# AtharvRN/dflash

Hardware: AMD Instinct MI355X
Metric: accepted_tokens_per_sec (higher is better)
Workload: dtype bf16

## Files before the change

### dflash_amd/_lib.py

```python
from __future__ import annotations

import ctypes as C
import os

import torch

HERE = os.path.dirname(os.path.abspath(__file__))
LIB_PATH = os.environ.get("DFL_LIB_PATH") or os.path.join(HERE, "lib", "libdflash_hip.so")

_p, _i, _i64, _f, _u64 = C.c_void_p, C.c_int, C.c_int64, C.c_float, C.c_uint64


class Rows(C.Structure):
    _fields_ = [("frag", C.c_void_p), ("rows", C.c_void_p), ("ld", C.c_int64), ("ss", C.c_void_p),
                ("nss", C.c_int32), ("norm_w", C.c_void_p), ("eps", C.c_float), ("valid_word", C.c_int32),
                ("mode", C.c_int32)]


_r = C.POINTER(Rows)


class RowsBatch(C.Structure):
    _fields_ = [("r0", Rows), ("frag_stride", C.c_int64), ("rows_stride", C.c_int64), ("ss_stride", C.c_int64)]


_rb = C.POINTER(RowsBatch)

W_BF16, W_E4M3 = 0, 1


class Weight(C.Structure):
    _fields_ = [("wp", C.c_void_p), ("scale", C.c_void_p), ("format", C.c_int32)]


_w = C.POINTER(Weight)

SIGNATURES = {
    "dfl_version": (_i, []),
    "dfl_last_error": (C.c_char_p, []),
    "dfl_pack_weight": (_i, [_p, _p, _i, _i, _p]),
    "dfl_pack_weight_gateup": (_i, [_p, _p, _p, _i, _i, _p]),
    "dfl_set_dyn": (_i, [_p, _i, _i, _i, _i, _p]),
    "dfl_set_dyn2": (_i, [_p, _i, _i, _i, _i, _p]),
    "dfl_pack_rows": (_i, [_p, _i64, _i, _i, _p, _p, _i, _p]),
    "dfl_gemm_f32": (_i, [_p, _r, _r, _i, _i, _i, _i, _p, _p, _p]),
    "dfl_gemm_silu_mul": (_i, [_w, _r, _i, _i, _p, _p, _p]),
    "dfl_gemm_resid": (_i, [_w, _r, _i, _i, _p, _i64, _i, _p, _i64, _p, _p, _p]),
    "dfl_embed_rows": (_i, [_p, _p, _p, _i, _p, _p, _i, _p]),
    "dfl_pack_weight_fp8": (_i, [_p, _p, _i, _i, _p]),
    "dfl_pack_weight_gateup_fp8": (_i, [_p, _p, _p, _i, _i, _p]),
    "dfl_argmax_ws_bytes": (_i64, []),
    "dfl_gemm_argmax": (_i, [_w, _r, _i, _i, _i, _i, _p, _i, _p, _p, _i, _p, _p, _p, _p, _p]),
    "dfl_gemm_sample": (_i, [_w, _r, _i, _i, _i, _i, _p, _i, _p, _p, _i, _p, _p, _u64, _f, _i, _p, _i, _i, _i, _p]),
    "dfl_sample_rows": (_i, [_p, _i64, _i, _i, _u64, _f, _i, _i, _p, _i, _p, _p, _p]),
    "dfl_sample_rows_nucleus": (_i, [_p, _i64, _i64, _i, _i, _i, _i, _p, _i, _i, _i, _p, _i, _i, _p, _u64, _p, _i, _p, _f,
                                     _p, _f, _i, _i, _p, _i64, _i, _p, _p, _p]),
    "dfl_norm_pack": (_i, [_p, _i, _i64, _i, _i, _p, _p, _p, _p, _p, _i64, _p, _f, _p, _i, _p, _i, _p]),
    "dfl_qknorm_rope_append": (_i, [_p, _i, _i64, _i, _i, _i, _i, _i, _i, _i, _i, _p, _p, _f, _p, _p, _i, _p, _p, _p, _i, _p,
                                    _i, _i, _p]),
    "dfl_attn_ws_bytes": (_i64, [_i, _i]),
    "dfl_block_attn": (_i, [_p, _p, _p, _i, _i, _i, _f, _i, _p, _i, _p, _i, _p, _p]),
    "dfl_attn_fused_ws_bytes": (_i64, [_i, _i, _i]),
    "dfl_attn_fused": (_i, [_p, _i, _i64, _i, _i, _i, _i, _i, _i, _i, _i, _p, _p, _f, _p, _p, _i, _p, _p, _i, _f, _i, _p,
                            _i, _p, _i, _p, _p]),
    "dfl_attn_head_ws_bytes": (_i64, [_i, _i, _i]),
    "dfl_attn_head": (_i, [_p, _i64, _i, _i, _i, _p, _i64, _i, _i, _i, _i, _p, _p, _f, _p, _p, _i, _p, _p, _i, _f, _i,
                           _p, _i, _i, _i, _i, _i, _p, _i, _p, _i64, _p]),
    "dfl_attn_head_oproj": (_i, [_p, _i64, _i, _i, _i, _p, _i64, _i, _i, _i, _i, _p, _p, _f, _p, _p, _i, _p, _p, _i, _f, _i,
                                 _p, _i, _i, _i, _i, _p, _i, _p, _p, _i, _p, _i64, _p, _p, _p]),
    "dfl_attn_head_cand": (_i, [_p, _i64, _i, _i, _i, _i, _i64, _i, _i, _p, _p, _f, _p, _p, _i, _p, _p, _i, _f, _i, _i,
                                _p, _i, _p, _i64, _i64, _i, _p, _p, _i64, _i, _p]),
    "dfl_attn_head_batch_f32": (_i, [_p, _i, _i64, _i64, _i, _i, _i, _i, _i64, _i, _i, _p, _p, _f, _p, _p, _i, _p, _p, _i, _i64, _f,
                                     _i, _p, _i, _p, _i, _p, _i64, _p]),
    "dfl_attn_head_batch": (_i, [_p, _i64, _i, _i, _i, _i, _i64, _i, _i, _p, _p, _f, _p, _p, _i, _p, _p, _i, _i64, _f, _i,
                                 _p, _i, _p, _i, _p, _i64, _i64, _i, _p]),
    "dfl_topk_rows": (_i, [_p, _i64, _i, _i, _i, _p, _p, _p, _p]),
    "dfl_candidate_select": (_i, [_p, _i64, _p, _i64, _p, _i, _i, _p, _i64, _p, _p, _i, _p, _p]),
    "dfl_moe_route": (_i, [_p, _i, _i, _i, _i, _p, _p, _p, _p, _p, _i, _p]),
    "dfl_moe_router": (_i, [_p, _i64, _p, _f, _p, _p, _i, _i, _i, _i, _p, _i, _p, _p, _p, _p, _p, _i, _p, _p]),
    "dfl_gemm_silu_mul_experts": (_i, [_p, _i64, _r, _i, _i, _i, _p, _i64, _p, _p, _p, _p]),
    "dfl_moe_gate_up": (_i, [_w, _p, _i, _i, _i, _p, _p, _p, _p, _i, _p]),
    "dfl_moe_down": (_i, [_w, _i64, _p, _i64, _p, _p, _p, _i, _i, _i, _i, _p, _p]),
    "dfl_argmax": (_i, [_p, _i, _i, _i64, _p, _p]),
    "dfl_accept_commit": (_i, [_p, _p, _i, _p, _i64, _p, _p, _i, _p, _p, _i, _i64, _p, _p]),
    "dfl_prefill_rows_padded": (_i64, [_i]),
    "dfl_prefill_gemm_rows": (_i, [_p, _p, _i, _i, _i, _p, _i64, _p]),
    "dfl_prefill_gemm_resid": (_i, [_p, _p, _i, _i, _i, _p, _i64, _p, _i64, _p]),
    "dfl_prefill_gemm_silu": (_i, [_p, _p, _i, _i, _i, _p, _p]),
    "dfl_prefill_norm_pack": (_i, [_p, _i64, _i, _i, _p, _f, _p, _p]),
    "dfl_prefill_pack_rows": (_i, [_p, _i64, _i, _i, _p, _p]),
    "dfl_prefill_qk_rope": (_i, [_p, _i64, _i, _i, _i, _i, _i, _i, _p, _p, _f, _p, _p, _i, _i, _p, _p, _i, _i, _p]),
    "dfl_prefill_attn": (_i, [_p, _i64, _i, _p, _p, _i, _i, _i, _i, _f, _p, _p]),
    "dfl_prefill_moe_max_tiles": (_i64, [_i, _i, _i]),
    "dfl_prefill_moe_max_items": (_i64, [_i, _i, _i]),
    "dfl_prefill_moe_route": (_i, [_p, _i64, _i, _i, _i, _i, _p, _p, _p, _p, _p, _p, _p, _p, _p, _i, _p]),
    "dfl_prefill_moe_gather": (_i, [_p, _i, _i, _i, _i, _p, _p, _p, _p]),
    "dfl_prefill_moe_gemm_silu": (_i, [_p, _i64, _p, _p, _p, _i, _i, _i, _p, _i, _p, _p, _p]),
    "dfl_prefill_moe_gemm_down": (_i, [_p, _i64, _p, _p, _p, _i, _i, _i, _p, _p, _i, _p]),
    "dfl_prefill_moe_combine": (_i, [_p, _p, _i, _i, _i, _p, _i64, _p, _i64, _p, _p]),
    "dfl_moe_grouped_gate_up": (_i, [_w, _i64, _p, _p, _p, _i, _i, _i, _p, _i, _p, _p, _p]),
    "dfl_moe_grouped_down": (_i, [_w, _i64, _p, _p, _p, _i, _i, _i, _p, _p, _i, _p]),
    "dfl_batch_tiles": (_i, [_i]),
    "dfl_batch_ksplit": (_i, [_i]),
    "dfl_gemm_batch_ws_bytes": (_i64, [_i, _i]),
    "dfl_gemm_f32_batch": (_i, [_w, _rb, _i, _i, _i, _p, _p, _p]),
    "dfl_gemm_silu_mul_batch": (_i, [_w, _rb, _i, _i, _i, _p, _i64, _p, _p, _p]),
    "dfl_gemm_resid_batch": (_i, [_p, _rb, _i, _i, _i, _p, _i64, _i64, _i, _p, _i64, _i64, _p, _i64, _p, _p, _p]),
    "dfl_gemm_argmax_batch": (_i, [_w, _rb, _i, _i, _i, _i, _i, _p, _i, _p, _p, _i64, _i, _p, _i64, _p]),
    "dfl_gemm_sample_batch": (_i, [_w, _rb, _i, _i, _i, _i, _i, _p, _i, _p, _p, _i64, _i, _p, _i64, _p, _p, _f, _i, _i, _i, _i,
                                   _p]),
    "dfl_embed_rows_batch": (_i, [_p, _p, _i64, _i, _p, _i64, _i, _p, _i64, _p, _i, _p]),
    "dfl_norm_frag_batch": (_i, [_p, _i64, _i64, _i, _p, _i, _i64, _i, _p, _i64, _i64, _p, _f, _p, _i64, _i, _p, _i, _p]),
    "dfl_kv_append_batch": (_i, [_p, _i, _i64, _i, _i, _i, _i, _i, _i, _i, _i, _p, _i64, _f, _p, _p, _i, _p, _p, _i,
                                 _i64, _i64, _p, _i, _p]),
    "dfl_attn_fused_batch_ws_bytes": (_i64, [_i, _i, _i, _i]),
    "dfl_attn_fused_batch": (_i, [_p, _i, _i64, _i, _i, _i, _i, _i, _i, _i, _i, _i, _p, _p, _f, _p, _p, _i, _p, _p, _i,
                                  _i64, _f, _i, _p, _i, _p, _i, _p, _i64, _p]),
    "dfl_accept_commit_batch": (_i, [_p, _i64, _p, _i64, _i, _p, _i64, _i64, _p, _p, _p, _i, _p, _p, _i64, _i, _p, _p, _p]),
    "dfl_admit_slot": (_i, [_i, _i, _p, _i, _p, _p, _i64, _i64, _p, _p, _i, _p, _p, _i64, _i, _p, _i, _p, _p, _i, _p, _i64,
                            _i64, _p]),
}

_lib = None


class DFlashHipError(RuntimeError):
    pass


def lib():
    global _lib
    if _lib is None:
        if not os.path.exists(LIB_PATH):
            raise DFlashHipError(
                f"{LIB_PATH} not found: build it with `python -m dflash_amd.build` (hipcc, gfx950). "
                "dflash_amd has no CPU or PyTorch fallback for its kernels.")
        handle = C.CDLL(LIB_PATH)
        for name, (res, args) in SIGNATURES.items():
            fn = getattr(handle, name)
            fn.restype, fn.argtypes = res, args
        if handle.dfl_version() != 1:
            raise DFlashHipError(f"ABI version mismatch: library {handle.dfl_version()} != binding 1")
        _lib = handle
    return _lib


def check(rc: int, what: str) -> None:
    if rc != 0:
        raise DFlashHipError(f"{what} failed (rc={rc}): {lib().dfl_last_error().decode()}")
```

### dflash_amd/csrc/gemm_rows.h

```cpp
#pragma once
#include "dfl_common.h"

namespace {

enum { EPI_F32 = 0, EPI_SILU = 1, EPI_ARGMAX = 2, EPI_RESID = 3, EPI_SILU_E = 4 ,
       EPI_SAMPLE = 5 ,
       EPI_SAMPLE_T = 6  };

struct RowSrc {
  const bf16x8 *frag;
  const bf16_t *rows;
  int64_t ld;
  const float *ss;
  int nss;
  const bf16_t *nw;
  float eps;
  int valid_word;
  int mode;
};

__device__ __forceinline__ bf16x8 ld_stream(const bf16x8 *p) { return __builtin_nontemporal_load(p); }

template <int NF, int AUX = 2 >
__device__ __forceinline__ void load_ksteps(bf16x8 (&wr)[NF], const bf16x8 *first, int nf, int l, int half = -1) {
  const __amdgpu_buffer_rsrc_t r =
      __builtin_amdgcn_make_buffer_rsrc(const_cast<bf16x8 *>(first), 0, (nf < 0 ? 0 : nf) * 1024, 0x00020000);
  const int voff = (half < 0 || ((l >> 3) & 1) == half) ? l * 16 : 0x40000000;
#pragma unroll
  for (int f = 0; f < NF; ++f)
    wr[f] = __builtin_bit_cast(bf16x8, __builtin_amdgcn_raw_buffer_load_b128(r, voff + (f & 3) * 1024, (f >> 2) * 4096, AUX));
}

template <int NF, int AUX = 2>
__device__ __forceinline__ void load_ksteps_w8(bf16x8 (&wr)[NF / 2], const bf16x8 *first, int nf, int l, int half = -1) {
  static_assert(NF % 2 == 0, "W8: a wave's share is a whole number of k-step pairs");
  load_ksteps<NF / 2, AUX>(wr, first, nf >> 1, l, half);
}

__device__ __forceinline__ bf16x8 w8_frag(bf16x8 raw, int hi) {
  const u32x4 q = __builtin_bit_cast(u32x4, raw);
  const uint32_t d0 = hi ? q[2] : q[0], d1 = hi ? q[3] : q[1];
  const bf16x2 a = __builtin_amdgcn_cvt_scalef32_pk_bf16_fp8(d0, 1.0f, false);
  const bf16x2 b = __builtin_amdgcn_cvt_scalef32_pk_bf16_fp8(d0, 1.0f, true);
  const bf16x2 c = __builtin_amdgcn_cvt_scalef32_pk_bf16_fp8(d1, 1.0f, false);
  const bf16x2 d = __builtin_amdgcn_cvt_scalef32_pk_bf16_fp8(d1, 1.0f, true);
  return (bf16x8){a[0], a[1], b[0], b[1], c[0], c[1], d[0], d[1]};
}

template <bool W8, int NW>
__device__ __forceinline__ bf16x8 weight_frag(const bf16x8 (&wr)[NW], int f) {
  if constexpr (W8)
    return w8_frag(wr[f >> 1], f & 1);
  else
    return wr[f];
}

typedef float f32x16 __attribute__((ext_vector_type(16)));
__device__ __forceinline__ f32x16 tile_scales(const float *wscale, int t) {
  typedef const __attribute__((address_space(4))) f32x16 *cptr;
  return *(cptr)(uintptr_t)(wscale + (size_t)__builtin_amdgcn_readfirstlane(t) * 16);
}
__device__ __forceinline__ f32x4 lane_scales(const f32x16 &s, int fg) {
  f32x4 o;
#pragma unroll
  for (int r = 0; r < 4; ++r) o[r] = fg == 0 ? s[r] : fg == 1 ? s[4 + r] : fg == 2 ? s[8 + r] : s[12 + r];
  return o;
}

__device__ __forceinline__ float row_sum16(float v) {
  v += __builtin_bit_cast(float, __builtin_amdgcn_mov_dpp(__builtin_bit_cast(int, v), 0xB1, 0xF, 0xF, true));
  v += __builtin_bit_cast(float, __builtin_amdgcn_mov_dpp(__builtin_bit_cast(int, v), 0x4E, 0xF, 0xF, true));
  v += __builtin_bit_cast(float, __builtin_amdgcn_mov_dpp(__builtin_bit_cast(int, v), 0x141, 0xF, 0xF, true));
  v += __builtin_bit_cast(float, __builtin_amdgcn_mov_dpp(__builtin_bit_cast(int, v), 0x140, 0xF, 0xF, true));
  return v;
}

template <int NF, bool NORM = true>
__device__ __forceinline__ void issue_x(const RowSrc &s, const int (&ks)[NF], int l, int nv, bf16x8 (&raw)[NF],
                                        bf16x8 (&wv)[NF]) {
  (void)nv;
  const int m = l & 15, kq = l >> 4;
  const bool fr = s.mode == 0;
  const char *base = fr ? reinterpret_cast<const char *>(s.frag) + l * 16
                        : reinterpret_cast<const char *>(s.rows) + ((int64_t)m * s.ld + kq * 8) * 2;
  const int kstep = fr ? 1024 : 64;
  const char *nwb = s.mode == 2 ? reinterpret_cast<const char *>(s.nw) + kq * 16 : base;
  const int nstep = s.mode == 2 ? 64 : kstep;
#pragma unroll
  for (int f = 0; f < NF; ++f) raw[f] = *reinterpret_cast<const bf16x8 *>(base + (int64_t)ks[f] * kstep);
  if (NORM) {
#pragma unroll
    for (int f = 0; f < NF; ++f) wv[f] = *reinterpret_cast<const bf16x8 *>(nwb + (int64_t)ks[f] * nstep);
  }
}

template <int NF, bool NORM = true>
__device__ __forceinline__ void finish_x(const RowSrc &s, const bool (&take)[NF], int l, int nv, float rstd,
                                         const bf16x8 (&raw)[NF], const bf16x8 (&wv)[NF], bf16x8 (&x)[NF]) {
  const bf16x8 z = {0, 0, 0, 0, 0, 0, 0, 0};
  if (s.mode == 0) {
#pragma unroll
    for (int f = 0; f < NF; ++f) x[f] = take[f] ? raw[f] : z;
    return;
  }
  const int m = l & 15;
  const bool norm = NORM && s.mode == 2;
#pragma unroll
  for (int f = 0; f < NF; ++f) {
    const bf16x8 r = raw[f];
    bf16x8 o = r;
    if (norm) {
      const bf16x8 wq = wv[f];
#pragma unroll
      for (int j = 0; j < 8; ++j) o[j] = f2bf(bf2f(wq[j]) * rbf(bf2f(r[j]) * rstd));
    }
    x[f] = (take[f] && m < nv) ? o : z;
  }
}

template <int NF>
__device__ __forceinline__ void finish_xl(const RowSrc &s, const int (&ks)[NF], const bool (&take)[NF], int l, int nv,
                                          float rstd, const bf16x8 (&raw)[NF], const bf16x8 *nwl, bf16x8 (&x)[NF]) {
  const bf16x8 z = {0, 0, 0, 0, 0, 0, 0, 0};
  if (s.mode == 0) {
#pragma unroll
    for (int f = 0; f < NF; ++f) x[f] = take[f] ? raw[f] : z;
    return;
  }
  const int m = l & 15, kq = l >> 4;
  const bool norm = s.mode == 2;
#pragma unroll
  for (int f = 0; f < NF; ++f) {
    const bf16x8 r = raw[f];
    bf16x8 o = r;
    if (norm) {
      const bf16x8 wq = nwl[(ks[f] * 4 + kq) & 511];
#pragma unroll
      for (int j = 0; j < 8; ++j) o[j] = f2bf(bf2f(wq[j]) * rbf(bf2f(r[j]) * rstd));
    }
    x[f] = (take[f] && m < nv) ? o : z;
  }
}

template <int NF, bool NORM = true>
__device__ __forceinline__ void build_x(const RowSrc &s, const int (&ks)[NF], const bool (&take)[NF], int l, int nv,
                                        float rstd, bf16x8 (&x)[NF]) {
  bf16x8 raw[NF], wv[NF];
#pragma unroll
  for (int f = 0; f < NF; ++f) wv[f] = raw[f] = (bf16x8){0, 0, 0, 0, 0, 0, 0, 0};
  issue_x<NF, NORM>(s, ks, l, nv, raw, wv);
  finish_x<NF, NORM>(s, take, l, nv, rstd, raw, wv, x);
}

inline int pick_ksplit_min(int KS, int fr_max) { return (KS + 16 * fr_max - 1) / (16 * fr_max); }

inline int grid_x_for(int ngroups, int ksplit = 1) {
  int gx_max = 256 / ksplit;
  if (gx_max < 1) gx_max = 1;
  const int per_wg = (ngroups + gx_max - 1) / gx_max;
  return (ngroups + per_wg - 1) / per_wg;
}

inline bool fill_src(RowSrc &d, const dfl_rows *s, int K, const char *who) {
  if (!s) {
    dfl_set_error("%s: null row source", who);
    return false;
  }
  d.frag = (const bf16x8 *)s->frag;
  d.rows = (const bf16_t *)s->rows;
  d.ld = s->ld;
  d.ss = s->ss;
  d.nss = s->nss;
  d.nw = (const bf16_t *)s->norm_w;
  d.eps = s->eps;
  d.valid_word = s->valid_word;
  d.mode = s->mode;

  const bool ok = (s->mode == 0 && s->frag) || (s->mode == 1 && s->rows && s->ld >= K && s->ld % 8 == 0) ||
                  (s->mode == 2 && s->rows && s->ss && s->nss >= 1 && s->norm_w && s->ld >= K && s->ld % 8 == 0);
  if (!ok) dfl_set_error("%s: bad row source (mode %d)", who, s->mode);
  if (ok && s->mode == 2 && K > 4096) {
    dfl_set_error("%s: a normalised row source needs K <= 4096 (K=%d)", who, K);
    return false;
  }
  if (ok && s->mode == 2 && s->nss > 256) {
    dfl_set_error("%s: a normalised row source takes at most 256 partial sums of squares (nss=%d)", who, s->nss);
    return false;
  }
  return ok;
}


}
```

### dflash_amd/csrc/gemm_skinny.hip

```cpp
#include "gemm_rows.h"
#include "dfl_rng.h"

namespace {

struct GemmArgs {
  const bf16x8 *wp;
  int KS;
  int ntiles;
  int nfr;
  int nch;
  int nhalf;
  int gx;
  const int32_t *dyn;
  RowSrc src[2];
  float *out;
  int ldo;
  bf16_t *act;
  const int32_t *elist, *n_active;
  int npp;
  int row0, nrows;
  int nrows_word;
  float *best_val;
  int *best_idx;
  float *best2_val;
  bf16_t *logits;
  int N;
  bf16_t *h_io;
  int64_t ldh;
  int add_resid;
  bf16_t *tap;
  int64_t ldtap;
  float *ss_out;
  const float *wscale;
};

struct SampleArgs {
  uint64_t seed;
  float inv_t;
  int rng_stream;
  const int32_t *pos_dyn;
  int pos_word, pos_base, pos_add;
};

struct HeadBits {
  uint64_t KS : 17, nfr : 4, mode : 2, valid_word1 : 6 , nrows_word1 : 6 , gx : 9,
      nhalf : 9, nch_nss : 11 ;
};
static_assert(sizeof(HeadBits) == 8, "HeadBits is one 64-bit kernel argument");
struct GemmHead {
  const bf16x8 *wp;
  const void *x;
  const float *ss;
  const bf16_t *nw;
  const int32_t *dyn;
  uint64_t bits;
  int ld, ntiles;
};
#define GEMM_HEAD_DWORDS 14
static_assert(sizeof(GemmHead) == 4 * GEMM_HEAD_DWORDS, "the head is what the hardware preloads: at most 14 dwords, no padding");
#define GEMM_HEAD_PARAMS \
  const bf16x8 *wp, const void *x, const float *ss, const bf16_t *nw, const int32_t *dyn, uint64_t bits, int ld, int ntiles
#define GEMM_HEAD_NAMES wp, x, ss, nw, dyn, bits, ld, ntiles
#define GEMM_HEAD_OF(h) (h).wp, (h).x, (h).ss, (h).nw, (h).dyn, (h).bits, (h).ld, (h).ntiles

template <bool CHUNKED, bool NORM>
__device__ __forceinline__ GemmArgs with_head(GemmArgs a, GEMM_HEAD_PARAMS) {
  const HeadBits b = __builtin_bit_cast(HeadBits, bits);
  a.wp = wp;
  a.dyn = dyn;
  a.ntiles = ntiles;
  a.KS = (int)b.KS;
  a.nfr = (int)b.nfr;
  a.nhalf = (int)b.nhalf;
  a.gx = (int)b.gx;
  a.nch = CHUNKED ? (int)b.nch_nss : 1;
  a.nrows_word = (int)b.nrows_word1 - 1;
  RowSrc &s = a.src[0];
  s.frag = reinterpret_cast<const bf16x8 *>(x);
  s.rows = reinterpret_cast<const bf16_t *>(x);
  s.ld = ld;
  s.ss = ss;
  s.nw = nw;
  s.mode = (int)b.mode;
  s.valid_word = (int)b.valid_word1 - 1;
  if (NORM) s.nss = (int)b.nch_nss;
  return a;
}

template <bool CHUNKED>
bool gemm_head(GemmHead &h, const GemmArgs &a) {
  const RowSrc &s = a.src[0];
  HeadBits b{};
  b.KS = a.KS;
  b.nfr = a.nfr;
  b.mode = s.mode;
  b.valid_word1 = s.valid_word < 0 ? 0 : s.valid_word + 1;
  b.nrows_word1 = a.nrows_word < 0 ? 0 : a.nrows_word + 1;
  b.gx = a.gx;
  b.nhalf = a.nhalf;
  const int nch_nss = CHUNKED ? a.nch : (s.mode == 2 ? s.nss : 0);
  b.nch_nss = nch_nss;
  const int64_t ld = s.mode == 0 ? 0 : s.ld;
  const bool fits = (int)b.KS == a.KS && (int)b.nfr == a.nfr && (int)b.mode == s.mode && (int)b.gx == a.gx &&
                    (int)b.nhalf == a.nhalf && (int)b.nch_nss == nch_nss && (CHUNKED || a.nch == 1) && ld == (int)ld &&
                    (int)b.valid_word1 == (s.valid_word < 0 ? 0 : s.valid_word + 1) &&
                    (int)b.nrows_word1 == (a.nrows_word < 0 ? 0 : a.nrows_word + 1);
  if (!fits) {
    dfl_set_error("skinny GEMM: launch arguments outside the preloaded head's fields (K=%d, grid %d, ld=%lld)", a.KS * 32, a.gx,
                  (long long)s.ld);
    return false;
  }
  h.wp = a.wp;
  h.x = s.mode == 0 ? (const void *)s.frag : (const void *)s.rows;
  h.ss = s.ss;
  h.nw = s.nw;
  h.dyn = a.dyn;
  h.bits = __builtin_bit_cast(uint64_t, b);
  h.ld = (int)ld;
  h.ntiles = a.ntiles;
  return true;
}

#ifdef DFL_GEMM_STAMPS
__device__ unsigned long long g_gstamps[8];
__device__ unsigned long long g_wgstamps[256][4];
#define GSTAMP(i)                                                                         \
  do {                                                                                    \
    if (threadIdx.x == 0 && blockIdx.x == 0 && blockIdx.y == 0) g_gstamps[i] = __builtin_amdgcn_s_memrealtime(); \
    if (threadIdx.x == 0 && blockIdx.y == 0 && blockIdx.x < 256 && ((i) == 0 || (i) == 4 || (i) == 5))            \
      g_wgstamps[blockIdx.x][(i) == 0 ? 0 : (i) - 3] = __builtin_amdgcn_s_memrealtime();                           \
  } while (0)
#else
#define GSTAMP(i)
#endif

constexpr int gemm_fr(int MT, bool CHUNKED) { return CHUNKED ? 4 : (MT == 1 ? 8 : 4); }

template <int MT, bool CHUNKED, int EPI, bool NORM, bool W8 = false>
__device__ __forceinline__ void gemm_body(const GemmArgs &a, const SampleArgs &sa) {
  GSTAMP(0);
  constexpr int FR = gemm_fr(MT, CHUNKED);
  constexpr int NW = W8 ? FR / 2 : FR;
  __shared__ float red[2][16][MT][256];
  __shared__ float ssred[NORM ? MT : 1][16][16];
  __shared__ bf16x8 nwl[NORM ? MT : 1][NORM ? 512 : 1];

  const int tid = threadIdx.x;
  const int w = __builtin_amdgcn_readfirstlane(tid >> 6);
  const int l = tid & 63;

  auto ks0_of = [&](int c) { return ((blockIdx.y * a.nch + c) * 16 + w) * a.nfr; };
  auto nf_of = [&](int c) {
    int nf = a.KS - ks0_of(c);
    return nf < 0 ? 0 : (nf > a.nfr ? a.nfr : nf);
  };

  const int stride = a.gx;
  constexpr bool SILU = EPI == EPI_SILU || EPI == EPI_SILU_E;
  constexpr bool moe = EPI == EPI_SILU_E;
  const int nwhole = (!SILU && (int)blockIdx.x < a.ntiles) ? (a.ntiles - 1 - (int)blockIdx.x) / stride + 1 : 0;
  const bool has_half = !SILU && (int)blockIdx.x < a.nhalf;
  const int myhalf = (int)blockIdx.x & 1;
  auto half_of = [&](int j) -> int { return (!SILU && j >= nwhole) ? myhalf : -1; };
  auto tile_of = [&](int j) -> int {
    if (!SILU) return j < nwhole ? (int)blockIdx.x + j * stride : a.ntiles + ((int)blockIdx.x >> 1);
    int p = (int)blockIdx.x + (j >> 1) * stride;
    if (moe) p = a.elist[p / a.npp] * a.npp + p % a.npp;
    return 2 * p + (j & 1);
  };

  bf16x8 wA[NW], wB[NW];
  float scA = 1.f, scB = 1.f;
  bf16x8 xA[MT][FR], xB[MT][FR];
  bf16x8 xr[MT][FR];

  const int nf0 = nf_of(0);
  const int ngroups = SILU ? a.ntiles >> 1 : a.ntiles;
  int nseq;
  if (SILU) {
    const int npairs = moe ? a.n_active[0] * a.npp : a.ntiles >> 1;
    nseq = (int)blockIdx.x < npairs ? 2 * ((npairs - 1 - (int)blockIdx.x) / stride + 1) : 0;
  } else {
    nseq = nwhole + (has_half ? 1 : 0);
  }
  const int nitems = nseq * a.nch;

  int nv[MT];
  auto read_nv = [&]() {
#pragma unroll
    for (int mt = 0; mt < MT; ++mt) {
      const RowSrc &s0 = a.src[mt];
      nv[mt] = (s0.valid_word >= 0 && a.dyn) ? a.dyn[s0.valid_word] : 16;
    }
  };

  float best = -INFINITY;
  int bestn = 0x7fffffff;
  float second = -INFINITY;
  float gate_sum = 0.f;
  int arg_rows = 0;
  int pos_row0 = 0, rng_extra = 0;

  auto load_item_x = [&](bf16x8(&xb)[MT][FR], int c) {
    const int ks0 = ks0_of(c);
    int ks[FR];
#pragma unroll
    for (int f = 0; f < FR; ++f) ks[f] = ks0 + f < a.KS ? ks0 + f : a.KS - 1;
    bf16x8 wv[MT][FR];
#pragma unroll
    for (int mt = 0; mt < MT; ++mt)
#pragma unroll
      for (int f = 0; f < FR; ++f) wv[mt][f] = xb[mt][f] = (bf16x8){0, 0, 0, 0, 0, 0, 0, 0};
#pragma unroll
    for (int mt = 0; mt < MT; ++mt) issue_x<FR, false>(a.src[mt], ks, l, nv[mt], xb[mt], wv[mt]);
  };
  auto load_w8 = [&](bf16x8(&wr)[NW], float &sc, int t, int ks0, int nf, int half) {
    if constexpr (W8) {
      load_ksteps_w8<FR>(wr, a.wp + ((size_t)t * (a.KS >> 1) + (ks0 >> 1)) * 64, nf, l, half);
      sc = a.wscale[(size_t)t * 16 + (tid & 15)];
    }
  };
  auto load_item = [&](bf16x8(&wr)[NW], float &sc, bf16x8(&xb)[MT][FR], int t, int c, int half) {
    if constexpr (W8)
      load_w8(wr, sc, t, ks0_of(c), nf_of(c), half);
    else
      load_ksteps<FR>(wr, a.wp + ((size_t)t * a.KS + ks0_of(c)) * 64, nf_of(c), l, half);
    if (CHUNKED) load_item_x(xb, c);
  };

  f32x4 acc[MT];
  constexpr bool PREF = EPI == EPI_RESID && !NORM;
  bf16_t resid0 = (bf16_t)0.f;

  auto finish = [&](int t, int pos, float wsc) {
    const int buf = pos & 1;
    const int hf = half_of(pos);
#pragma unroll
    for (int mt = 0; mt < MT; ++mt) *reinterpret_cast<f32x4 *>(&red[buf][w][mt][l * 4]) = acc[mt];
    __syncthreads();
    if (tid < MT * 256) {
      const int mt = tid >> 8, ff = tid & 255;
      const int m = ff >> 4, nl = ff & 15;
      const int idx = 4 * (m + 16 * (nl >> 2)) + (nl & 3);
      float s = 0.f;
#pragma unroll
      for (int ww = 0; ww < 16; ++ww) s += red[buf][ww][mt][idx];
      if (W8) s *= wsc;
      const bool colok = hf < 0 || (nl >> 3) == hf;
      if (EPI == EPI_F32) {
        if (colok) a.out[((size_t)(blockIdx.y * MT + mt) * 16 + m) * a.ldo + t * 16 + nl] = s;
      } else if (SILU) {
        if (buf == 0) {
          gate_sum = s;
        } else {
          const float gb = rbf(gate_sum), ub = rbf(s);
          const float act = rbf(gb / (1.f + __expf(-gb)));
          const int n = (t >> 1) * 16 + nl;
          a.act[((size_t)(n >> 3) * 16 + m) * 8 + (n & 7)] = f2bf(act * ub);
        }
      } else if (EPI == EPI_ARGMAX || EPI == EPI_SAMPLE) {
        const int n = t * 16 + nl;
        float vb = rbf(s);
        const bool live = (m >= a.row0) && (m < a.row0 + arg_rows) && colok;
        if (a.logits && live) a.logits[(size_t)m * a.N + n] = f2bf(s);
        if (EPI == EPI_SAMPLE) {
          uint32_t wd[4];
          dfl_rng_words(sa.seed, (uint32_t)sa.rng_stream, (uint32_t)(pos_row0 + m), (uint32_t)n, (uint32_t)rng_extra, wd);
          const int k = nl & 3;
          vb = dfl_perturb_w(vb, sa.inv_t, k == 0 ? wd[0] : (k == 1 ? wd[1] : (k == 2 ? wd[2] : wd[3])));
        }
        if (live && (vb > best || bestn == 0x7fffffff)) {
          second = best;
          best = vb;
          bestn = n;
        } else if (live) {
          second = fmaxf(second, vb);
        }
      } else {
        const int n = t * 16 + nl;
        const float v = rbf(s);
        bf16_t *hp = a.h_io + (int64_t)m * a.ldh + n;
        float hn = v;
        if (a.add_resid) hn = rbf(bf2f((PREF && pos == 0) ? resid0 : *hp) + v);
        if (colok) {
          *hp = f2bf(hn);
          if (a.tap) a.tap[(int64_t)m * a.ldtap + n] = f2bf(hn);
        }
        const float q = row_sum16(hn * hn);
        if (nl == 0 && a.ss_out) a.ss_out[t * 16 + m] = q;
      }
    }
  };

  auto process = [&](bf16x8(&wr)[NW], float wsc, bf16x8(&xb)[MT][FR], int t, int c, int pos) {
    if (!CHUNKED || c == 0) {
#pragma unroll
      for (int mt = 0; mt < MT; ++mt) acc[mt] = (f32x4){0.f, 0.f, 0.f, 0.f};
    }
    const int ks0c = ks0_of(c);
#pragma unroll
    for (int f = 0; f < FR; ++f)
#pragma unroll
      for (int mt = 0; mt < MT; ++mt) {
        bf16x8 xv = xr[mt][f];
        if (CHUNKED) {
          const bool keep = ks0c + f < a.KS && (a.src[mt].mode == 0 || (l & 15) < nv[mt]);
          xv = keep ? xb[mt][f] : (bf16x8){0, 0, 0, 0, 0, 0, 0, 0};
        }
        acc[mt] = __builtin_amdgcn_mfma_f32_16x16x32_bf16(weight_frag<W8>(wr, f), xv, acc[mt], 0, 0, 0);
      }
    if (!CHUNKED || c == a.nch - 1) finish(t, pos, wsc);
  };

  const int first_tile = (SILU || nwhole > 0) ? (int)blockIdx.x : a.ntiles + ((int)blockIdx.x >> 1);
  const int first_half = (SILU || nwhole > 0) ? -1 : myhalf;
  const bool first_live = SILU ? (int)blockIdx.x < ngroups : (nwhole > 0 || has_half);
  auto ask_resid0 = [&]() {
    if (PREF) {
      const int ff = tid & 255;
      resid0 = a.h_io[(int64_t)(ff >> 4) * a.ldh + first_tile * 16 + (ff & 15)];
    }
  };

  read_nv();
  int arg_word = 0;
  const bool arg_dyn = (EPI == EPI_ARGMAX || EPI == EPI_SAMPLE) && a.dyn && a.nrows_word >= 0;
  if (arg_dyn) arg_word = a.dyn[a.nrows_word];
  if (EPI == EPI_SAMPLE) {
    const int base = sa.pos_dyn ? sa.pos_dyn[sa.pos_word] : sa.pos_base;
    pos_row0 = base + sa.pos_add;
    rng_extra = sa.rng_stream == (int)DFL_RNG_DRAFT ? base : 0;
  }
  __builtin_amdgcn_sched_barrier(0);
  float rstd[MT];
#pragma unroll
  for (int mt = 0; mt < MT; ++mt) rstd[mt] = 1.f;
  if (!CHUNKED) {
    bf16x8 nwv[MT];
    float ssv[MT][4];
    bool any_norm = false;
#pragma unroll
    for (int mt = 0; mt < MT; ++mt) {
      const RowSrc &s = a.src[mt];
#pragma unroll
      for (int u = 0; u < 4; ++u) ssv[mt][u] = 0.f;
      nwv[mt] = (bf16x8){0, 0, 0, 0, 0, 0, 0, 0};
      if (NORM) {
        const int c = min(tid & 511, a.KS * 4 - 1);
        const char *nb = s.mode == 2 ? reinterpret_cast<const char *>(s.nw)
                                     : (s.mode == 0 ? reinterpret_cast<const char *>(s.frag) : reinterpret_cast<const char *>(s.rows));
        nwv[mt] = *reinterpret_cast<const bf16x8 *>(nb + c * 16);
      }
      if (NORM && s.mode == 2) {
        const int m = l & 15, part = l >> 4;
#pragma unroll
        for (int u = 0; u < 4; ++u) {
          const int i = w + 16 * (part + 4 * u);
          ssv[mt][u] = s.ss[(i < s.nss ? i : s.nss - 1) * 16 + m];
        }
        any_norm = true;
      }
    }
    int ks[FR];
    bool take[FR];
#pragma unroll
    for (int f = 0; f < FR; ++f) {
      take[f] = f < nf0;
      ks[f] = take[f] ? ks0_of(0) + f : 0;
    }
    bf16x8 raw[MT][FR], wv0[MT][FR];
#pragma unroll
    for (int mt = 0; mt < MT; ++mt)
#pragma unroll
      for (int f = 0; f < FR; ++f) wv0[mt][f] = raw[mt][f] = (bf16x8){0, 0, 0, 0, 0, 0, 0, 0};
#pragma unroll
    for (int mt = 0; mt < MT; ++mt) issue_x<FR, false>(a.src[mt], ks, l, 16, raw[mt], wv0[mt]);
    __builtin_amdgcn_sched_barrier(0);
    if (!NORM) {
      __builtin_amdgcn_s_barrier();
      __builtin_amdgcn_sched_barrier(0);
    }
    if constexpr (W8)
      load_w8(wA, scA, SILU ? 2 * (int)blockIdx.x : first_tile, ks0_of(0), first_live ? nf0 : 0, first_half);
    else if (!moe)
      load_ksteps<FR>(wA, a.wp + ((size_t)(SILU ? 2 * blockIdx.x : first_tile) * a.KS + ks0_of(0)) * 64,
                      first_live ? nf0 : 0, l, first_half);
    else if (nitems > 0)
      load_ksteps<FR>(wA, a.wp + ((size_t)tile_of(0) * a.KS + ks0_of(0)) * 64, nf0, l);
    GSTAMP(6);
    __builtin_amdgcn_sched_barrier(0);
    ask_resid0();
    GSTAMP(1);
    if (NORM && any_norm) {
#pragma unroll
      for (int mt = 0; mt < MT; ++mt) {
        const RowSrc &s = a.src[mt];
        if (NORM) nwl[mt][tid & 511] = nwv[mt];
        if (NORM && s.mode == 2) {
          const int m = l & 15, part = l >> 4;
          float v[4];
#pragma unroll
          for (int u = 0; u < 4; ++u) v[u] = (w + 16 * (part + 4 * u)) < s.nss ? ssv[mt][u] : 0.f;
          float t = (v[0] + v[1]) + (v[2] + v[3]);
          t += __shfl_xor(t, 16, 64);
          t += __shfl_xor(t, 32, 64);
          if (part == 0) ssred[mt][w][m] = t;
        }
      }
      __syncthreads();
#pragma unroll
      for (int mt = 0; mt < MT; ++mt)
        if (a.src[mt].mode == 2) {
          float t = 0.f;
#pragma unroll
          for (int ww = 0; ww < 16; ++ww) t += ssred[mt][ww][l & 15];
          rstd[mt] = rsqrtf(t / (float)(a.KS * 32) + a.src[mt].eps);
        }
    }
    GSTAMP(2);
#pragma unroll
    for (int mt = 0; mt < MT; ++mt) {
      if (NORM)
        finish_xl<FR>(a.src[mt], ks, take, l, nv[mt], rstd[mt], raw[mt], nwl[mt], xr[mt]);
      else
        finish_x<FR, false>(a.src[mt], take, l, nv[mt], 1.f, raw[mt], wv0[mt], xr[mt]);
    }
  } else {
    if constexpr (W8)
      load_w8(wA, scA, first_tile, ks0_of(0), first_live ? nf0 : 0, first_half);
    else if (nitems > 0 || !moe)
      load_ksteps<FR>(wA, a.wp + ((size_t)first_tile * a.KS + ks0_of(0)) * 64, first_live ? nf0 : 0, l, first_half);
    GSTAMP(6);
    load_item_x(xA, 0);
    ask_resid0();
    GSTAMP(1);
    GSTAMP(2);
  }

  if (EPI == EPI_ARGMAX || EPI == EPI_SAMPLE) arg_rows = arg_dyn ? arg_word - a.row0 : a.nrows;
  GSTAMP(3);
  if (nitems > 0) {
    int j = 0, c = 0;
    for (int i = 0;; i += 2) {
      int jn = j, cn = c + 1;
      if (cn == a.nch) {
        cn = 0;
        ++jn;
      }
      if (i + 1 < nitems) load_item(wB, scB, xB, tile_of(jn), cn, half_of(jn));
      process(wA, scA, xA, tile_of(j), c, j);
      if (i == 0) GSTAMP(4);
      if (i + 1 >= nitems) break;
      int j2 = jn, c2 = cn + 1;
      if (c2 == a.nch) {
        c2 = 0;
        ++j2;
      }
      if (i + 2 < nitems) load_item(wA, scA, xA, tile_of(j2), c2, half_of(j2));
      process(wB, scB, xB, tile_of(jn), cn, jn);
      if (i + 2 >= nitems) break;
      j = j2;
      c = c2;
    }
  }

  GSTAMP(5);
  if (EPI == EPI_ARGMAX || EPI == EPI_SAMPLE) {
    if (tid < 256) {
#pragma unroll
      for (int o = 1; o <= 8; o <<= 1) {
        const float ov = __shfl_xor(best, o, 64);
        const int oi = __shfl_xor(bestn, o, 64);
        const float os = __shfl_xor(second, o, 64);
        second = fmaxf(fmaxf(second, os), fminf(best, ov));
        if (ov > best || (ov == best && oi < bestn)) {
          best = ov;
          bestn = oi;
        }
      }
      if ((tid & 15) == 0) {
        a.best_val[blockIdx.x * 16 + (tid >> 4)] = best;
        a.best_idx[blockIdx.x * 16 + (tid >> 4)] = bestn;
        if (a.best2_val) a.best2_val[blockIdx.x * 16 + (tid >> 4)] = second;
      }
    }
  }
}

template <int MT, bool CHUNKED, int EPI, bool NORM>
__global__ __launch_bounds__(1024) void k_gemm(GEMM_HEAD_PARAMS, GemmArgs rest) {
  gemm_body<MT, CHUNKED, EPI, NORM>(with_head<CHUNKED, NORM>(rest, GEMM_HEAD_NAMES), SampleArgs{});
}

template <bool CHUNKED, int EPI, bool NORM>
__global__ __launch_bounds__(1024) void k_gemm_w8(GEMM_HEAD_PARAMS, GemmArgs rest) {
  gemm_body<1, CHUNKED, EPI, NORM, true>(with_head<CHUNKED, NORM>(rest, GEMM_HEAD_NAMES), SampleArgs{});
}

template <bool NORM>
__global__ __launch_bounds__(1024) void k_gemm_s(GEMM_HEAD_PARAMS, GemmArgs rest, SampleArgs sa) {
  gemm_body<1, false, EPI_SAMPLE, NORM>(with_head<false, NORM>(rest, GEMM_HEAD_NAMES), sa);
}

template <bool NORM>
__global__ __launch_bounds__(1024) void k_gemm_s_w8(GEMM_HEAD_PARAMS, GemmArgs rest, SampleArgs sa) {
  gemm_body<1, false, EPI_SAMPLE, NORM, true>(with_head<false, NORM>(rest, GEMM_HEAD_NAMES), sa);
}

template <int MT, bool CHUNKED, int EPI, bool W8 = false>
bool launch_gemm(GemmArgs &a, dim3 grid, hipStream_t stream) {
  bool norm = false;
  for (int mt = 0; mt < MT; ++mt) norm |= a.src[mt].mode == 2;
  a.gx = (int)grid.x;
  GemmHead h;
  if (!gemm_head<CHUNKED>(h, a)) return false;
  if constexpr (W8) {
    static_assert(MT == 1, "the W8 kernels take one 16-row tile");
    if (!a.wscale || a.KS % 2 || a.nfr % 2) {
      dfl_set_error("skinny GEMM (fp8): needs a scale vector, K %% 64 == 0 and an even share per wave (K=%d, nfr=%d)",
                    a.KS * 32, a.nfr);
      return false;
    }
    if constexpr (!CHUNKED) {
      if (norm) {
        hipLaunchKernelGGL((k_gemm_w8<false, EPI, true>), grid, dim3(1024), 0, stream, GEMM_HEAD_OF(h), a);
        return true;
      }
    }
    hipLaunchKernelGGL((k_gemm_w8<CHUNKED, EPI, false>), grid, dim3(1024), 0, stream, GEMM_HEAD_OF(h), a);
    return true;
  }
  if constexpr (!CHUNKED) {
    if (norm) {
      hipLaunchKernelGGL((k_gemm<MT, false, EPI, true>), grid, dim3(1024), 0, stream, GEMM_HEAD_OF(h), a);
      return true;
    }
  }
  hipLaunchKernelGGL((k_gemm<MT, CHUNKED, EPI, false>), grid, dim3(1024), 0, stream, GEMM_HEAD_OF(h), a);
  return true;
}

__global__ __launch_bounds__(64) void k_argmax_finish(const float *best_val, const int *best_idx, const float *best2_val,
                                                      int nblk, int row0, int nrows, const int32_t *dyn, int nrows_word,
                                                      int64_t *out_ids, int out_off, float *margin_out) {
  int rows = nrows;
  if (dyn && nrows_word >= 0) rows = dyn[nrows_word] - row0;
  const int m = row0 + blockIdx.x;
  if ((int)blockIdx.x >= rows) return;
  float bv = -INFINITY, sv = -INFINITY;
  int bi = 0x7fffffff;
  for (int b = threadIdx.x; b < nblk; b += 64) {
    const float ov = best_val[b * 16 + m];
    const int oi = best_idx[b * 16 + m];
    const float os = best2_val ? best2_val[b * 16 + m] : -INFINITY;
    if (oi != 0x7fffffff) sv = fmaxf(fmaxf(sv, os), bi == 0x7fffffff ? -INFINITY : fminf(bv, ov));
    if (ov > bv || (ov == bv && oi < bi) || bi == 0x7fffffff) {
      bv = ov;
      bi = oi;
    }
  }
#pragma unroll
  for (int o = 32; o > 0; o >>= 1) {
    const float ov = __shfl_xor(bv, o, 64);
    const int oi = __shfl_xor(bi, o, 64);
    const float os = __shfl_xor(sv, o, 64);
    const bool have = bi != 0x7fffffff, ohave = oi != 0x7fffffff;
    sv = fmaxf(sv, os);
    if (have && ohave) sv = fmaxf(sv, fminf(bv, ov));
    if (ohave && (!have || ov > bv || (ov == bv && oi < bi))) {
      bv = ov;
      bi = oi;
    }
  }
  if (threadIdx.x == 0) {
    out_ids[out_off + blockIdx.x] = (int64_t)bi;
    if (margin_out) margin_out[out_off + blockIdx.x] = bv - sv;
  }
}

__global__ void k_pack_weight(const bf16x8 *__restrict__ w, bf16x8 *__restrict__ wp, int ntiles, int KS,
                              int tile_mul, int tile_add) {
  const size_t total = (size_t)ntiles * KS * 64;
  for (size_t c = blockIdx.x * (size_t)blockDim.x + threadIdx.x; c < total; c += (size_t)gridDim.x * blockDim.x) {
    const int l = c & 63;
    const size_t tk = c >> 6;
    const int ks = tk % KS;
    const size_t t = tk / KS;
    const size_t row = t * 16 + (l & 15);
    const size_t src = row * (size_t)(KS * 4) + (size_t)ks * 4 + (l >> 4);
    const size_t dt = t * tile_mul + tile_add;
    wp[(dt * KS + ks) * 64 + l] = w[src];
  }
}

__global__ void k_pack_weight_fp8(const uint2 *__restrict__ q, uint4 *__restrict__ wp, int ntiles, int KP, int tile_mul,
                                  int tile_add) {
  const size_t total = (size_t)ntiles * KP * 64;
  for (size_t c = blockIdx.x * (size_t)blockDim.x + threadIdx.x; c < total; c += (size_t)gridDim.x * blockDim.x) {
    const int l = c & 63;
    const size_t tj = c >> 6;
    const int j = tj % KP;
    const size_t t = tj / KP;
    const size_t row = t * 16 + (l & 15);
    const size_t src = row * (size_t)(KP * 8) + (size_t)j * 8 + (l >> 4);
    const uint2 lo = q[src], hi = q[src + 4];
    const size_t dt = t * tile_mul + tile_add;
    wp[(dt * KP + j) * 64 + l] = make_uint4(lo.x, lo.y, hi.x, hi.y);
  }
}

__global__ __launch_bounds__(256) void k_embed_rows(const bf16_t *embed, const int64_t *ids, bf16_t *h, int H,
                                                    float *ss_out, const int32_t *dyn, int dyn_word) {
  __shared__ float wsum[4];
  const int m = blockIdx.x, tid = threadIdx.x;
  const int nv = dyn ? dyn[dyn_word] : 16;
  float ss = 0.f;
  if (m < nv) {
    const bf16_t *src = embed + ids[m] * (int64_t)H;
    for (int c = tid; c < (H >> 3); c += 256) {
      const bf16x8 v = *reinterpret_cast<const bf16x8 *>(src + c * 8);
      *reinterpret_cast<bf16x8 *>(h + (int64_t)m * H + c * 8) = v;
#pragma unroll
      for (int j = 0; j < 8; ++j) ss += bf2f(v[j]) * bf2f(v[j]);
    }
  }
  ss = wave_sum(ss);
  if ((tid & 63) == 0) wsum[tid >> 6] = ss;
  __syncthreads();
  if (tid == 0) ss_out[m] = wsum[0] + wsum[1] + wsum[2] + wsum[3];
}

}

#ifdef DFL_GEMM_STAMPS
extern "C" int dfl_debug_read_gemm_stamps(unsigned long long *host_out) {
  return (int)hipMemcpyFromSymbol(host_out, HIP_SYMBOL(g_gstamps), sizeof(unsigned long long) * 8);
}
extern "C" int dfl_debug_read_wg_stamps(unsigned long long *host_out) {
  return (int)hipMemcpyFromSymbol(host_out, HIP_SYMBOL(g_wgstamps), sizeof(unsigned long long) * 256 * 4);
}
#endif

static void plan_tiles(GemmArgs &a, int ntiles, bool allow_half, int &gx) {
  gx = grid_x_for(ntiles);
  a.ntiles = ntiles;
  a.nhalf = 0;
  const int r = ntiles % 256;
  if (allow_half && ntiles <= 128) {
    gx = 2 * ntiles;
    a.ntiles = 0;
    a.nhalf = 2 * ntiles;
    return;
  }
  if (!allow_half || ntiles <= 256 || r == 0 || r > 128) return;
  gx = 256;
  a.ntiles = ntiles - r;
  a.nhalf = 2 * r;
}

extern "C" int dfl_pack_weight(const void *w, void *wp, int N, int K, void *stream) {
  DFL_REQUIRE(w && wp, "dfl_pack_weight: null pointer");
  DFL_REQUIRE(N > 0 && K > 0 && N % 16 == 0 && K % 32 == 0, "dfl_pack_weight: need N%%16==0, K%%32==0 (N=%d K=%d)", N, K);
  hipLaunchKernelGGL(k_pack_weight, dim3(2048), dim3(256), 0, (hipStream_t)stream, (const bf16x8 *)w, (bf16x8 *)wp,
                     N / 16, K / 32, 1, 0);
  DFL_CHECK_LAUNCH("dfl_pack_weight");
  return DFL_OK;
}

extern "C" int dfl_pack_weight_gateup(const void *gate, const void *up, void *wp, int I, int K, void *stream) {
  DFL_REQUIRE(gate && up && wp, "dfl_pack_weight_gateup: null pointer");
  DFL_REQUIRE(I > 0 && K > 0 && I % 16 == 0 && K % 32 == 0, "dfl_pack_weight_gateup: need I%%16==0, K%%32==0");
  hipLaunchKernelGGL(k_pack_weight, dim3(2048), dim3(256), 0, (hipStream_t)stream, (const bf16x8 *)gate,
                     (bf16x8 *)wp, I / 16, K / 32, 2, 0);
  hipLaunchKernelGGL(k_pack_weight, dim3(2048), dim3(256), 0, (hipStream_t)stream, (const bf16x8 *)up, (bf16x8 *)wp,
                     I / 16, K / 32, 2, 1);
  DFL_CHECK_LAUNCH("dfl_pack_weight_gateup");
  return DFL_OK;
}

extern "C" int dfl_pack_weight_fp8(const void *q, void *wp8, int N, int K, void *stream) {
  DFL_REQUIRE(q && wp8, "dfl_pack_weight_fp8: null pointer");
  DFL_REQUIRE(N > 0 && K > 0 && N % 16 == 0 && K % 64 == 0, "dfl_pack_weight_fp8: need N%%16==0, K%%64==0 (N=%d K=%d)", N, K);
  hipLaunchKernelGGL(k_pack_weight_fp8, dim3(2048), dim3(256), 0, (hipStream_t)stream, (const uint2 *)q, (uint4 *)wp8,
                     N / 16, K / 64, 1, 0);
  DFL_CHECK_LAUNCH("dfl_pack_weight_fp8");
  return DFL_OK;
}

extern "C" int dfl_pack_weight_gateup_fp8(const void *gate_q, const void *up_q, void *wp8, int I, int K, void *stream) {
  DFL_REQUIRE(gate_q && up_q && wp8, "dfl_pack_weight_gateup_fp8: null pointer");
  DFL_REQUIRE(I > 0 && K > 0 && I % 16 == 0 && K % 64 == 0, "dfl_pack_weight_gateup_fp8: need I%%16==0, K%%64==0 (I=%d K=%d)", I,
              K);
  hipLaunchKernelGGL(k_pack_weight_fp8, dim3(2048), dim3(256), 0, (hipStream_t)stream, (const uint2 *)gate_q, (uint4 *)wp8,
                     I / 16, K / 64, 2, 0);
  hipLaunchKernelGGL(k_pack_weight_fp8, dim3(2048), dim3(256), 0, (hipStream_t)stream, (const uint2 *)up_q, (uint4 *)wp8,
                     I / 16, K / 64, 2, 1);
  DFL_CHECK_LAUNCH("dfl_pack_weight_gateup_fp8");
  return DFL_OK;
}

extern "C" int dfl_embed_rows(const void *embed, const int64_t *ids, void *h_out, int H, float *ss_out,
                              const int32_t *dyn, int dyn_word, void *stream) {
  DFL_REQUIRE(embed && ids && h_out && ss_out, "dfl_embed_rows: null pointer");
  DFL_REQUIRE(H > 0 && H % 8 == 0, "dfl_embed_rows: H%%8 != 0");
  hipLaunchKernelGGL(k_embed_rows, dim3(16), dim3(256), 0, (hipStream_t)stream, (const bf16_t *)embed, ids,
                     (bf16_t *)h_out, H, ss_out, dyn, dyn_word);
  DFL_CHECK_LAUNCH("dfl_embed_rows");
  return DFL_OK;
}

extern "C" int dfl_gemm_f32(const void *wp, const dfl_rows *x0, const dfl_rows *x1, int mt, int N, int K, int ksplit,
                            float *out, const int32_t *dyn, void *stream) {
  DFL_REQUIRE(wp && out, "dfl_gemm_f32: null pointer");
  DFL_REQUIRE(mt == 1 || mt == 2, "dfl_gemm_f32: mt must be 1 or 2");
  DFL_REQUIRE(N > 0 && K > 0 && N % 16 == 0 && K % 32 == 0, "dfl_gemm_f32: need N%%16==0, K%%32==0 (N=%d K=%d)", N, K);
  const int KS = K / 32;
  const int fr_max = mt == 1 ? 8 : 4;
  DFL_REQUIRE(ksplit >= pick_ksplit_min(KS, fr_max) && ksplit <= 64, "dfl_gemm_f32: ksplit=%d too small for K=%d (need >= %d)",
              ksplit, K, pick_ksplit_min(KS, fr_max));
  GemmArgs a{};
  if (!fill_src(a.src[0], x0, K, "dfl_gemm_f32")) return DFL_EINVAL;
  if (mt == 2 && !fill_src(a.src[1], x1, K, "dfl_gemm_f32")) return DFL_EINVAL;
  a.wp = (const bf16x8 *)wp;
  a.dyn = dyn;
  a.KS = KS;
  a.ntiles = N / 16;
  a.nfr = (KS + 16 * ksplit - 1) / (16 * ksplit);
  a.nch = 1;
  a.out = out;
  a.ldo = N;
  int gx1 = 0;
  if (ksplit == 1) plan_tiles(a, N / 16, true, gx1);
  dim3 grid(ksplit == 1 ? gx1 : grid_x_for(a.ntiles, ksplit), ksplit);
  const bool ok = mt == 1 ? launch_gemm<1, false, EPI_F32>(a, grid, (hipStream_t)stream)
                          : launch_gemm<2, false, EPI_F32>(a, grid, (hipStream_t)stream);
  if (!ok) return DFL_EINVAL;
  DFL_CHECK_LAUNCH("dfl_gemm_f32");
  return DFL_OK;
}

namespace {
template <bool W8>
int gemm_silu_mul_impl(const char *who, const dfl_weight *w, const dfl_rows *x, int I, int K, void *act_frag,
                       const int32_t *dyn, void *stream) {
  DFL_REQUIRE(w->wp && act_frag && (!W8 || w->scale), "%s: null pointer", who);
  DFL_REQUIRE(I > 0 && K > 0 && I % 16 == 0 && K % (W8 ? 64 : 32) == 0, "%s: need I%%16==0, K%%%d==0", who, W8 ? 64 : 32);
  const int KS = K / 32;
  DFL_REQUIRE(KS <= 16 * 8, "%s: K=%d needs a K split, which the fused activation cannot take", who, K);
  GemmArgs a{};
  if (!fill_src(a.src[0], x, K, who)) return DFL_EINVAL;
  a.wp = (const bf16x8 *)w->wp;
  a.wscale = w->scale;
  a.dyn = dyn;
  a.KS = KS;
  a.ntiles = 2 * (I / 16);
  a.nfr = (KS + 15) / 16;
  if (W8) a.nfr += a.nfr & 1;
  a.nch = 1;
  a.act = (bf16_t *)act_frag;
  if (!launch_gemm<1, false, EPI_SILU, W8>(a, dim3(grid_x_for(I / 16), 1), (hipStream_t)stream)) return DFL_EINVAL;
  DFL_CHECK_LAUNCH(who);
  return DFL_OK;
}
}

extern "C" int dfl_gemm_silu_mul(const dfl_weight *w_gateup, const dfl_rows *x, int I, int K, void *act_frag,
                                 const int32_t *dyn, void *stream) {
  const char *who = "dfl_gemm_silu_mul";
  if (!weight_ok(who, w_gateup)) return DFL_EINVAL;
  return w_gateup->format == DFL_W_BF16 ? gemm_silu_mul_impl<false>(who, w_gateup, x, I, K, act_frag, dyn, stream)
                                        : gemm_silu_mul_impl<true>(who, w_gateup, x, I, K, act_frag, dyn, stream);
}

extern "C" int dfl_gemm_silu_mul_experts(const void *wp_gateup, int64_t wp_expert_stride, const dfl_rows *x, int E, int I, int K,
                                         void *act_frag, int64_t act_expert_stride, const int32_t *list,
                                         const int32_t *n_active, const int32_t *dyn, void *stream) {
  DFL_REQUIRE(wp_gateup && act_frag && list && n_active, "dfl_gemm_silu_mul_experts: null pointer");
  DFL_REQUIRE(E >= 1 && E <= 1024 && I > 0 && K > 0 && I % 16 == 0 && K % 32 == 0, "dfl_gemm_silu_mul_experts: bad shape");
  DFL_REQUIRE(wp_expert_stride == (int64_t)2 * I * K && act_expert_stride == (int64_t)16 * I,
              "dfl_gemm_silu_mul_experts: the experts' weights and outputs must lie back to back (strides %lld, %lld)",
              (long long)wp_expert_stride, (long long)act_expert_stride);
  const int KS = K / 32;
  DFL_REQUIRE(KS <= 16 * 8, "dfl_gemm_silu_mul_experts: K=%d exceeds 4096", K);
  GemmArgs a{};
  if (!fill_src(a.src[0], x, K, "dfl_gemm_silu_mul_experts")) return DFL_EINVAL;
  a.wp = (const bf16x8 *)wp_gateup;
  a.dyn = dyn;
  a.KS = KS;
  a.ntiles = 2 * (I / 16) * E;
  a.nfr = (KS + 15) / 16;
  a.nch = 1;
  a.act = (bf16_t *)act_frag;
  a.elist = list;
  a.n_active = n_active;
  a.npp = I / 16;
  if (!launch_gemm<1, false, EPI_SILU_E>(a, dim3(256, 1), (hipStream_t)stream)) return DFL_EINVAL;
  DFL_CHECK_LAUNCH("dfl_gemm_silu_mul_experts");
  return DFL_OK;
}

extern "C" int64_t dfl_argmax_ws_bytes(void) { return 256 * 16 * (int64_t)(2 * sizeof(float) + sizeof(int)); }

namespace {
int gemm_argmax_impl(const char *who, const dfl_weight *w, const dfl_rows *x, int V, int K, int row0, int nrows,
                     const int32_t *dyn, int nrows_dyn_word, void *ws, int64_t *out_ids, int out_off, void *logits,
                     float *margin_out, hipEvent_t ev0, hipEvent_t ev1, void *stream, const SampleArgs *smp = nullptr) {
  const bool w8 = w->format == DFL_W_E4M3;
  DFL_REQUIRE(w->wp && ws && out_ids && (!w8 || w->scale), "%s: null pointer", who);
  DFL_REQUIRE(V > 0 && K > 0 && V % 16 == 0 && K % (w8 ? 64 : 32) == 0, "%s: need V%%16==0, K%%%d==0 (V=%d K=%d)", who,
              w8 ? 64 : 32, V, K);
  DFL_REQUIRE(row0 >= 0 && nrows >= 0 && row0 + nrows <= 16, "%s: rows [%d,%d) outside the 16-row tile", who, row0,
              row0 + nrows);
  const int KS = K / 32;
  DFL_REQUIRE(KS <= 16 * 8, "%s: K=%d exceeds 4096 (argmax needs finished sums)", who, K);
  GemmArgs a{};
  if (!fill_src(a.src[0], x, K, who)) return DFL_EINVAL;
  a.wp = (const bf16x8 *)w->wp;
  a.dyn = dyn;
  a.KS = KS;
  a.ntiles = V / 16;
  a.nfr = (KS + 15) / 16;
  if (w8) a.nfr += a.nfr & 1;
  a.wscale = w->scale;
  a.nch = 1;
  a.row0 = row0;
  a.nrows = nrows;
  a.nrows_word = nrows_dyn_word;
  a.best_val = (float *)ws;
  a.best_idx = (int *)((char *)ws + 256 * 16 * sizeof(float));
  a.best2_val = margin_out ? (float *)((char *)ws + 256 * 16 * (sizeof(float) + sizeof(int))) : nullptr;
  a.logits = (bf16_t *)logits;
  a.N = V;
  int gx = 0;
  plan_tiles(a, V / 16, true, gx);
  if (ev0) (void)hipEventRecord(ev0, (hipStream_t)stream);
  if (smp) {
    a.gx = gx;
    GemmHead h;
    if (!gemm_head<false>(h, a)) return DFL_EINVAL;
    if (w8) {
      if (a.src[0].mode == 2)
        hipLaunchKernelGGL(k_gemm_s_w8<true>, dim3(gx, 1), dim3(1024), 0, (hipStream_t)stream, GEMM_HEAD_OF(h), a, *smp);
      else
        hipLaunchKernelGGL(k_gemm_s_w8<false>, dim3(gx, 1), dim3(1024), 0, (hipStream_t)stream, GEMM_HEAD_OF(h), a, *smp);
    } else if (a.src[0].mode == 2)
      hipLaunchKernelGGL(k_gemm_s<true>, dim3(gx, 1), dim3(1024), 0, (hipStream_t)stream, GEMM_HEAD_OF(h), a, *smp);
    else
      hipLaunchKernelGGL(k_gemm_s<false>, dim3(gx, 1), dim3(1024), 0, (hipStream_t)stream, GEMM_HEAD_OF(h), a, *smp);
  } else if (w8) {
    if (!launch_gemm<1, false, EPI_ARGMAX, true>(a, dim3(gx, 1), (hipStream_t)stream)) return DFL_EINVAL;
  } else {
    if (!launch_gemm<1, false, EPI_ARGMAX>(a, dim3(gx, 1), (hipStream_t)stream)) return DFL_EINVAL;
  }
  if (ev1) (void)hipEventRecord(ev1, (hipStream_t)stream);
  hipLaunchKernelGGL(k_argmax_finish, dim3(16), dim3(64), 0, (hipStream_t)stream, a.best_val, a.best_idx, a.best2_val, gx,
                     row0, nrows, dyn, nrows_dyn_word, out_ids, out_off, margin_out);
  DFL_CHECK_LAUNCH(who);
  return DFL_OK;
}
}

extern "C" int dfl_gemm_argmax(const dfl_weight *w, const dfl_rows *x, int V, int K, int row0, int nrows,
                               const int32_t *dyn, int nrows_dyn_word, void *ws, int64_t *out_ids, int out_off,
                               void *logits, float *margin_out, void *ev_start, void *ev_end, void *stream) {
  const char *who = "dfl_gemm_argmax";
  if (!weight_ok(who, w)) return DFL_EINVAL;
  return gemm_argmax_impl(who, w, x, V, K, row0, nrows, dyn, nrows_dyn_word, ws, out_ids, out_off, logits, margin_out,
                          (hipEvent_t)ev_start, (hipEvent_t)ev_end, stream);
}

extern "C" int dfl_gemm_sample(const dfl_weight *w, const dfl_rows *x, int V, int K, int row0, int nrows,
                               const int32_t *dyn, int nrows_dyn_word, void *ws, int64_t *out_ids, int out_off,
                               void *logits, float *margin_out, uint64_t seed, float inv_t, int rng_stream,
                               const int32_t *pos_dyn, int pos_word, int pos_base, int pos_add, void *stream) {
  const char *who = "dfl_gemm_sample";
  if (!weight_ok(who, w)) return DFL_EINVAL;
  DFL_REQUIRE(w->wp && (w->format == DFL_W_BF16 || w->scale) && ws && out_ids, "%s: null pointer", who);
  DFL_REQUIRE(inv_t > 0.f && inv_t <= 1e5f, "%s: inv_t=%g outside (0, 1e5]", who, (double)inv_t);
  DFL_REQUIRE(rng_stream == (int)DFL_RNG_TARGET || rng_stream == (int)DFL_RNG_DRAFT, "%s: unknown stream %d", who,
              rng_stream);
  DFL_REQUIRE(!pos_dyn || (pos_word >= 0 && pos_word < DFL_DYN_WORDS), "%s: pos_word=%d outside the record", who, pos_word);
  const SampleArgs smp{seed, inv_t, rng_stream, pos_dyn, pos_word, pos_base, pos_add};
  return gemm_argmax_impl(who, w, x, V, K, row0, nrows, dyn, nrows_dyn_word, ws, out_ids, out_off, logits, margin_out,
                          nullptr, nullptr, stream, &smp);
}


namespace {
template <bool W8>
int gemm_resid_impl(const char *who, const dfl_weight *w, const dfl_rows *x, int N, int K, void *h_io, int64_t ldh,
                    int add_residual, void *tap, int64_t ldtap, float *ss_out, const int32_t *dyn, void *stream) {
  DFL_REQUIRE(w->wp && h_io && (!W8 || w->scale), "%s: null pointer", who);
  DFL_REQUIRE(N > 0 && K > 0 && N % 16 == 0 && K % (W8 ? 64 : 32) == 0, "%s: need N%%16==0, K%%%d==0 (N=%d K=%d)", who,
              W8 ? 64 : 32, N, K);
  DFL_REQUIRE(ldh >= N && (!tap || ldtap >= N), "%s: row strides shorter than N", who);
  const int KS = K / 32;
  GemmArgs a{};
  if (!fill_src(a.src[0], x, K, who)) return DFL_EINVAL;
  a.wp = (const bf16x8 *)w->wp;
  a.wscale = w->scale;
  a.dyn = dyn;
  a.KS = KS;
  a.ntiles = N / 16;
  a.h_io = (bf16_t *)h_io;
  a.ldh = ldh;
  a.add_resid = add_residual ? 1 : 0;
  a.tap = (bf16_t *)tap;
  a.ldtap = ldtap;
  a.ss_out = ss_out;
  int gx = 0;
  plan_tiles(a, N / 16, KS <= 16 * 8 && !ss_out, gx);
  const dim3 grid(gx, 1);
  if (KS <= 16 * 8) {
    a.nfr = (KS + 15) / 16;
    if (W8) a.nfr += a.nfr & 1;
    a.nch = 1;
    if (!launch_gemm<1, false, EPI_RESID, W8>(a, grid, (hipStream_t)stream)) return DFL_EINVAL;
  } else {
    DFL_REQUIRE(a.src[0].mode != 2, "%s: a normalised source needs K <= 4096", who);
    a.nfr = 4;
    a.nch = (KS + 63) / 64;
    if (!launch_gemm<1, true, EPI_RESID, W8>(a, grid, (hipStream_t)stream)) return DFL_EINVAL;
  }
  DFL_CHECK_LAUNCH(who);
  return DFL_OK;
}
}

extern "C" int dfl_gemm_resid(const dfl_weight *w, const dfl_rows *x, int N, int K, void *h_io, int64_t ldh,
                              int add_residual, void *tap, int64_t ldtap, float *ss_out, const int32_t *dyn,
                              void *stream) {
  const char *who = "dfl_gemm_resid";
  if (!weight_ok(who, w)) return DFL_EINVAL;
  return w->format == DFL_W_BF16
             ? gemm_resid_impl<false>(who, w, x, N, K, h_io, ldh, add_residual, tap, ldtap, ss_out, dyn, stream)
             : gemm_resid_impl<true>(who, w, x, N, K, h_io, ldh, add_residual, tap, ldtap, ss_out, dyn, stream);
}
```

### dflash_amd/model.py

```python
from __future__ import annotations

import json
import os
from typing import Optional

import torch

from . import ops
from .config import DFlashConfig
from .tile_stack import TileStack, gemm_ws

BF16 = torch.bfloat16


def _rope_tables(head_dim: int, theta: float, max_pos: int, device):
    inv = 1.0 / (theta ** (torch.arange(0, head_dim, 2, dtype=torch.float) / head_dim))
    pos = torch.arange(max_pos, dtype=torch.float)
    freqs = (inv[None, :, None] @ pos[None, None, :]).transpose(1, 2)[0]
    return freqs.cos().to(BF16).to(device).contiguous(), freqs.sin().to(BF16).to(device).contiguous()


class DFlashKVCache:

    def __init__(self, cfg: DFlashConfig, max_rows: int, device):
        self.cfg = cfg
        self.max_rows = int(max_rows)
        L, kv = cfg.num_hidden_layers, cfg.num_key_value_heads
        self.k = torch.zeros(L, kv, self.max_rows, cfg.head_dim, dtype=BF16, device=device)
        self.v = torch.zeros_like(self.k)
        self.dyn = torch.zeros(16, dtype=torch.int32, device=device)
        self.length = 0

    def get_seq_length(self, layer_idx: int = 0) -> int:
        return self.length

    def crop(self, max_length: int) -> None:
        if 0 < max_length < self.length:
            self.length = int(max_length)
        elif max_length < 0:
            self.length = max(0, self.length + int(max_length))



class WideRows:

    def __init__(self, src, dyn, tiles: int = 2):
        self.src, self.dyn, self.tiles = src, dyn, tiles

    def __len__(self):
        return self.tiles


WEIGHT_FORMATS = ("bf16", "fp8_e4m3")


class DFlashDraftModel:
    def __init__(self, config, device=None, weight_format: str = "bf16"):
        if weight_format not in WEIGHT_FORMATS:
            raise ValueError(f"weight_format must be one of {WEIGHT_FORMATS}, got {weight_format!r}")
        self.weight_format = weight_format
        self.config = DFlashConfig.from_any(config)
        c = self.config
        if c.head_dim != 128:
            raise NotImplementedError("the gfx950 kernels are built for head_dim == 128")
        if c.hidden_size % 32 or c.intermediate_size % 32 or c.vocab_size % 16:
            raise NotImplementedError("need hidden/intermediate % 32 == 0 and vocab % 16 == 0")
        self.wide_hidden = c.hidden_size // 32 > 128
        self.block_size = c.block_size
        self.mask_token_id = c.mask_token_id
        self.target_layer_ids = list(c.target_layer_ids)
        self.device = torch.device(device) if device is not None else torch.device("cuda", torch.cuda.current_device())
        self.dtype = BF16
        if weight_format == "fp8_e4m3" and any(k % 64 for k in (c.hidden_size, c.intermediate_size, c.fc_in, c.q_dim)):
            raise NotImplementedError("fp8_e4m3 weights need hidden, intermediate, fc input and q widths % 64 == 0")
        self.w: Optional[dict] = None
        self.w8: Optional[dict] = None
        self.fp8_stream = True
        self._ws = None
        self._lm_head_cache = {}
        self._lm_head_cache8 = {}
        self._tile_layers = {}
        self._rope = None
        self.attn_impl = "head"
        self.fuse_oproj = False
        self.wide_one_pass = True
        self._wide = None
        self.lm_head_events = None
        self.lm_head_events_log = None
        self.wide_prefill = True
        self.rows_prefill = True

    def eval(self):
        return self

    def load_state_dict(self, sd: dict, strict: bool = True):
        c = self.config
        want = c.state_dict_shapes()
        missing = [k for k in want if k not in sd]
        unexpected = [k for k in sd if k not in want and "rotary_emb" not in k]
        if strict and (missing or unexpected):
            raise KeyError(f"load_state_dict: missing={missing[:4]}... unexpected={unexpected[:4]}...")
        for k, shape in want.items():
            if k in sd and tuple(sd[k].shape) != tuple(shape):
                raise ValueError(f"{k}: shape {tuple(sd[k].shape)} != {tuple(shape)}")

        def dev(name):
            return sd[name].to(device=self.device, dtype=BF16).contiguous()

        fp8 = self.weight_format == "fp8_e4m3"
        w8 = {"layers": []} if fp8 else None

        def mat(name, store, key):
            m = dev(name)
            if fp8:
                m, store[key] = ops.quantize_keep_fp8(m)
            return m

        top8 = {}
        w = {"fc": ops.pack_weight(mat("fc.weight", top8, "fc")), "hidden_norm": dev("hidden_norm.weight"),
             "norm": dev("norm.weight"), "layers": []}
        if fp8:
            w8["fc"] = ops.pack_weight_fp8(*top8.pop("fc"))
        for i in range(c.num_hidden_layers):
            p = f"layers.{i}."
            l8 = {}
            qkv = torch.cat([mat(p + "self_attn.q_proj.weight", l8, "q"), mat(p + "self_attn.k_proj.weight", l8, "k"),
                             mat(p + "self_attn.v_proj.weight", l8, "v")], dim=0)
            gate, up = mat(p + "mlp.gate_proj.weight", l8, "gate"), mat(p + "mlp.up_proj.weight", l8, "up")
            o, down = mat(p + "self_attn.o_proj.weight", l8, "o"), mat(p + "mlp.down_proj.weight", l8, "down")
            if fp8:
                w8["layers"].append(ops.pack_layer_fp8(l8))
            del l8
            w["layers"].append({
                "qkv": ops.pack_weight(qkv),
                "o": ops.pack_weight(o),
                "gu": ops.pack_weight_gateup(gate, up),
                "down": ops.pack_weight(down),
                "q_norm": dev(p + "self_attn.q_norm.weight"), "k_norm": dev(p + "self_attn.k_norm.weight"),
                "ln1": dev(p + "input_layernorm.weight"), "ln2": dev(p + "post_attention_layernorm.weight"),
            })
            del qkv, gate, up, o, down
        w["kv_all"] = torch.cat([lw["qkv"][c.q_dim * c.hidden_size:] for lw in w["layers"]]).contiguous()
        w["k_norm_all"] = torch.stack([lw["k_norm"] for lw in w["layers"]]).contiguous()
        if fp8:
            nkv2 = 2 * c.kv_dim
            w8["kv_all"] = ops.Fp8Weight(
                torch.cat([l8["qkv"].wp[c.q_dim * c.hidden_size:] for l8 in w8["layers"]]).contiguous(),
                torch.cat([l8["qkv"].scale[c.q_dim:] for l8 in w8["layers"]]).contiguous(),
                c.num_hidden_layers * nkv2, c.hidden_size)
        torch.cuda.synchronize(self.device)
        self.w = w
        self.w8 = w8
        self._tile_layers = {}
        self._ws = None
        return self

    @classmethod
    def from_pretrained(cls, path: str, device=None, weight_format: str = "bf16", **_):
        from safetensors.torch import load_file
        with open(os.path.join(path, "config.json")) as f:
            cfg = json.load(f)
        model = cls(cfg, device=device, weight_format=weight_format)
        sd = {}
        for fn in sorted(os.listdir(path)):
            if fn.endswith(".safetensors"):
                sd.update(load_file(os.path.join(path, fn)))
        sd = {k[len("model."):] if k.startswith("model.") and k[6:] in model.config.state_dict_shapes() else k: v
              for k, v in sd.items()}
        return model.load_state_dict(sd)

    def _workspace(self):
        if self._ws is None:
            c, d = self.config, self.device
            H, I = c.hidden_size, c.intermediate_size
            nqkv = c.q_dim + 2 * c.kv_dim
            self.ks_fc = ops.pick_ksplit(H, c.fc_in, 1)
            self.ks_qkv = ops.pick_ksplit(nqkv, H, 2)
            self.ks_o = ops.pick_ksplit(H, c.q_dim, 1)
            self.ks_down = ops.pick_ksplit(H, I, 1)
            self.ks_kv = ops.pick_ksplit(2 * c.kv_dim, H, 1)
            npart = max(self.ks_fc * 16 * H, self.ks_qkv * 32 * nqkv, self.ks_o * 16 * H, self.ks_down * 16 * H,
                        self.ks_kv * 16 * 2 * c.kv_dim)
            self.max_splits = 32
            NT = 2
            self._ws = dict(
                th_frag=torch.zeros(16 * c.fc_in, dtype=BF16, device=d),
                ctx_frag=torch.zeros(16 * H, dtype=BF16, device=d),
                xn_frag=torch.zeros(NT, 16 * H, dtype=BF16, device=d),
                attn_frag=torch.zeros(NT, 16 * c.q_dim, dtype=BF16, device=d),
                act_frag=torch.zeros(NT, 16 * I, dtype=BF16, device=d),
                h=torch.zeros(16 * NT, H, dtype=BF16, device=d),
                ctxh=torch.zeros(16, H, dtype=BF16, device=d),
                ss_emb=torch.zeros(16 * NT, dtype=torch.float32, device=d),
                ss_h=torch.zeros(NT, H, dtype=torch.float32, device=d),
                ss_ctx=torch.zeros(H, dtype=torch.float32, device=d),
                q_rot=torch.zeros(c.num_attention_heads, 16, 128, dtype=BF16, device=d),
                part=torch.zeros(npart, dtype=torch.float32, device=d),
                attn_ws=ops.attn_fused_ws(c.num_attention_heads, c.num_key_value_heads, self.max_splits, d),
                argmax_ws=ops.argmax_ws(d),
                ids16=torch.zeros(16, dtype=torch.int64, device=d),
                xq=torch.zeros(16 * NT, nqkv, dtype=BF16, device=d),
                xc=torch.zeros(16, c.num_hidden_layers * 2 * c.kv_dim, dtype=BF16, device=d),
                head_ws=ops.attn_head_ws(c.num_attention_heads, self.max_splits, NT, d),
                sync=torch.zeros(ops.ATTN_OPROJ_SYNC_WORDS, dtype=torch.int32, device=d),
            )
            ws, eps, nt = self._ws, c.rms_norm_eps, H // 16
            L = self.w["layers"]
            hs = [ws["h"][16 * t:16 * t + 16] for t in range(NT)]
            self._src = dict(
                ctx=ops.rows_normed(ws["ctxh"], ws["ss_ctx"], nt, self.w["hidden_norm"], eps, ops.DYN_TAU),
                ln1_first=[ops.rows_normed(hs[t], ws["ss_emb"][16 * t:], 1, L[0]["ln1"], eps, ops.DYN_BS) for t in range(NT)],
                ln1=[[ops.rows_normed(hs[t], ws["ss_h"][t], nt, lw["ln1"], eps, ops.DYN_BS) for t in range(NT)] for lw in L],
                ln2=[[ops.rows_normed(hs[t], ws["ss_h"][t], nt, lw["ln2"], eps, ops.DYN_BS) for t in range(NT)] for lw in L],
                final=[ops.rows_normed(hs[t], ws["ss_h"][t], nt, self.w["norm"], eps, ops.DYN_BS) for t in range(NT)],
                attn=[ops.rows_frag(ws["attn_frag"][t]) for t in range(NT)],
                act=[ops.rows_frag(ws["act_frag"][t]) for t in range(NT)],
            )
        return self._ws

    def _rope_tab(self, need: int):
        if self._rope is None or self._rope[0].shape[0] < need:
            n = max(need, 4096)
            n = 1 << (n - 1).bit_length()
            self._rope = _rope_tables(self.config.head_dim, self.config.rope_theta, n, self.device)
        return self._rope

    def new_cache(self, max_rows: int) -> DFlashKVCache:
        return DFlashKVCache(self.config, max_rows, self.device)

    def packed_lm_head(self, lm_head) -> torch.Tensor:
        wt = lm_head.weight if hasattr(lm_head, "weight") else lm_head
        key = (wt.data_ptr(), tuple(wt.shape), wt._version)
        if key not in self._lm_head_cache:
            self._lm_head_cache.clear()
            self._lm_head_cache[key] = ops.pack_weight(wt.detach().to(device=self.device, dtype=BF16).contiguous())
        return self._lm_head_cache[key]

    def packed_lm_head_fp8(self, lm_head) -> ops.Fp8Weight:
        wt = lm_head.weight if hasattr(lm_head, "weight") else lm_head
        key = (wt.data_ptr(), tuple(wt.shape), wt._version)
        if key not in self._lm_head_cache8:
            self._lm_head_cache8.clear()
            q, sc = ops.quantize_fp8_rows(wt.detach().to(device=self.device, dtype=BF16).contiguous())
            self._lm_head_cache8[key] = ops.pack_weight_fp8(q, sc)
        return self._lm_head_cache8[key]

    def streams_fp8(self, bs: int) -> bool:
        return (self.w8 is not None and self.fp8_stream and bs <= 16 and self.attn_impl == "head" and not self.fuse_oproj
                and not self.wide_hidden)

    def streams_fp8_tiles(self) -> bool:
        return self.w8 is not None and self.fp8_stream and self.attn_impl == "head"

    def tile_layers(self, qkv_parts: bool) -> list:
        if not self.streams_fp8_tiles():
            return self.w["layers"]
        return ops.tile_layers(self.w["layers"], self.w8["layers"], qkv_parts, self._tile_layers)

    def _ctx_rows(self, th_rows: torch.Tensor, n: int, dyn, dyn_word: Optional[int]):
        c, ws, w = self.config, self._workspace(), self.w
        ops.pack_rows(th_rows, n, ws["th_frag"], dyn if dyn_word is not None else None, dyn_word or 0)
        ops.gemm_f32(w["fc"], ws["th_frag"], None, 1, c.hidden_size, c.fc_in, self.ks_fc, ws["part"])
        ops.norm_pack(norm_w=w["hidden_norm"], frag=ws["ctx_frag"], H=c.hidden_size, eps=c.rms_norm_eps,
                      part=ws["part"], nsplit=self.ks_fc, part_split=16 * c.hidden_size, ldp=c.hidden_size,
                      dyn=dyn if dyn_word is not None else None, dyn_word=dyn_word or 0)

    def _prefill_ws(self):
        if getattr(self, "_pws", None) is None:
            c, d, MT = self.config, self.device, 4
            H, nkv = c.hidden_size, c.num_hidden_layers * 2 * c.kv_dim
            z = lambda *s_, dt=BF16: torch.zeros(*s_, dtype=dt, device=d)
            self._pws = dict(taps=z(MT, 16, c.fc_in), ctxh=z(MT, 16, H), xn=z(MT, 16 * H),
                             part=z(ops.batch_ksplit(H) * MT * 16 * nkv, dt=torch.float32),
                             dyn=z(MT, 8, dt=torch.int32),
                             gws=torch.zeros(ops.lib().dfl_gemm_batch_ws_bytes(H, c.fc_in), dtype=torch.uint8, device=d))
            p = self._pws
            p["src_taps"], p["src_xn"] = ops.brows_plain(p["taps"], ops.DYN_TAU), ops.brows_frag(p["xn"])
        return self._pws

    def _prefill_context_wide(self, cache: DFlashKVCache, th: torch.Tensor, pos0: int) -> None:
        c, w, p = self.config, self.w, self._prefill_ws()
        MT, H, L = 4, c.hidden_size, c.num_hidden_layers
        nkv = L * 2 * c.kv_dim
        n, S = th.shape[0], cache.length
        cos, sin = self._rope_tab(pos0 + n + 64)
        nsp = ops.batch_ksplit(H)
        for g0 in range(0, n, 64):
            rows = min(64, n - g0)
            R = (rows + 15) // 16
            rec = [[S + g0 + 16 * r, max(0, min(16, rows - 16 * r)), 0, pos0 + g0 + 16 * r, 0, 0, 0, 0] for r in range(MT)]
            p["dyn"].copy_(torch.tensor(rec, dtype=torch.int32))
            p["taps"].view(MT * 16, c.fc_in)[:rows].copy_(th[g0:g0 + rows])
            ops.gemm_resid_batch(w["fc"], p["src_taps"], R, H, c.fc_in, p["ctxh"], add_residual=False, ws=p["gws"],
                                 dyn=p["dyn"])
            ops.norm_frag_batch(p["ctxh"], R, w["hidden_norm"], c.rms_norm_eps, p["xn"], p["dyn"], ops.DYN_TAU)
            ops.gemm_f32_batch(w["kv_all"], p["src_xn"], R, nkv, H, p["part"], p["dyn"])
            ops.kv_append_batch(kv=p["part"], nsplit=nsp, split_stride=ops.batch_tiles(R) * 16 * nkv, ld=nkv, k_col=0,
                                v_col=c.kv_dim, col_layer_stride=2 * c.kv_dim, n_layers=L, R=R,
                                n_kv=c.num_key_value_heads, k_norm_w=w["k_norm_all"], eps=c.rms_norm_eps, cos_tab=cos,
                                sin_tab=sin, kcache=cache.k, vcache=cache.v, dyn=p["dyn"])
        cache.length = S + n

    def _prefill_context_rows(self, cache: DFlashKVCache, th: torch.Tensor, pos0: int) -> None:
        c, w = self.config, self.w
        H, L, n, S = c.hidden_size, c.num_hidden_layers, th.shape[0], cache.length
        nkv = L * 2 * c.kv_dim
        Pp = ops.prefill_rows_padded(n)
        r = getattr(self, "_rws", None)
        if r is None or r["h"].shape[0] < Pp:
            z = lambda *s_: torch.zeros(*s_, dtype=BF16, device=self.device)
            r = self._rws = dict(xf=z(Pp * c.fc_in), h=z(Pp, H), xn=z(Pp * H), kv=z(Pp, nkv))
        cos, sin = self._rope_tab(pos0 + n + 64)
        ops.prefill_pack_rows(th, n, c.fc_in, r["xf"])
        ops.prefill_gemm_rows(w["fc"], r["xf"], n, H, c.fc_in, r["h"])
        ops.prefill_norm_pack(r["h"], n, H, w["hidden_norm"], c.rms_norm_eps, r["xn"])
        ops.prefill_gemm_rows(w["kv_all"], r["xn"], n, nkv, H, r["kv"])
        for i, lw in enumerate(w["layers"]):
            ops.prefill_qk_rope(r["kv"], n, 0, i * 2 * c.kv_dim, i * 2 * c.kv_dim + c.kv_dim, 0, c.num_key_value_heads, None,
                                lw["k_norm"], c.rms_norm_eps, cos, sin, pos0, cache.k[i], cache.v[i], S)
        cache.length = S + n

    def prefill_context(self, cache: DFlashKVCache, target_hidden: torch.Tensor, pos0: int) -> None:
        c, ws, w = self.config, self._workspace(), self.w
        th = target_hidden.reshape(-1, c.fc_in)
        if th.dtype != BF16:
            raise TypeError("target_hidden must be bf16")
        n = th.shape[0]
        S = cache.length
        if S + n > cache.max_rows:
            raise ValueError("draft KV cache too small")
        if (n >= 128 and self.rows_prefill and c.hidden_size % 128 == 0 and c.fc_in % 64 == 0
                and (c.num_hidden_layers * 2 * c.kv_dim) % 128 == 0 and "kv_all" in self.w):
            return self._prefill_context_rows(cache, th.contiguous(), pos0)
        if (n > 16 and self.wide_prefill) or self.wide_hidden:
            return self._prefill_context_wide(cache, th, pos0)
        cos, sin = self._rope_tab(pos0 + n + 64)
        ops.set_dyn(cache.dyn, S, 0, 0, pos0)
        nkv2 = 2 * c.kv_dim
        for g0 in range(0, n, 16):
            rows = min(16, n - g0)
            self._ctx_rows(th[g0:g0 + rows], rows, None, None)
            for i, lw in enumerate(w["layers"]):
                kv_wp = lw["qkv"][c.q_dim * c.hidden_size:]
                ops.gemm_f32(kv_wp, ws["ctx_frag"], None, 1, nkv2, c.hidden_size, self.ks_kv, ws["part"])
                ops.qknorm_rope_append(qkv=ws["part"], nsplit=self.ks_kv, split_stride=16 * nkv2, ld=nkv2, q_col=-1,
                                       k_col=0, v_col=c.kv_dim, ctx_row0=0, blk_row0=-1,
                                       n_q=c.num_attention_heads, n_kv=c.num_key_value_heads, q_norm_w=lw["q_norm"],
                                       k_norm_w=lw["k_norm"], eps=c.rms_norm_eps, cos_tab=cos, sin_tab=sin,
                                       q_out=None, kcache=cache.k[i], vcache=cache.v[i], dyn=cache.dyn,
                                       ctx_rows_override=rows, row_base=g0)
        cache.length = S + n


    def raise_if_failed(self) -> None:
        if self.fuse_oproj and self._ws is not None and int(self._ws["sync"][ops.ATTN_OPROJ_FAIL_WORD]) != 0:
            self._ws["sync"].zero_()
            raise RuntimeError("dfl_attn_head_oproj: an o_proj workgroup gave up waiting for the attention stage")

    def draft_block(self, cache: DFlashKVCache, *, th_rows: Optional[torch.Tensor], tau: int, bs: int, pos0: int,
                    block_ids: Optional[torch.Tensor] = None, embed: Optional[torch.Tensor] = None,
                    noise: Optional[torch.Tensor] = None, append: bool = True, dyn_ready: bool = False,
                    s_bound: Optional[int] = None) -> list:
        c, ws, w = self.config, self._workspace(), self.w
        ww = self.w8 if self.streams_fp8(bs) else w
        if bs < 1 or bs > 32 or tau < 0 or tau > 16:
            raise ValueError(f"bs={bs} / tau={tau}: the kernels take 1..32 block rows and 0..16 context rows")
        head = self.attn_impl == "head"
        if bs > 16 and not head:
            raise ValueError("blocks of more than 16 rows need attn_impl='head'")
        ahead = s_bound is not None
        if ahead and not (dyn_ready and bs <= 16 and head and tau > 0 and noise is None):
            raise ValueError("s_bound needs dyn_ready, a block of <= 16 rows, context rows and the 'head' attention stage")
        S = int(s_bound) if ahead else cache.length
        if S + tau + bs > cache.max_rows:
            raise ValueError("draft KV cache too small")
        H, I = c.hidden_size, c.intermediate_size
        nqkv = c.q_dim + 2 * c.kv_dim
        cos, sin = self._rope_tab(pos0 + tau + bs + 64)
        src = self._src
        if not (dyn_ready and bs <= 16):
            ops.set_dyn2(cache.dyn, S, tau, bs, pos0)
        dyn = cache.dyn[:8]
        tiles = [(t, cache.dyn[8 * t:8 * t + 8]) for t in range((bs + 15) // 16)]
        if tau > 0:
            ops.gemm_resid(ww["fc"], ops.rows_plain(th_rows, ops.DYN_TAU), H, c.fc_in, ws["ctxh"], add_residual=False,
                           ss_out=ws["ss_ctx"], dyn=dyn)
        if head and tau > 0:
            ops.gemm_resid(ww["kv_all"], src["ctx"], c.num_hidden_layers * 2 * c.kv_dim, H, ws["xc"], add_residual=False,
                           dyn=dyn)
        L = w["layers"]
        if len(tiles) == 2 and self.wide_one_pass and head:
            return self._draft_block_wide(cache, ws, S, tau, bs, pos0, block_ids, embed, noise, append, cos, sin)
        if noise is not None:
            ws["h"][:bs].copy_(noise[:bs])
            ws["ss_emb"][:bs].copy_(noise[:bs].float().pow(2).sum(-1))
        else:
            for t, dt in tiles:
                ops.embed_rows(embed, block_ids[16 * t:], ws["h"][16 * t:], H, ws["ss_emb"][16 * t:], dt, ops.DYN_BS)
        hrow = [ws["h"][16 * t:16 * t + 16] for t in range(2)]
        fuse_o = self.fuse_oproj and head and len(tiles) == 1 and c.q_dim <= 4096
        for i, lw in enumerate(L):
            lm = ww["layers"][i]
            x1 = src["ln1_first"] if i == 0 else src["ln1"][i]
            if head:
                for t, dt in tiles:
                    ops.gemm_resid(lm["qkv"], x1[t], nqkv, H, ws["xq"][16 * t:], add_residual=False, dyn=dt)
                kw = dict(xq=ws["xq"], q_col=0, k_col=c.q_dim, v_col=c.q_dim + c.kv_dim,
                          xc=ws["xc"] if tau > 0 else None, ck_col=i * 2 * c.kv_dim,
                          cv_col=i * 2 * c.kv_dim + c.kv_dim, n_q=c.num_attention_heads,
                          n_kv=c.num_key_value_heads, q_norm_w=lw["q_norm"], k_norm_w=lw["k_norm"],
                          eps=c.rms_norm_eps, cos_tab=cos, sin_tab=sin, kcache=cache.k[i], vcache=cache.v[i],
                          scale=c.head_dim ** -0.5, causal=False, S=S, tau=tau, bs=bs, pos0=pos0,
                          ws=ws["head_ws"], max_splits=self.max_splits, dyn=dyn if ahead else None)
                if fuse_o:
                    ops.attn_head_oproj(**kw, attn_frag=ws["attn_frag"][0], wo=lw["o"], H=H, h_io=hrow[0],
                                        ss_out=ws["ss_h"][0], sync=ws["sync"])
                else:
                    ops.attn_head(**kw, out_frag=ws["attn_frag"], q_tiles=len(tiles),
                                  out_tile_stride=ws["attn_frag"].stride(0))
            else:
                ops.gemm_f32(lw["qkv"], src["ctx"], x1[0], 2, nqkv, H, self.ks_qkv, ws["part"], dyn)
                ops.attn_fused(qkv=ws["part"], nsplit=self.ks_qkv, split_stride=32 * nqkv, ld=nqkv, q_col=0,
                               k_col=c.q_dim, v_col=c.q_dim + c.kv_dim, ctx_row0=0, blk_row0=16,
                               n_q=c.num_attention_heads, n_kv=c.num_key_value_heads, q_norm_w=lw["q_norm"],
                               k_norm_w=lw["k_norm"], eps=c.rms_norm_eps, cos_tab=cos, sin_tab=sin, kcache=cache.k[i],
                               vcache=cache.v[i], dyn=dyn, scale=c.head_dim ** -0.5, kv_len_max=S + tau + bs,
                               ws=ws["attn_ws"], max_splits=self.max_splits, out_frag=ws["attn_frag"][0])
            for t, dt in tiles:
                if not fuse_o:
                    ops.gemm_resid(lm["o"], src["attn"][t], H, c.q_dim, hrow[t], add_residual=True, ss_out=ws["ss_h"][t],
                                   dyn=dt)
            for t, dt in tiles:
                ops.gemm_silu_mul(lm["gu"], src["ln2"][i][t], I, H, ws["act_frag"][t], dt)
            for t, dt in tiles:
                ops.gemm_resid(lm["down"], src["act"][t], H, I, hrow[t], add_residual=True, ss_out=ws["ss_h"][t],
                               dyn=dt)
        if append and not ahead:
            cache.length = S + tau
        return src["final"][:len(tiles)]

    def _draft_block_wide(self, cache, ws, S, tau, bs, pos0, block_ids, embed, noise, append, cos, sin) -> WideRows:
        c, w, R = self.config, self.w, 2
        H, I = c.hidden_size, c.intermediate_size
        nqkv = c.q_dim + 2 * c.kv_dim
        if self._wide is None:
            self._wide = TileStack(H=H, q_dim=c.q_dim, I=I, nqkv=nqkv, eps=c.rms_norm_eps, MT=2,
                                   gws=gemm_ws(H, (c.vocab_size, 2 * I, nqkv), (H, I, c.q_dim), self.device),
                                   h=ws["h"].view(2, 16, H), attn=ws["attn_frag"], act=ws["act_frag"],
                                   xq=ws["xq"].view(2, 16, nqkv))
            self._wide_ids = torch.zeros(2, 16, dtype=torch.int64, device=self.device)
        st = self._wide
        dyn2 = cache.dyn[:16].view(2, 8)
        if noise is not None:
            ws["h"][:bs].copy_(noise[:bs])
        else:
            self._wide_ids.view(-1)[:bs].copy_(block_ids[:bs])
            ops.embed_rows_batch(embed, self._wide_ids, R, st.h, H, ws["ss_emb"].view(2, 16), dyn2, ops.DYN_BS)

        def attend(i, lw):
            ops.attn_head(xq=ws["xq"], q_col=0, k_col=c.q_dim, v_col=c.q_dim + c.kv_dim,
                          xc=ws["xc"] if tau > 0 else None, ck_col=i * 2 * c.kv_dim, cv_col=i * 2 * c.kv_dim + c.kv_dim,
                          n_q=c.num_attention_heads, n_kv=c.num_key_value_heads, q_norm_w=lw["q_norm"],
                          k_norm_w=lw["k_norm"], eps=c.rms_norm_eps, cos_tab=cos, sin_tab=sin, kcache=cache.k[i],
                          vcache=cache.v[i], scale=c.head_dim ** -0.5, causal=False, S=S, tau=tau, bs=bs, pos0=pos0,
                          ws=ws["head_ws"], max_splits=self.max_splits, out_frag=ws["attn_frag"], q_tiles=2,
                          out_tile_stride=ws["attn_frag"].stride(0))

        st.run(self.tile_layers(qkv_parts=False), R, dyn2, attend, qkv="rows")
        st.finish(w["norm"])
        if append:
            cache.length = S + tau
        return WideRows(st.src["xn"], dyn2)

    def draft_tokens(self, hid_frag, lm_head_wp: torch.Tensor, bs: int, block_ids: torch.Tensor,
                     logits: Optional[torch.Tensor] = None, margins: Optional[torch.Tensor] = None,
                     sample: Optional[dict] = None) -> None:
        c, ws = self.config, self._workspace()
        if isinstance(hid_frag, WideRows):
            if margins is not None:
                raise NotImplementedError("top-2 margins are computed for blocks of <= 16 rows")
            gws, ids = self._wide.gws, self._wide_ids
            if sample is not None and isinstance(lm_head_wp, ops.Fp8Weight):
                raise ValueError("a sampled draft takes the bf16 lm_head")
            if sample is not None and logits is None:
                logits = torch.empty(32, c.vocab_size, dtype=BF16, device=self.device)
            ops.gemm_argmax_batch(lm_head_wp, hid_frag.src, 2, c.vocab_size, c.hidden_size, 0, 16, gws, ids, 0,
                                  hid_frag.dyn, nrows_dyn_word=ops.DYN_BS,
                                  logits=None if logits is None else logits.view(2, 16, c.vocab_size))
            if sample is not None:
                if sample.get("start") is None:
                    raise ValueError("a sampled draft of more than 16 rows needs the block start on the host")
                st = int(sample["start"])
                ops.sample_rows(logits.view(-1, c.vocab_size)[:bs], seed=sample["seed"], temperature=sample["temperature"],
                                pos0=st, stream=ops.RNG_DRAFT, extra=st, out=ids.view(-1)[:bs])
            block_ids[1:bs].copy_(ids.view(-1)[1:bs])
            return
        srcs = hid_frag if isinstance(hid_frag, (list, tuple)) else [hid_frag]
        for t, x in enumerate(srcs):
            row0 = 1 if t == 0 else 0
            nrows = min(bs - 16 * t, 16) - row0
            if nrows <= 0:
                continue
            if sample is not None:
                dyn = sample.get("dyn")
                if dyn is None and sample.get("start") is None:
                    raise ValueError("a sampled draft needs the block start: a length record or the host value")
                ops.gemm_sample(lm_head_wp, x, c.vocab_size, c.hidden_size, row0, nrows, ws["argmax_ws"], block_ids,
                                16 * t + row0, seed=sample["seed"], temperature=sample["temperature"], stream=ops.RNG_DRAFT,
                                pos_dyn=dyn, pos_word=ops.DYN_START, pos_base=int(sample.get("start") or 0),
                                pos_add=16 * t, logits=None if logits is None else logits[16 * t:16 * t + 16],
                                margins=margins)
                continue
            ev = self.lm_head_events if t == 0 else None
            if ev is not None and self.lm_head_events_log is not None:
                self.lm_head_events_log.append(ev)
            ops.gemm_argmax(lm_head_wp, x, c.vocab_size, c.hidden_size, row0, nrows, ws["argmax_ws"], block_ids,
                            16 * t + row0, logits=None if logits is None else logits[16 * t:16 * t + 16],
                            margins=margins, events=ev)

    @torch.inference_mode()
    def forward(self, position_ids: torch.LongTensor, attention_mask=None, noise_embedding=None, target_hidden=None,
                past_key_values: Optional[DFlashKVCache] = None, use_cache: bool = False, **kwargs) -> torch.Tensor:
        if self.w is None:
            raise RuntimeError("weights not loaded")
        if attention_mask is not None:
            raise NotImplementedError("the draft attends without a mask (is_causal=False, attention_mask=None)")
        c = self.config
        if noise_embedding.shape[0] != 1:
            raise NotImplementedError("batch = 1 by construction (SURVEY.md §1)")
        q_len, ctx = noise_embedding.shape[1], target_hidden.shape[1]
        pos0 = int(position_ids[0, 0])
        if position_ids.shape[1] != ctx + q_len:
            raise ValueError("position_ids must cover context + block rows")
        cache = past_key_values if past_key_values is not None else self.new_cache(ctx + q_len)
        if past_key_values is None:
            cache.length = 0
        th = target_hidden[0].to(BF16)
        head = max(0, ctx - 16) if ctx > 16 else 0
        if head:
            self.prefill_context(cache, th[:head], pos0)
        tau = ctx - head
        frag = self.draft_block(cache, th_rows=th[head:].contiguous() if tau else None, tau=tau, bs=q_len,
                                pos0=pos0 + head, noise=noise_embedding[0].to(BF16).contiguous())
        cache.length += q_len
        H, ws = c.hidden_size, self._workspace()
        out = []
        for t in range(len(frag)):
            ops.norm_pack(norm_w=self.w["norm"], frag=ws["xn_frag"][t], H=H, eps=c.rms_norm_eps,
                          resid_in=ws["h"][16 * t:16 * t + 16], dyn=cache.dyn[8 * t:8 * t + 8], dyn_word=ops.DYN_BS)
            out.append(ws["xn_frag"][t].view(H // 8, 16, 8).permute(1, 0, 2).reshape(16, H))
        return torch.cat(out)[:q_len].unsqueeze(0).clone()

    __call__ = forward

    @torch.inference_mode()
    def spec_generate(self, target, input_ids: torch.LongTensor, max_new_tokens: int, stop_token_ids,
                      temperature: float, draft_token_hook=None, sampler: str = "torch",
                      seed: Optional[int] = None, top_k: int = 0, top_p: float = 1.0) -> torch.LongTensor:
        from .generate import _generate_wide_hidden, run_decode
        if self.wide_hidden:
            return _generate_wide_hidden(self, target, input_ids, self.mask_token_id, max_new_tokens, self.block_size,
                                         stop_token_ids, temperature, draft_token_hook=draft_token_hook, sampler=sampler,
                                         seed=seed, top_k=top_k, top_p=top_p).output_ids
        r = run_decode(self, target, input_ids, mask_token_id=self.mask_token_id, max_new_tokens=max_new_tokens,
                       block_size=self.block_size, stop_token_ids=stop_token_ids, temperature=temperature,
                       clamp_tail=False, draft_token_hook=draft_token_hook, sampler=sampler, seed=seed, top_k=top_k,
                       top_p=top_p)
        return r.output_ids
```

### dflash_amd/ops.py

```python
from __future__ import annotations

from typing import NamedTuple, Optional

import torch

from ._lib import W_BF16, W_E4M3, Rows, Weight, check, lib

BF16, F32, I32, I64 = torch.bfloat16, torch.float32, torch.int32, torch.int64
DYN_S, DYN_TAU, DYN_BS, DYN_POS0, DYN_START, DYN_STOP, DYN_CYCLE = range(7)


def _stream() -> int:
    return torch.cuda.current_stream().cuda_stream


def _p(t: Optional[torch.Tensor], dtype=None, name="tensor") -> Optional[int]:
    if t is None:
        return None
    if not t.is_cuda:
        raise RuntimeError(f"dflash_amd: {name} must be a GPU tensor (got {t.device}); there is no CPU path")
    if dtype is not None and t.dtype != dtype:
        raise TypeError(f"dflash_amd: {name} must be {dtype}, got {t.dtype}")
    if not t.is_contiguous():
        raise ValueError(f"dflash_amd: {name} must be contiguous")
    return t.data_ptr()


def pack_weight(w: torch.Tensor) -> torch.Tensor:
    n, k = w.shape
    out = torch.empty(n * k, dtype=BF16, device=w.device)
    check(lib().dfl_pack_weight(_p(w, BF16, "w"), _p(out), n, k, _stream()), "dfl_pack_weight")
    return out


def pack_weight_gateup(gate: torch.Tensor, up: torch.Tensor) -> torch.Tensor:
    i, k = gate.shape
    assert up.shape == gate.shape
    out = torch.empty(2 * i * k, dtype=BF16, device=gate.device)
    check(lib().dfl_pack_weight_gateup(_p(gate, BF16, "gate"), _p(up, BF16, "up"), _p(out), i, k, _stream()),
          "dfl_pack_weight_gateup")
    return out


U8 = torch.uint8
FP8_MAX = 448.0


class Fp8Weight(NamedTuple):
    wp: torch.Tensor
    scale: torch.Tensor
    N: int
    K: int


_fp8_cast_on_device = {}


def fp8_cast_on_device(device) -> bool:
    device = torch.device(device)
    if device.type == "cpu":
        return True
    key = str(device)
    if key not in _fp8_cast_on_device:
        codes = torch.arange(256, dtype=U8)
        v = codes.view(torch.float8_e4m3fn).float()
        v = v[torch.isfinite(v)].sort().values
        probe = torch.cat([v, (v[1:] + v[:-1]) / 2])
        try:
            got = probe.to(device).to(torch.float8_e4m3fn).view(U8).cpu()
            ok = bool(torch.equal(got, probe.to(torch.float8_e4m3fn).view(U8)))
        except (RuntimeError, TypeError, NotImplementedError):
            ok = False
        _fp8_cast_on_device[key] = ok
    return _fp8_cast_on_device[key]


def quantize_fp8_rows(w: torch.Tensor):
    assert w.dim() == 2
    dev = w.device
    if not fp8_cast_on_device(dev):
        q, scale = quantize_fp8_rows(w.cpu())
        return q.to(dev), scale.to(dev)
    wf = w.detach().float()
    amax = wf.abs().amax(dim=1)
    m, e = torch.frexp(amax / FP8_MAX)
    e = torch.where(m == 0.5, e - 1, e)
    scale = torch.ldexp(torch.ones_like(amax), e)
    scale = torch.where(amax / scale > FP8_MAX, scale * 2, scale)
    scale = torch.where(amax == 0, torch.ones_like(scale), scale)
    x = (wf / scale[:, None]).clamp_(-FP8_MAX, FP8_MAX)
    q = x.to(torch.float8_e4m3fn).view(U8)
    return q.contiguous(), scale.contiguous()


def dequantize_fp8_rows(q: torch.Tensor, scale: torch.Tensor) -> torch.Tensor:
    return (q.view(torch.float8_e4m3fn).float() * scale[:, None].float()).to(BF16)


def pack_weight_fp8(q: torch.Tensor, scale: torch.Tensor) -> Fp8Weight:
    n, k = q.shape
    assert scale.numel() == n
    out = torch.empty(n * k, dtype=U8, device=q.device)
    check(lib().dfl_pack_weight_fp8(_p(q, U8, "q"), _p(out), n, k, _stream()), "dfl_pack_weight_fp8")
    return Fp8Weight(out, scale.to(device=q.device, dtype=F32).contiguous(), n, k)


def pack_weight_gateup_fp8(gate_q: torch.Tensor, gate_scale: torch.Tensor, up_q: torch.Tensor,
                           up_scale: torch.Tensor) -> Fp8Weight:
    i, k = gate_q.shape
    assert up_q.shape == gate_q.shape and gate_scale.numel() == i and up_scale.numel() == i
    out = torch.empty(2 * i * k, dtype=U8, device=gate_q.device)
    check(lib().dfl_pack_weight_gateup_fp8(_p(gate_q, U8, "gate_q"), _p(up_q, U8, "up_q"), _p(out), i, k, _stream()),
          "dfl_pack_weight_gateup_fp8")
    sc = torch.stack([gate_scale.to(F32).view(i // 16, 16), up_scale.to(F32).view(i // 16, 16)], dim=1)
    return Fp8Weight(out, sc.reshape(-1).to(gate_q.device).contiguous(), 2 * i, k)


class Fp8Experts(NamedTuple):
    wp: torch.Tensor
    scale: torch.Tensor
    E: int
    N: int
    K: int


def pack_experts_fp8(q: torch.Tensor, scale: torch.Tensor, gateup: bool) -> Fp8Experts:
    e, n, k = q.shape
    assert scale.shape == (e, n) and q.dtype == U8
    wp = torch.empty(e, n * k, dtype=U8, device=q.device)
    sc = torch.empty(e, n, dtype=F32, device=q.device)
    for j in range(e):
        if gateup:
            i = n // 2
            w8 = pack_weight_gateup_fp8(q[j, :i].contiguous(), scale[j, :i], q[j, i:].contiguous(), scale[j, i:])
        else:
            w8 = pack_weight_fp8(q[j].contiguous(), scale[j])
        wp[j].copy_(w8.wp)
        sc[j].copy_(w8.scale)
    return Fp8Experts(wp, sc, e, n, k)


def quantize_keep_fp8(m: torch.Tensor):
    q, sc = quantize_fp8_rows(m)
    return dequantize_fp8_rows(q, sc), (q, sc)


def pack_layer_fp8(l8: dict) -> dict:
    return {"qkv": pack_weight_fp8(torch.cat([l8[k][0] for k in "qkv"]), torch.cat([l8[k][1] for k in "qkv"])),
            "o": pack_weight_fp8(*l8["o"]), "gu": pack_weight_gateup_fp8(*l8["gate"], *l8["up"]),
            "down": pack_weight_fp8(*l8["down"])}


def tile_layers(layers: list, layers8: list, qkv_parts: bool, cache: dict) -> list:
    if qkv_parts not in cache:
        keys = ("gu", "o", "down") + (("qkv",) if qkv_parts else ())
        cache[qkv_parts] = [{**lw, **{k: l8[k] for k in keys}} for lw, l8 in zip(layers, layers8)]
    return cache[qkv_parts]


def _w(wp, N: int, K: int, name: str) -> Weight:
    if not isinstance(wp, Fp8Weight):
        return Weight(_p(wp, BF16, name), None, W_BF16)
    if (wp.N, wp.K) != (N, K):
        raise ValueError(f"dflash_amd: {name} is an fp8 weight of {wp.N} x {wp.K}, the launch asks for {N} x {K}")
    return Weight(_p(wp.wp, U8, name), _p(wp.scale, F32, name + ".scale"), W_E4M3)


def _we(wp, E: int, N: int, K: int, name: str):
    if not isinstance(wp, Fp8Experts):
        assert wp.dim() == 2 and wp.is_contiguous()
        return Weight(_p(wp, BF16, name), None, W_BF16), wp
    if (wp.E, wp.N, wp.K) != (E, N, K):
        raise ValueError(f"dflash_amd: {name} holds fp8 experts of {wp.E} x {wp.N} x {wp.K}, the launch asks for "
                         f"{E} x {N} x {K}")
    return Weight(_p(wp.wp, U8, name), _p(wp.scale, F32, name + ".scale"), W_E4M3), wp.wp


def set_dyn(dyn: torch.Tensor, S: int, tau: int, bs: int, pos0: int) -> None:
    check(lib().dfl_set_dyn(_p(dyn, I32, "dyn"), S, tau, bs, pos0, _stream()), "dfl_set_dyn")


def set_dyn2(dyn: torch.Tensor, S: int, tau: int, bs: int, pos0: int) -> None:
    assert dyn.numel() >= 16
    check(lib().dfl_set_dyn2(_p(dyn, I32, "dyn"), S, tau, bs, pos0, _stream()), "dfl_set_dyn2")


def pack_rows(x: torch.Tensor, rows: int, out_frag: torch.Tensor, dyn=None, dyn_word=0) -> None:
    assert x.dim() == 2 and x.stride(1) == 1 and x.dtype == BF16 and x.is_cuda
    k = x.shape[1]
    assert out_frag.numel() >= 16 * k
    check(lib().dfl_pack_rows(x.data_ptr(), x.stride(0), rows, k, _p(out_frag, BF16, "out_frag"),
                              _p(dyn, I32, "dyn"), dyn_word, _stream()), "dfl_pack_rows")


import ctypes as _C


class RowSource:

    def __init__(self, struct: Rows, *keep):
        self.struct, self.keep = struct, keep

    @property
    def ref(self):
        return _C.byref(self.struct)


def rows_frag(frag: torch.Tensor) -> RowSource:
    return RowSource(Rows(_p(frag, BF16, "frag"), None, 0, None, 0, None, 0.0, -1, 0), frag)


def _readable16(rows: torch.Tensor) -> torch.Tensor:
    need = (15 * rows.stride(0) + rows.shape[1]) * rows.element_size()
    have = rows.untyped_storage().nbytes() - rows.storage_offset() * rows.element_size()
    if rows.shape[0] >= 16 or have >= need:
        return rows
    pad = torch.zeros(16, rows.shape[1], dtype=rows.dtype, device=rows.device)
    pad[:rows.shape[0]] = rows
    return pad


def rows_plain(rows: torch.Tensor, valid_word: int = -1) -> RowSource:
    assert rows.is_cuda and rows.dtype == BF16 and rows.dim() == 2 and rows.stride(1) == 1
    rows = _readable16(rows)
    return RowSource(Rows(None, rows.data_ptr(), rows.stride(0), None, 0, None, 0.0, valid_word, 1), rows)


def rows_normed(rows: torch.Tensor, ss: torch.Tensor, nss: int, norm_w: torch.Tensor, eps: float,
                valid_word: int = -1) -> RowSource:
    assert rows.is_cuda and rows.dtype == BF16 and rows.dim() == 2 and rows.stride(1) == 1
    assert ss.numel() >= nss * 16
    rows = _readable16(rows)
    return RowSource(Rows(None, rows.data_ptr(), rows.stride(0), _p(ss, F32, "ss"), nss, _p(norm_w, BF16, "norm_w"),
                          eps, valid_word, 2), rows, ss, norm_w)


def _src(x) -> RowSource:
    return x if isinstance(x, RowSource) else rows_frag(x)


def gemm_f32(wp, x0, x1, mt: int, N: int, K: int, ksplit: int, out: torch.Tensor, dyn=None) -> None:
    assert out.numel() >= ksplit * mt * 16 * N
    s0, s1 = _src(x0), (_src(x1) if x1 is not None else None)
    check(lib().dfl_gemm_f32(_p(wp, BF16, "wp"), s0.ref, s1.ref if s1 is not None else None, mt, N, K, ksplit,
                             _p(out, F32, "out"), _p(dyn, I32, "dyn"), _stream()), "dfl_gemm_f32")


def min_ksplit(K: int, mt: int) -> int:
    per = 16 * (8 if mt == 1 else 4) * 32
    return (K + per - 1) // per


def pick_ksplit(N: int, K: int, mt: int) -> int:
    ntiles, ks_steps = N // 16, K // 32
    best, best_score = None, None
    for ks in range(min_ksplit(K, mt), 17):
        nfr = -(-ks_steps // (16 * ks))
        if nfr < 2 and ks > min_ksplit(K, mt):
            break
        gx_max = max(1, 256 // ks)
        per_wg = -(-ntiles // gx_max)
        fill = (ntiles * ks) / (256.0 * per_wg)
        score = (round(min(fill, 1.0), 3), min(per_wg, 2), -ks)
        if best_score is None or score > best_score:
            best, best_score = ks, score
    return best


def gemm_silu_mul(wp_gu, x, I: int, K: int, act_frag: torch.Tensor, dyn=None) -> None:
    assert act_frag.numel() >= 16 * I
    check(lib().dfl_gemm_silu_mul(_w(wp_gu, 2 * I, K, "wp_gu"), _src(x).ref, I, K, _p(act_frag, BF16, "act"),
                                  _p(dyn, I32, "dyn"), _stream()), "dfl_gemm_silu_mul")


def argmax_ws(device) -> torch.Tensor:
    return torch.empty(lib().dfl_argmax_ws_bytes(), dtype=torch.uint8, device=device)


def gemm_argmax(wp, x, V: int, K: int, row0: int, nrows: int, ws, out_ids: torch.Tensor, out_off: int = 0,
                dyn=None, nrows_dyn_word: int = -1, logits: Optional[torch.Tensor] = None,
                margins: Optional[torch.Tensor] = None, events=None) -> None:
    if logits is not None:
        assert logits.numel() >= 16 * V
    if margins is not None:
        assert margins.numel() >= out_off + nrows
    ev_start, ev_end = (None, None) if events is None else (events[0].cuda_event, events[1].cuda_event)
    check(lib().dfl_gemm_argmax(_w(wp, V, K, "wp"), _src(x).ref, V, K, row0, nrows, _p(dyn, I32, "dyn"), nrows_dyn_word,
                                _p(ws), _p(out_ids, I64, "out_ids"), out_off, _p(logits, BF16, "logits"),
                                _p(margins, F32, "margins"), ev_start, ev_end, _stream()), "dfl_gemm_argmax")


RNG_TARGET, RNG_DRAFT = 0, 1


def _seed64(seed: int) -> int:
    return int(seed) & 0xFFFFFFFFFFFFFFFF


def inv_temperature(temperature: float) -> float:
    import numpy as np
    return float(np.float32(1.0 / float(temperature)))


def gemm_sample(wp, x, V: int, K: int, row0: int, nrows: int, ws, out_ids: torch.Tensor, out_off: int = 0, *,
                seed: int, temperature: float, stream: int = RNG_TARGET, pos_dyn=None, pos_word: int = DYN_POS0,
                pos_base: int = 0, pos_add: int = 0, dyn=None, nrows_dyn_word: int = -1,
                logits: Optional[torch.Tensor] = None, margins: Optional[torch.Tensor] = None) -> None:
    if logits is not None:
        assert logits.numel() >= 16 * V
    if margins is not None:
        assert margins.numel() >= out_off + nrows
    check(lib().dfl_gemm_sample(_w(wp, V, K, "wp"), _src(x).ref, V, K, row0, nrows, _p(dyn, I32, "dyn"), nrows_dyn_word,
                                _p(ws), _p(out_ids, I64, "out_ids"), out_off, _p(logits, BF16, "logits"),
# ... 706 lines not shown
```

### dflash_amd/target.py

```python
from __future__ import annotations

from types import SimpleNamespace
from typing import Optional, Sequence

import torch

from . import ops
from .model import WEIGHT_FORMATS, _rope_tables
from .tile_stack import TileStack, gemm_ws
from .utils import sample

BF16 = torch.bfloat16


class TargetKVCache:

    def __init__(self, n_layers, n_kv, max_rows, device):
        self.max_rows = int(max_rows)
        self.k = torch.zeros(n_layers, n_kv, self.max_rows, 128, dtype=BF16, device=device)
        self.v = torch.zeros_like(self.k)
        self.dyn = torch.zeros(16, dtype=torch.int32, device=device)
        self.length = 0

    def get_seq_length(self, layer_idx: int = 0) -> int:
        return self.length

    def crop(self, max_length: int) -> None:
        if 0 < max_length < self.length:
            self.length = int(max_length)
        elif max_length < 0:
            self.length = max(0, self.length + int(max_length))


class _HiddenStates:

    def __init__(self, kept: dict, n: int):
        self._kept, self._n = kept, n

    def __len__(self):
        return self._n

    def __getitem__(self, i):
        if i < 0:
            i += self._n
        if i not in self._kept:
            raise KeyError(f"hidden state {i} was not kept by this prefill (tap_layers = {sorted(k - 1 for k in self._kept)})")
        return self._kept[i]


class _Weight:

    def __init__(self, w):
        self.weight = w


class NativeTarget:
    def __init__(self, hf_model, max_splits: int = 32, attn_impl: str = "head", keep_hf: bool = True,
                 prefill: str = "native", weight_format: str = "bf16", expert_format: str = "bf16"):
        if attn_impl not in ("head", "fused"):
            raise ValueError("attn_impl must be 'head' or 'fused'")
        if prefill not in ("native", "hf"):
            raise ValueError("prefill must be 'native' or 'hf'")
        self.attn_impl = attn_impl
        self.fuse_oproj = False
        self.wide_one_pass = True
        self._wide = None
        self._wide_seed = None
        self._nuc_logits = None
        self.moe_pair_kernel = True
        self.moe_shared_pass = True
        self.moe_shared_min = 2
        self._moe_sh = None
        cfg = hf_model.config
        self.check_config(cfg, weight_format, expert_format)
        self.weight_format = weight_format
        self.expert_format = expert_format
        fp8 = weight_format == "fp8_e4m3"
        e8 = expert_format == "fp8_e4m3"
        self.expert_stream = True
        self.experts8 = [] if e8 else None
        self.fp8_stream = True
        self.layers8 = [] if fp8 else None
        self.lm_wp8 = None
        self._tile_layers = {}
        self.hf = hf_model
        self.model = hf_model.model
        self.lm_head = hf_model.lm_head
        self.config = cfg
        dev = hf_model.lm_head.weight.device
        if dev.type != "cuda":
            raise RuntimeError("NativeTarget: the wrapped model must live on the GPU")
        self._dev = dev
        self.H = cfg.hidden_size
        self.L = cfg.num_hidden_layers
        self.n_q = cfg.num_attention_heads
        self.n_kv = getattr(cfg, "num_key_value_heads", self.n_q)
        self.hd = getattr(cfg, "head_dim", None) or self.H // self.n_q
        self.I = cfg.intermediate_size
        self.V = cfg.vocab_size
        self.eps = float(cfg.rms_norm_eps)
        rope = getattr(cfg, "rope_parameters", None) or {}
        rtype = rope.get("rope_type", "default") if isinstance(rope, dict) else "default"
        theta = (rope.get("rope_theta") if isinstance(rope, dict) else None) or getattr(cfg, "rope_theta", None)
        if self.hd != 128 or self.H % 32 or (self.I % 32 and not getattr(cfg, "num_experts", 0)) or self.V % 16:
            raise NotImplementedError("NativeTarget: needs head_dim 128, hidden %32, vocab %16")
        self.wide_hidden = self.H // 32 > 128
        if rtype not in ("default", "llama3", "linear", "yarn") or (rtype == "default" and theta is None):
            raise NotImplementedError(f"NativeTarget: rope_type {rtype!r} is not supported; keep the HF target")
        self.rope_type = rtype
        self.E = int(getattr(cfg, "num_experts", 0) or 0)
        if getattr(cfg, "num_local_experts", 0) and not self.E:
            raise NotImplementedError("NativeTarget: only the Qwen3-MoE expert layout is supported; keep the HF target")
        if self.E:
            self.top_k = int(cfg.num_experts_per_tok)
            self.Ie = int(cfg.moe_intermediate_size)
            self.norm_topk = bool(getattr(cfg, "norm_topk_prob", False))
            if self.E > 256 or self.top_k > 8 or self.Ie % 32:
                raise NotImplementedError("NativeTarget: MoE needs <= 256 experts, top-k <= 8, moe_intermediate_size % 32 == 0")
        if getattr(cfg, "attention_bias", False) or getattr(cfg, "mlp_bias", False):
            raise NotImplementedError("NativeTarget: biased projections are not supported")
        self.theta = float(theta) if theta is not None else None
        sd = hf_model.state_dict()

        def w(name):
            return sd[name].detach().to(device=dev, dtype=BF16).contiguous()

        def mat(name, store, key):
            m = w(name)
            if fp8:
                m, store[key] = ops.quantize_keep_fp8(m)
                with torch.no_grad():
                    sd[name].copy_(m)
            return m

        if fp8:
            h8 = {}
            mat("lm_head.weight", h8, "lm")
            self.lm_wp8 = ops.pack_weight_fp8(*h8.pop("lm"))
        self.layers = []
        for i in range(self.L):
            p = f"model.layers.{i}."
            l8 = {}
            qkv = torch.cat([mat(p + "self_attn.q_proj.weight", l8, "q"), mat(p + "self_attn.k_proj.weight", l8, "k"),
                             mat(p + "self_attn.v_proj.weight", l8, "v")], dim=0)
            has_qk = (p + "self_attn.q_norm.weight") in sd
            lw = {"qkv": ops.pack_weight(qkv), "o": ops.pack_weight(mat(p + "self_attn.o_proj.weight", l8, "o")),
                  "q_norm": w(p + "self_attn.q_norm.weight") if has_qk else None,
                  "k_norm": w(p + "self_attn.k_norm.weight") if has_qk else None,
                  "ln1": w(p + "input_layernorm.weight"), "ln2": w(p + "post_attention_layernorm.weight")}
            if (p + "mlp.experts.0.gate_proj.weight") in sd:
                raise NotImplementedError("NativeTarget: per-expert ModuleList MoE weights (mlp.experts.{e}.gate_proj) are "
                                          "not supported, only the fused gate_up_proj / down_proj tensors; keep the HF target")
            if (p + "mlp.experts.gate_up_proj") in sd:
                gup, dwn = w(p + "mlp.experts.gate_up_proj"), w(p + "mlp.experts.down_proj")
                Ie = self.Ie
                if gup.shape != (self.E, 2 * Ie, self.H) or dwn.shape != (self.E, self.H, Ie):
                    raise ValueError(f"layer {i}: unexpected expert tensor shapes {tuple(gup.shape)} {tuple(dwn.shape)}")
                if e8:
                    x8 = {}
                    for key, name, t in (("gu_e", "mlp.experts.gate_up_proj", gup), ("down_e", "mlp.experts.down_proj", dwn)):
                        q, sc = ops.quantize_fp8_rows(t.view(-1, t.shape[2]))
                        t.copy_(ops.dequantize_fp8_rows(q, sc).view_as(t))
                        with torch.no_grad():
                            sd[p + name].copy_(t)
                        x8[key] = ops.pack_experts_fp8(q.view(t.shape), sc.view(t.shape[:2]), gateup=key == "gu_e")
                        del q, sc
                    self.experts8.append(x8)
                    lw["gu_e8"], lw["down_e8"] = x8["gu_e"], x8["down_e"]
                lw["gu_e"] = torch.stack([ops.pack_weight_gateup(gup[e, :Ie].contiguous(), gup[e, Ie:].contiguous())
                                          for e in range(self.E)])
                lw["down_e"] = torch.stack([ops.pack_weight(dwn[e].contiguous()) for e in range(self.E)])
                ep = (self.E + 15) // 16 * 16
                rw = torch.zeros(ep, self.H, dtype=BF16, device=dev)
                rw[:self.E] = w(p + "mlp.gate.weight")
                lw["router"] = ops.pack_weight(rw)
                if ep % 128:
                    rp = torch.zeros((self.E + 127) // 128 * 128, self.H, dtype=BF16, device=dev)
                    rp[:self.E] = rw[:self.E]
                    lw["router_p"] = ops.pack_weight(rp)
                    del rp
                else:
                    lw["router_p"] = lw["router"]
                del gup, dwn, rw
            else:
                lw["gu"] = ops.pack_weight_gateup(mat(p + "mlp.gate_proj.weight", l8, "gate"),
                                                  mat(p + "mlp.up_proj.weight", l8, "up"))
                lw["down"] = ops.pack_weight(mat(p + "mlp.down_proj.weight", l8, "down"))
                if e8:
                    self.experts8.append(None)
            if fp8:
                if "gate" not in l8:
                    raise NotImplementedError("NativeTarget: fp8_e4m3 needs dense MLP layers")
                self.layers8.append(ops.pack_layer_fp8(l8))
            self.layers.append(lw)
            del qkv, l8
        self.norm = w("model.norm.weight")
        self.embed = w("model.embed_tokens.weight")
        self.lm_wp = None
        self.max_splits = max_splits
        self.q_dim, self.kv_dim = self.n_q * 128, self.n_kv * 128
        self.nqkv = self.q_dim + 2 * self.kv_dim
        self.ks_qkv = ops.pick_ksplit(self.nqkv, self.H, 1)
        self.ks_o = ops.pick_ksplit(self.H, self.q_dim, 1)
        self.ks_down = ops.pick_ksplit(self.H, self.I, 1)
        npart = max(self.ks_qkv * 16 * self.nqkv, self.ks_o * 16 * self.H, self.ks_down * 16 * self.H)
        z = lambda *s, dt=BF16: torch.zeros(*s, dtype=dt, device=dev)
        NT = 2
        self.ws = dict(attn=z(NT, 16 * self.q_dim), act=z(NT, 16 * self.I), h=z(16 * NT, self.H),
                       ss_emb=z(16 * NT, dt=torch.float32), ss_h=z(NT, self.H, dt=torch.float32),
                       q=z(self.n_q, 16, 128), part=z(npart, dt=torch.float32),
                       attn_ws=ops.attn_fused_ws(self.n_q, self.n_kv, max_splits, dev), argmax_ws=ops.argmax_ws(dev),
                       xq=z(16 * NT, self.nqkv), head_ws=ops.attn_head_ws(self.n_q, max_splits, NT, dev),
                       sync=torch.zeros(ops.ATTN_OPROJ_SYNC_WORDS, dtype=torch.int32, device=dev),
                       post=torch.zeros(16 * NT, dtype=torch.int64, device=dev))
        self.is_moe = any("gu_e" in lw for lw in self.layers)
        if self.is_moe:
            ep = (self.E + 15) // 16 * 16
            self.moe_nsplit = 2 if self.H % 32 else 4
            self.ws.update(xn=z(NT, 16 * self.H), xn1=z(NT, 16 * self.H), rlog=z(NT, 16, ep), wt=z(NT, 16, self.E),
                           act_e=z(self.E, 16 * self.Ie), moe_part=z(self.moe_nsplit, 16, self.H, dt=torch.float32),
                           active=torch.zeros(self.E, dtype=torch.int32, device=dev),
                           elist=torch.zeros(self.E, dtype=torch.int32, device=dev),
                           n_active=torch.zeros(1, dtype=torch.int32, device=dev),
                           rticket=torch.zeros(1, dtype=torch.int32, device=dev))
            self.moe_router_fused = self.H <= 4096 and self.E % 2 == 0
        ws, nt = self.ws, self.H // 16
        hs = [ws["h"][16 * t:16 * t + 16] for t in range(NT)]
        self.src = dict(
            ln1=[[ops.rows_normed(hs[t], ws["ss_emb"][16 * t:] if i == 0 else ws["ss_h"][t], 1 if i == 0 else nt,
                                  lw["ln1"], self.eps, ops.DYN_BS) for t in range(NT)]
                 for i, lw in enumerate(self.layers)],
            ln2=[[ops.rows_normed(hs[t], ws["ss_h"][t], nt, lw["ln2"], self.eps, ops.DYN_BS) for t in range(NT)]
                 for lw in self.layers],
            final=[ops.rows_normed(hs[t], ws["ss_h"][t], nt, self.norm, self.eps, ops.DYN_BS) for t in range(NT)],
            attn=[ops.rows_frag(ws["attn"][t]) for t in range(NT)], act=[ops.rows_frag(ws["act"][t]) for t in range(NT)])
        if self.is_moe:
            self.src["xn"] = [ops.rows_frag(ws["xn"][t]) for t in range(NT)]
            self.src["xn1"] = [ops.rows_frag(ws["xn1"][t]) for t in range(NT)]
        q_dim, kv_dim = self.n_q * 128, self.n_kv * 128
        self._pf = self._pf_moe = None
        dense_ok = all("gu_e" in lw for lw in self.layers) or self.I % 64 == 0
        self.native_prefill = (prefill == "native" and (q_dim + 2 * kv_dim) % 128 == 0 and self.H % 128 == 0 and dense_ok
                               and q_dim % 64 == 0 and (not self.is_moe or self.Ie % 64 == 0))
        self.prefill_attn = "native"
        self._rotary = getattr(hf_model.model, "rotary_emb", None)
        if not keep_hf:
            if not self.native_prefill:
                raise NotImplementedError("NativeTarget(keep_hf=False) needs the native prefill (widths % 128, FFN widths % 64)")
            if self.lm_wp is None:
                self.lm_wp = ops.pack_weight(self.lm_head.weight.detach().to(BF16).contiguous())
            self.hf = None
            self.model = SimpleNamespace(embed_tokens=_Weight(self.embed), rotary_emb=self._rotary)
            self.lm_head = _Weight(self.lm_head.weight.detach())
        self.debug_routing = None
        self.gu_events = None
        self.moe_events = None
        self._rope = None
        self._taps = {}
        torch.cuda.synchronize(dev)

    @staticmethod
    def check_config(cfg, weight_format: str = "bf16", expert_format: str = "bf16") -> None:
        if weight_format not in WEIGHT_FORMATS:
            raise ValueError(f"NativeTarget: weight_format must be one of {WEIGHT_FORMATS}, got {weight_format!r}")
        if expert_format not in WEIGHT_FORMATS:
            raise ValueError(f"NativeTarget: expert_format must be one of {WEIGHT_FORMATS}, got {expert_format!r}")
        n_q = cfg.num_attention_heads
        hd = getattr(cfg, "head_dim", None) or cfg.hidden_size // n_q
        if hd != 128:
            raise NotImplementedError(f"NativeTarget: the gfx950 kernels are built for head_dim == 128 (got {hd}); keep the HF target")
        if getattr(cfg, "attention_bias", False) or getattr(cfg, "mlp_bias", False):
            raise NotImplementedError("NativeTarget: biased projections are not supported; keep the HF target")
        lt = getattr(cfg, "layer_types", None) or ()
        if any(t == "sliding_attention" for t in lt) and getattr(cfg, "sliding_window", None):
            raise NotImplementedError("NativeTarget: sliding-window attention layers are not supported; keep the HF target")
        if weight_format == "fp8_e4m3":
            if getattr(cfg, "num_experts", 0) or getattr(cfg, "num_local_experts", 0):
                raise NotImplementedError("NativeTarget: fp8_e4m3 weights are not supported for sparse-MoE targets (the "
                                          "expert kernels have no e4m3 form); use weight_format='bf16'")
            widths = dict(hidden_size=cfg.hidden_size, intermediate_size=cfg.intermediate_size, q_width=n_q * hd)
            bad = {k: v for k, v in widths.items() if v % 64}
            if bad:
                raise NotImplementedError(f"NativeTarget: fp8_e4m3 weights need hidden, intermediate and q widths % 64 == 0 "
                                          f"(got {bad})")
        if expert_format == "fp8_e4m3":
            if not getattr(cfg, "num_experts", 0):
                raise NotImplementedError("NativeTarget: expert_format='fp8_e4m3' needs a sparse-MoE target (Qwen3-MoE expert "
                                          "layout); a dense target takes weight_format='fp8_e4m3'")
            widths = dict(hidden_size=cfg.hidden_size, moe_intermediate_size=getattr(cfg, "moe_intermediate_size", 0))
            bad = {k: v for k, v in widths.items() if not v or v % 64}
            if bad:
                raise NotImplementedError(f"NativeTarget: fp8_e4m3 experts need hidden and moe_intermediate widths % 64 == 0 "
                                          f"(got {bad})")

    @property
    def device(self):
        return self._dev

    def __call__(self, *a, **kw):
        if self.hf is None:
            raise RuntimeError("NativeTarget(keep_hf=False): the wrapped model is gone; use prefill() / verify()")
        return self.hf(*a, **kw)

    def share_lm_head(self, packed: torch.Tensor) -> None:
        self.lm_wp = packed

    def streams_fp8(self, bs: int = 16) -> bool:
        if self.layers8 is None or not self.fp8_stream or self.attn_impl != "head" or self.wide_hidden:
            return False
        return (not self.fuse_oproj) if bs <= 16 else self.wide_one_pass

    def streams_fp8_tiles(self) -> bool:
        return (self.layers8 is not None and self.fp8_stream and self.attn_impl == "head"
                and min(self.H, self.I, self.q_dim) >= 256)

    def tile_layers(self, qkv_parts: bool) -> list:
        if not self.streams_fp8_tiles():
            return self.layers
        return ops.tile_layers(self.layers, self.layers8, qkv_parts, self._tile_layers)

    def fp8_tensors(self) -> tuple:
        ws = []
        if self.layers8 is not None:
            ws += [w8 for l8 in self.layers8 for w8 in l8.values()] + [self.lm_wp8]
        if self.experts8 is not None:
            ws += [x8 for l8 in self.experts8 if l8 is not None for x8 in l8.values()]
        return tuple(t for w8 in ws for t in (w8.wp, w8.scale))

    def expert_weights(self, lw: dict) -> tuple:
        if "gu_e8" not in lw or not self.expert_stream:
            return lw["gu_e"], lw["down_e"]
        return (lw["gu_e8"] if (self.H <= 2048 and self.moe_pair_kernel) else lw["gu_e"]), lw["down_e8"]

    def tile_head(self):
        return self.lm_wp8 if self.streams_fp8_tiles() else self.lm_wp

    def new_cache(self, max_rows: Optional[int] = None) -> TargetKVCache:
        if max_rows is None:
            raise ValueError("NativeTarget.new_cache needs max_rows (prompt + new tokens + block)")
        return TargetKVCache(self.L, self.n_kv, max_rows, self._dev)

    def _rope_tab(self, need: int):
        if self._rope is None or self._rope[0].shape[0] < need:
            n = 1 << (max(need, 4096) - 1).bit_length()
            if self.rope_type == "default":
                self._rope = _rope_tables(128, self.theta, n, self._dev)
            else:
                pos = torch.arange(n, device=self._dev).unsqueeze(0)
                cos, sin = self._rotary(torch.zeros(1, dtype=BF16, device=self._dev), pos)
                self._rope = (cos[0, :, :64].to(BF16).contiguous(), sin[0, :, :64].to(BF16).contiguous())
        return self._rope

    @torch.inference_mode()
    def prefill(self, input_ids: torch.Tensor, cache: TargetKVCache, output_hidden_states: bool = True,
                tap_layers: Optional[Sequence[int]] = None):
        P = input_ids.shape[1]
        if P > cache.max_rows:
            raise ValueError("target KV cache too small for the prompt")
        if self.native_prefill:
            return self._prefill_native(input_ids, cache, output_hidden_states, tap_layers)
        return self._prefill_hf(input_ids, cache, output_hidden_states)

    def _prefill_native(self, input_ids, cache, output_hidden_states, tap_layers):
        import torch.nn.functional as F
        P = input_ids.shape[1]
        H, I, dev = self.H, self.I, self._dev
        Pp = ops.prefill_rows_padded(P)
        q_dim, kv_dim, nqkv = self.q_dim, self.kv_dim, self.nqkv
        if self._pf is None or self._pf["h"].shape[0] < Pp:
            z = lambda *s: torch.zeros(*s, dtype=BF16, device=dev)
            dense_I = I if any("gu" in lw for lw in self.layers) else 0
            self._pf = dict(h=z(Pp, H), xf=z(Pp * max(H, q_dim)), qkv=z(Pp, nqkv), act=z(Pp * max(dense_I, 1)), attn=z(Pp, q_dim),
                            logits=z(16, self.V), ids=torch.zeros(16, dtype=torch.int64, device=dev))
        pf = self._pf
        h, xf, qkv, act, attn = pf["h"], pf["xf"], pf["qkv"], pf["act"], pf["attn"]
        h.zero_()
        torch.index_select(self.embed, 0, input_ids[0], out=h[:P])
        cos, sin = self._rope_tab(P + 64)
        want = None
        if output_hidden_states:
            want = set(range(self.L + 1)) if tap_layers is None else {int(l) + 1 for l in tap_layers}
            if max(want) >= self.L and tap_layers is not None:
                raise NotImplementedError("tapping the last layer (post-norm state) is not supported")
        kept = {}
        if want and 0 in want:
            kept[0] = h[:P].clone().unsqueeze(0)
        for i, lw in enumerate(self.layers):
            ops.prefill_norm_pack(h, P, H, lw["ln1"], self.eps, xf)
            ops.prefill_gemm_rows(lw["qkv"], xf, P, nqkv, H, qkv)
            ops.prefill_qk_rope(qkv, P, 0, q_dim, q_dim + kv_dim, self.n_q, self.n_kv, lw["q_norm"], lw["k_norm"], self.eps,
                                cos, sin, 0, cache.k[i], cache.v[i], 0)
            if self.prefill_attn == "native":
                ops.prefill_attn(qkv, P, 0, cache.k[i], cache.v[i], self.n_q, self.n_kv, 128 ** -0.5, xf)
            else:
                q = qkv[:P, :q_dim].view(P, self.n_q, 128).transpose(0, 1).unsqueeze(0)
                o = F.scaled_dot_product_attention(q, cache.k[i][:, :P].unsqueeze(0), cache.v[i][:, :P].unsqueeze(0),
                                                   is_causal=True, scale=128 ** -0.5, enable_gqa=self.n_kv != self.n_q)
                attn[:P].view(P, self.n_q, 128).copy_(o[0].transpose(0, 1))
                ops.prefill_norm_pack(attn, P, q_dim, None, self.eps, xf)
            ops.prefill_gemm_resid(lw["o"], xf, P, H, q_dim, h)
            ops.prefill_norm_pack(h, P, H, lw["ln2"], self.eps, xf)
            tap = None
            if want and (i + 1) in want and i + 1 < self.L:
                tap = torch.empty(P, H, dtype=BF16, device=dev)
                kept[i + 1] = tap.unsqueeze(0)
            if "gu_e" in lw:
                if self._pf_moe is None or self._pf_moe["P"] < P:
                    self._pf_moe = ops.prefill_moe_scratch(P, H, self.Ie, self.E, self.top_k,
                                                           (self.E + 127) // 128 * 128, dev)
                ops.prefill_moe_mlp(lw["router_p"], lw["gu_e"], lw["down_e"], xf, P, H, self.Ie, self.E, self.top_k,
                                    self.norm_topk, h, self._pf_moe, tap=tap)
                if self.debug_routing is not None:
                    self.debug_routing.append((i, self._pf_moe["pair_e"][:P, :self.top_k].clone()))
                continue
            ops.prefill_gemm_silu(lw["gu"], xf, P, I, H, act)
            ops.prefill_gemm_resid(lw["down"], act, P, H, I, h, tap=tap)
        if self.lm_wp is None:
            self.lm_wp = ops.pack_weight(self.lm_head.weight.detach().to(BF16).contiguous())
        t0 = (P - 1) // 16 * 16
        rows = h[t0:t0 + 16]
        if self.wide_hidden:
            if "wxn" not in pf:
                pf["wxn"] = torch.zeros(2, 16 * H, dtype=BF16, device=dev)
                pf["wdyn"] = torch.tensor([[0, 0, 16, 0, 0, 0, 0, 0]] * 2, dtype=torch.int32, device=dev)
                pf["wgws"] = torch.zeros(ops.lib().dfl_gemm_batch_ws_bytes(self.V, H), dtype=torch.uint8, device=dev)
                pf["wh"] = torch.zeros(2, 16, H, dtype=BF16, device=dev)
                pf["wlogits"], pf["wids"] = torch.zeros(2, 16, self.V, dtype=BF16, device=dev), torch.zeros(2, 16, dtype=torch.int64, device=dev)
            pf["wh"][0].copy_(rows)
            ops.norm_frag_batch(pf["wh"], 1, self.norm, self.eps, pf["wxn"], pf["wdyn"], ops.DYN_BS)
            ops.gemm_argmax_batch(self.lm_wp, ops.brows_frag(pf["wxn"]), 1, self.V, H, 0, 16, pf["wgws"], pf["wids"], 0,
                                  pf["wdyn"], nrows_dyn_word=ops.DYN_BS, logits=pf["wlogits"])
            pf["logits"].copy_(pf["wlogits"][0])
        else:
            ss = rows.float().pow(2).sum(-1).contiguous()
            ops.gemm_argmax(self.lm_wp, ops.rows_normed(rows, ss, 1, self.norm, self.eps), self.V, H, 0, 16,
                            self.ws["argmax_ws"], pf["ids"], 0, logits=pf["logits"])
        logits = pf["logits"][P - 1 - t0].clone().view(1, 1, self.V)
        cache.length = P
        return SimpleNamespace(logits=logits, hidden_states=_HiddenStates(kept, self.L + 1) if output_hidden_states else None)

    def _prefill_hf(self, input_ids, cache, output_hidden_states):
        from transformers import DynamicCache
        P = input_ids.shape[1]
        tmp = DynamicCache()
        pos = torch.arange(P, device=self._dev).unsqueeze(0)
        out = self.hf(input_ids, position_ids=pos, past_key_values=tmp, use_cache=True, logits_to_keep=1,
                      output_hidden_states=output_hidden_states)
        for i in range(self.L):
            cache.k[i, :, :P].copy_(tmp.layers[i].keys[0])
            cache.v[i, :, :P].copy_(tmp.layers[i].values[0])
        cache.length = P
        return out

    def _moe_mlp(self, i: int, lw: dict, tiles, hrow, taps, sl) -> None:
        ws, H, E = self.ws, self.H, self.E
        nxt = self.layers[i + 1]["ln1"] if i + 1 < self.L else self.norm
        gu_e, down_e = self.expert_weights(lw)
        for t, dt in tiles:
# ... 48 lines not shown
                               dyn_word=ops.DYN_BS)
            else:
                ops.gemm_resid(lw["router"], ops.rows_frag(x), w["rlog"].shape[2], H, w["rlog"][0], add_residual=False, dyn=dt)
                ops.moe_route(w["rlog"][0], self.E, self.top_k, self.norm_topk, w["wt"][0], w["active"], w["elist"],
                              w["n_active"], dyn=dt, dyn_word=ops.DYN_BS)
            if H <= 2048 and self.moe_pair_kernel:
                ops.moe_gate_up(gu_e, x, self.E, self.Ie, H, w["act_e"], w["elist"], w["n_active"], dyn=dt,
                                valid_word=ops.DYN_BS)
            else:
                ops.gemm_silu_mul_experts(lw["gu_e"], ops.rows_frag(x), self.E, self.Ie, H, w["act_e"], w["elist"],
                                          w["n_active"], dyn=dt)
            ops.moe_down(down_e, w["act_e"], w["wt"][0], w["elist"], w["n_active"], self.E, H, self.Ie, ns,
                         w["moe_part"])
            pv[:, r * 16:(r + 1) * 16].copy_(w["moe_part"])
        return ns

    def _moe_mlp_shared(self, lw: dict, R: int, MT: int, dyn: torch.Tensor, xn: torch.Tensor, part: torch.Tensor) -> int:
        H, P = self.H, R * 16
        if self._moe_sh is None:
            ep = (self.E + 127) // 128 * 128
            self._moe_sh = dict(sc=ops.prefill_moe_scratch(4 * 16, H, self.Ie, self.E, self.top_k, ep, self._dev),
                                rlog=torch.zeros(4, 16, ep, dtype=BF16, device=self._dev),
                                gws=torch.zeros(ops.lib().dfl_gemm_batch_ws_bytes(ep, H), dtype=torch.uint8, device=self._dev))
        sh = self._moe_sh
        sc, L, st = sh["sc"], ops.lib(), ops._stream()
        ops.gemm_resid_batch(lw["router_p"], ops.brows_frag(xn), R, sh["rlog"].shape[2], H, sh["rlog"], add_residual=False,
                             ws=sh["gws"], dyn=dyn)
        ops.prefill_moe_route(sh["rlog"].view(64, -1), P, sc, self.norm_topk)
        e8 = "gu_e8" in lw and self.expert_stream
        ops.moe_grouped_gate_up(lw["gu_e8"] if e8 else lw["gu_e"], xn, sc, H, gather=True)
        ops.moe_grouped_down(lw["down_e8"] if e8 else lw["down_e"], sc, H)
        ops.check(L.dfl_prefill_moe_combine(sc["out32"].data_ptr(), sc["posmap"].data_ptr(), P, H, self.top_k, None, 0, None, 0,
                                            part.data_ptr(), st), "dfl_prefill_moe_combine")
        return 1

    def _nucleus_logits(self) -> torch.Tensor:
        if self._nuc_logits is None:
            self._nuc_logits = torch.zeros(32, self.V, dtype=BF16, device=self._dev)
        return self._nuc_logits

    def _verify_wide(self, block_ids, start, cache, bs, tap_layers, taps, logits_out, temperature, cos, sin, seed=None,
                     flt=None):
        ws, H, R = self.ws, self.H, 2
        if self._wide is None:
            self._wide = TileStack(H=H, q_dim=self.q_dim, I=self.I, nqkv=self.nqkv, eps=self.eps, MT=2,
                                   gws=gemm_ws(H, (self.V, 2 * self.I, self.nqkv), (H, self.I, self.q_dim), self._dev),
                                   h=ws["h"].view(2, 16, H), attn=ws["attn"], act=ws["act"],
                                   xq=ws["xq"].view(2, 16, self.nqkv), moe_nsplit=self.moe_nsplit if self.is_moe else 0)
            self._wide_ids = torch.zeros(2, 16, dtype=torch.int64, device=self._dev)
        st = self._wide
        s, gws = st.src, st.gws
        dyn2 = cache.dyn[:16].view(2, 8)
        self._wide_ids.view(-1)[:bs].copy_(block_ids[:bs])
        ops.embed_rows_batch(self.embed, self._wide_ids, R, st.h, H, ws["ss_emb"].view(2, 16), dyn2, ops.DYN_BS)

        def attend(i, lw):
            ops.attn_head(xq=ws["xq"], q_col=0, k_col=self.q_dim, v_col=self.q_dim + self.kv_dim, n_q=self.n_q,
                          n_kv=self.n_kv, q_norm_w=lw["q_norm"], k_norm_w=lw["k_norm"], eps=self.eps, cos_tab=cos,
                          sin_tab=sin, kcache=cache.k[i], vcache=cache.v[i], scale=128 ** -0.5, causal=True, S=start,
                          tau=0, bs=bs, pos0=start, ws=ws["head_ws"], max_splits=self.max_splits, out_frag=ws["attn"],
                          q_tiles=2, out_tile_stride=ws["attn"].stride(0))

        st.run(self.tile_layers(qkv_parts=False), R, dyn2, attend, qkv="rows",
               taps=None if taps is None else taps.view(2, 16, -1), tap_layers=tap_layers, moe=self.moe_mlp_tiles)
        st.finish(self.norm)
        post = ws["post"]
        if flt is None and temperature >= 1e-5 and seed is not None and self.streams_fp8_tiles():
            ops.set_dyn2(cache.dyn, start, 0, bs, start)
            if self._wide_seed is None:
                self._wide_seed = torch.zeros(1, dtype=torch.int64, device=self._dev)
            self._wide_seed.fill_(ops.seed_i64(seed))
            ops.gemm_sample_batch(self.lm_wp8, s["xn"], R, self.V, H, 0, 16, gws, post.view(2, 16), 0, dyn2,
                                  seeds=self._wide_seed, temperature=temperature, pos_word=ops.DYN_POS0, pos_add=1,
                                  tiles_per_req=2, nrows_dyn_word=ops.DYN_BS,
                                  logits=None if logits_out is None else logits_out.view(2, 16, self.V))
            cache.length = start + bs
            return post[:bs].unsqueeze(0), taps
        logits = logits_out
        if flt is not None and logits is None:
            logits = self._nucleus_logits()
        elif temperature >= 1e-5:
            logits = torch.empty(32, self.V, dtype=BF16, device=self._dev)
        lv = None if logits is None else logits.view(2, 16, self.V)
        ops.gemm_argmax_batch(self.tile_head(), s["xn"], R, self.V, H, 0, 16, gws, post.view(2, 16), 0, dyn2,
                              nrows_dyn_word=ops.DYN_BS, logits=lv)
        if flt is not None:
            ops.sample_rows_nucleus(logits.view(2, 16, self.V), seed=seed, temperature=temperature, dyn=dyn2,
                                    nrows_dyn_word=ops.DYN_BS, pos_base=start, pos_add=1, tiles_per_req=2,
                                    out=post.view(2, 16), **flt)
            posterior = post[:bs].unsqueeze(0)
        elif temperature >= 1e-5 and seed is not None:
            ops.sample_rows(logits[:bs], seed=seed, temperature=temperature, pos0=start + 1, out=post[:bs])
            posterior = post[:bs].unsqueeze(0)
        else:
            posterior = post[:bs].unsqueeze(0) if temperature < 1e-5 else sample(logits[:bs].unsqueeze(0), temperature)
        cache.length = start + bs
        return posterior, taps

    def raise_if_failed(self) -> None:
        if self.fuse_oproj and int(self.ws["sync"][ops.ATTN_OPROJ_FAIL_WORD]) != 0:
            self.ws["sync"].zero_()
            raise RuntimeError("dfl_attn_head_oproj: an o_proj workgroup gave up waiting for the attention stage")

    @torch.inference_mode()
    def verify(self, block_ids: torch.Tensor, start: int, cache: TargetKVCache, *, tap_layers: Sequence[int] = (),
               temperature: float = 0.0, logits_out: Optional[torch.Tensor] = None,
               taps_out: Optional[torch.Tensor] = None, dyn_lengths: bool = False, seed: Optional[int] = None,
               top_k: int = 0, top_p: float = 1.0):
        bs = block_ids.numel()
        flt = None
        if ops.check_filter(top_k, top_p) and temperature >= 1e-5:
            if seed is None:
                raise ValueError("top_k / top_p at temperature > 0 need the seeded draw (seed=...)")
            flt = dict(top_k=int(top_k), top_p=float(top_p))
        if self.wide_hidden:
            raise NotImplementedError("NativeTarget.verify: hidden > 4096 runs through the ragged-batch path "
                                      "(dflash_generate / dflash_generate_batch / BatchedDecoder)")
        if bs < 1 or bs > 32:
            raise ValueError("verify takes 1..32 block rows")
        if bs > 16 and self.attn_impl != "head":
            raise ValueError("blocks of more than 16 rows need attn_impl='head'")
        if start + bs > cache.max_rows:
            raise ValueError("target KV cache too small")
        ws, H = self.ws, self.H
        if self.lm_wp is None:
            self.lm_wp = ops.pack_weight(self.lm_head.weight.detach().to(BF16).contiguous())
        cos, sin = self._rope_tab(start + bs + 64)
        if dyn_lengths:
            if bs > 16 or self.attn_impl != "head" or self.fuse_oproj:
                raise ValueError("dyn_lengths needs a block of <= 16 rows and the plain 'head' attention stage")
        elif self.attn_impl != "head" or getattr(cache, "_dyn_bs", None) != bs:
            ops.set_dyn2(cache.dyn, start, 0, bs, start)
            cache._dyn_bs = bs
        dyn = cache.dyn[:8]
        tiles = [(t, cache.dyn[8 * t:8 * t + 8]) for t in range((bs + 15) // 16)]
        taps = None
        tap_layers = list(tap_layers)
        if tap_layers:
            if max(tap_layers) >= self.L - 1:
                raise NotImplementedError("tapping the last layer (post-norm state) is not supported")
            key = len(tap_layers)
            if taps_out is not None:
                if taps_out.shape != (32, key * H) or taps_out.dtype != BF16 or not taps_out.is_contiguous():
                    raise ValueError("taps_out must be a contiguous bf16 [32, len(tap_layers)*H] tensor")
                taps = taps_out
            else:
                if key not in self._taps:
                    self._taps[key] = torch.zeros(32, key * H, dtype=BF16, device=self._dev)
                taps = self._taps[key]
        Ls, src = self.layers, self.src
        w8 = self.streams_fp8(bs)
        Lm = self.layers8 if w8 else Ls
        head = self.lm_wp8 if w8 else self.lm_wp
        if len(tiles) == 2 and self.wide_one_pass and self.attn_impl == "head":
            return self._verify_wide(block_ids, start, cache, bs, tap_layers, taps, logits_out, temperature, cos, sin, seed,
                                     flt)
        hrow = [ws["h"][16 * t:16 * t + 16] for t in range(2)]
        for t, dt in tiles:
            ops.embed_rows(self.embed, block_ids[16 * t:], hrow[t], H, ws["ss_emb"][16 * t:], dt, ops.DYN_BS)
        fuse_o = self.fuse_oproj and self.attn_impl == "head" and len(tiles) == 1 and self.q_dim <= 4096
        prev_moe = False
        for i, lw in enumerate(Ls):
            lm = Lm[i]
            x1 = src["xn1"] if prev_moe else src["ln1"][i]
            if self.attn_impl == "head":
                for t, dt in tiles:
                    ops.gemm_resid(lm["qkv"], x1[t], self.nqkv, H, ws["xq"][16 * t:], add_residual=False, dyn=dt)
                kw = dict(xq=ws["xq"], q_col=0, k_col=self.q_dim, v_col=self.q_dim + self.kv_dim, n_q=self.n_q,
                          n_kv=self.n_kv, q_norm_w=lw["q_norm"], k_norm_w=lw["k_norm"], eps=self.eps, cos_tab=cos,
                          sin_tab=sin, kcache=cache.k[i], vcache=cache.v[i], scale=128 ** -0.5, causal=True,
                          S=start, tau=0, bs=bs, pos0=start, ws=ws["head_ws"], max_splits=self.max_splits,
                          dyn=dyn if dyn_lengths else None)
                if fuse_o:
                    ops.attn_head_oproj(**kw, attn_frag=ws["attn"][0], wo=lw["o"], H=H, h_io=hrow[0],
                                        ss_out=ws["ss_h"][0], sync=ws["sync"])
                else:
                    ops.attn_head(**kw, out_frag=ws["attn"], q_tiles=len(tiles), out_tile_stride=ws["attn"].stride(0))
            else:
                ops.gemm_f32(lw["qkv"], x1[0], None, 1, self.nqkv, H, self.ks_qkv, ws["part"], dyn)
                ops.attn_fused(qkv=ws["part"], nsplit=self.ks_qkv, split_stride=16 * self.nqkv, ld=self.nqkv, q_col=0,
                               k_col=self.q_dim, v_col=self.q_dim + self.kv_dim, ctx_row0=0, blk_row0=0, n_q=self.n_q,
                               n_kv=self.n_kv, q_norm_w=lw["q_norm"], k_norm_w=lw["k_norm"], eps=self.eps,
                               cos_tab=cos, sin_tab=sin, kcache=cache.k[i], vcache=cache.v[i], dyn=dyn,
                               scale=128 ** -0.5, kv_len_max=start + bs, ws=ws["attn_ws"],
                               max_splits=self.max_splits, out_frag=ws["attn"][0], causal=True)
            for t, dt in tiles:
                if not fuse_o:
                    ops.gemm_resid(lm["o"], src["attn"][t], H, self.q_dim, hrow[t], add_residual=True,
                                   ss_out=None if "gu_e" in lw else ws["ss_h"][t], dyn=dt)
            sl = [j for j, l in enumerate(tap_layers) if l == i]
            prev_moe = "gu_e" in lw
            if prev_moe:
                self._moe_mlp(i, lw, tiles, hrow, taps, sl)
            else:
                gev = self.gu_events if (self.gu_events is not None and self.gu_events[0] == i) else None
                if gev is not None:
                    gev[1].record()
                for t, dt in tiles:
                    ops.gemm_silu_mul(lm["gu"], src["ln2"][i][t], self.I, H, ws["act"][t], dt)
                if gev is not None:
                    gev[2].record()
                for t, dt in tiles:
                    tap = taps[16 * t:16 * t + 16, sl[0] * H:(sl[0] + 1) * H] if sl else None
                    ops.gemm_resid(lm["down"], src["act"][t], H, self.I, hrow[t], add_residual=True,
                                   ss_out=ws["ss_h"][t], tap=tap, dyn=dt)
            for j in sl[1:]:
                taps[:, j * H:(j + 1) * H].copy_(taps[:, sl[0] * H:(sl[0] + 1) * H])
        post = ws["post"]
        logits = logits_out
        fin = src["xn1"] if prev_moe else src["final"]
        if flt is not None:
            if logits is None:
                logits = self._nucleus_logits()
            for t, dt in tiles:
                n = min(16, bs - 16 * t)
                ops.gemm_argmax(head, fin[t], self.V, H, 0, n, ws["argmax_ws"], post, 16 * t, dyn=dt,
                                logits=logits[16 * t:16 * t + 16])
                ops.sample_rows_nucleus(logits[16 * t:16 * t + 16], seed=seed, temperature=temperature, nrows=n, dyn=dt,
                                        pos_word=ops.DYN_POS0 if dyn_lengths else -1, pos_base=start, pos_add=16 * t + 1,
                                        out=post[16 * t:16 * t + 16], **flt)
            cache.length = start + bs
            return post[:bs].unsqueeze(0), taps
        if temperature >= 1e-5 and seed is not None:
            for t, dt in tiles:
                ops.gemm_sample(head, fin[t], self.V, H, 0, min(16, bs - 16 * t), ws["argmax_ws"], post, 16 * t,
                                seed=seed, temperature=temperature, pos_dyn=dt if dyn_lengths else None,
                                pos_word=ops.DYN_POS0, pos_base=start, pos_add=16 * t + 1, dyn=dt,
                                logits=None if logits is None else logits[16 * t:16 * t + 16])
            cache.length = start + bs
            return post[:bs].unsqueeze(0), taps
        if temperature >= 1e-5:
            logits = torch.empty(16 * len(tiles), self.V, dtype=BF16, device=self._dev)
        for t, dt in tiles:
            ops.gemm_argmax(head, fin[t], self.V, H, 0, min(16, bs - 16 * t), ws["argmax_ws"], post, 16 * t,
                            dyn=dt, logits=None if logits is None else logits[16 * t:16 * t + 16])
        if temperature < 1e-5:
            posterior = post[:bs].unsqueeze(0)
        else:
            posterior = sample(logits[:bs].unsqueeze(0), temperature)
        cache.length = start + bs
        return posterior, taps
```

### include/dflash_hip.h

```cpp
#ifndef DFLASH_HIP_H
#define DFLASH_HIP_H

#include <stdint.h>

#ifdef __cplusplus
extern "C" {
#endif

#define DFL_ABI_VERSION 1

#define DFL_OK 0
#define DFL_EINVAL (-22)
#define DFL_ELAUNCH (-5)

#define DFL_DYN_WORDS 8
#define DFL_DYN_S 0
#define DFL_DYN_TAU 1
#define DFL_DYN_BS 2
#define DFL_DYN_POS0 3
#define DFL_DYN_START 4
#define DFL_DYN_STOP 5
#define DFL_DYN_CYCLE 6

typedef struct dfl_rows {
  const void *frag;
  const void *rows;
  int64_t ld;
  const float *ss;
  int32_t nss;
  const void *norm_w;
  float eps;
  int32_t valid_word;
  int32_t mode;
} dfl_rows;

enum { DFL_W_BF16 = 0, DFL_W_E4M3 = 1 };
typedef struct dfl_weight {
  const void *wp;
  const float *scale;
  int32_t format;
} dfl_weight;

int dfl_version(void);
const char *dfl_last_error(void);


int dfl_pack_weight(const void *w, void *wp, int N, int K, void *stream);
int dfl_pack_weight_gateup(const void *gate, const void *up, void *wp, int I, int K, void *stream);
int dfl_pack_weight_fp8(const void *q, void *wp8, int N, int K, void *stream);
int dfl_pack_weight_gateup_fp8(const void *gate_q, const void *up_q, void *wp8, int I, int K, void *stream);


int dfl_set_dyn(int32_t *dyn, int S, int tau, int bs, int pos0, void *stream);
int dfl_set_dyn2(int32_t *dyn, int S, int tau, int bs, int pos0, void *stream);

int dfl_pack_rows(const void *x, int64_t ldx, int rows, int K, void *xf, const int32_t *dyn, int dyn_word,
                  void *stream);

int dfl_gemm_f32(const void *wp, const dfl_rows *x0, const dfl_rows *x1, int mt, int N, int K, int ksplit, float *out,
                 const int32_t *dyn, void *stream);

int dfl_gemm_silu_mul(const dfl_weight *w_gateup, const dfl_rows *x, int I, int K, void *act_frag, const int32_t *dyn,
                      void *stream);

int64_t dfl_argmax_ws_bytes(void);
int dfl_gemm_argmax(const dfl_weight *w, const dfl_rows *x, int V, int K, int row0, int nrows, const int32_t *dyn,
                    int nrows_dyn_word, void *ws, int64_t *out_ids, int out_off, void *logits, float *margin_out,
                    void *ev_start, void *ev_end, void *stream);

int dfl_gemm_sample(const dfl_weight *w, const dfl_rows *x, int V, int K, int row0, int nrows, const int32_t *dyn,
                    int nrows_dyn_word, void *ws, int64_t *out_ids, int out_off, void *logits, float *margin_out,
                    uint64_t seed, float inv_t, int rng_stream, const int32_t *pos_dyn, int pos_word, int pos_base,
                    int pos_add, void *stream);

int dfl_gemm_resid(const dfl_weight *w, const dfl_rows *x, int N, int K, void *h_io, int64_t ldh, int add_residual,
                   void *tap, int64_t ldtap, float *ss_out, const int32_t *dyn, void *stream);

int dfl_embed_rows(const void *embed, const int64_t *ids, void *h_out, int H, float *ss_out, const int32_t *dyn,
                   int dyn_word, void *stream);

int dfl_norm_pack(const float *part, int nsplit, int64_t part_split, int ldp, int row_off, const void *resid_in,
                  const void *embed, const int64_t *ids, void *h_out, void *h_out2, int64_t ld2, const void *norm_w,
                  float eps, void *frag, int H, const int32_t *dyn, int dyn_word, void *stream);

int dfl_qknorm_rope_append(const float *qkv, int nsplit, int64_t split_stride, int ld, int q_col, int k_col,
                           int v_col, int ctx_row0, int blk_row0, int n_q, int n_kv, const void *q_norm_w,
                           const void *k_norm_w, float eps, const void *cos_tab, const void *sin_tab, int max_pos,
                           void *q_out, void *kcache, void *vcache, int cache_rows, const int32_t *dyn,
                           int ctx_rows_override, int row_base, void *stream);

int64_t dfl_attn_ws_bytes(int n_q, int max_splits);
int dfl_block_attn(const void *q, const void *kcache, const void *vcache, int cache_rows, int n_q, int n_kv,
                   float scale, int causal, const int32_t *dyn, int kv_len_max, void *ws, int max_splits,
                   void *out_frag, void *stream);

int64_t dfl_attn_fused_ws_bytes(int n_q, int n_kv, int max_splits);
int dfl_attn_fused(const float *qkv, int nsplit, int64_t split_stride, int ld, int q_col, int k_col, int v_col,
                   int ctx_row0, int blk_row0, int n_q, int n_kv, const void *q_norm_w, const void *k_norm_w,
                   float eps, const void *cos_tab, const void *sin_tab, int max_pos, void *kcache, void *vcache,
                   int cache_rows, float scale, int causal, const int32_t *dyn, int kv_len_max, void *ws,
                   int max_splits, void *out_frag, void *stream);

int64_t dfl_attn_head_ws_bytes(int n_q, int max_splits, int q_tiles);
int dfl_attn_head(const void *xq, int64_t ldq, int q_col, int k_col, int v_col, const void *xc, int64_t ldc,
                  int ck_col, int cv_col, int n_q, int n_kv, const void *q_norm_w, const void *k_norm_w, float eps,
                  const void *cos_tab, const void *sin_tab, int max_pos, void *kcache, void *vcache, int cache_rows,
                  float scale, int causal, const int32_t *dyn, int S, int tau, int bs, int pos0, int q_tiles,
                  void *ws, int max_splits, void *out_frag, int64_t out_tile_stride, void *stream);

#define DFL_ATTN_OPROJ_SYNC_WORDS 1056
int dfl_attn_head_oproj(const void *xq, int64_t ldq, int q_col, int k_col, int v_col, const void *xc, int64_t ldc,
                        int ck_col, int cv_col, int n_q, int n_kv, const void *q_norm_w, const void *k_norm_w, float eps,
                        const void *cos_tab, const void *sin_tab, int max_pos, void *kcache, void *vcache,
                        int cache_rows, float scale, int causal, const int32_t *dyn, int S, int tau, int bs, int pos0,
                        void *ws, int max_splits, void *attn_frag, const void *wo_packed, int H, void *h_io,
                        int64_t ldh, float *ss_out, int32_t *sync, void *stream);

int dfl_attn_head_cand(const void *xq, int64_t ldq, int q_col, int k_col, int v_col, int n_cand, int64_t xq_cand_stride,
                       int n_q, int n_kv, const void *q_norm_w, const void *k_norm_w, float eps, const void *cos_tab,
                       const void *sin_tab, int max_pos, const void *kcache, const void *vcache, int cache_rows,
                       float scale, int S, int bs, void *ws, int max_splits, void *out_frag, int64_t out_cand_stride,
                       int64_t out_tile_stride, int q_tiles, void *k_out, void *v_out, int64_t kv_out_cand_stride,
                       int out_rows, void *stream);

int dfl_attn_head_batch(const void *xq, int64_t ldq, int q_col, int k_col, int v_col, int R, int64_t xq_req_stride, int n_q,
                        int n_kv, const void *q_norm_w, const void *k_norm_w, float eps, const void *cos_tab,
                        const void *sin_tab, int max_pos, void *kcache, void *vcache, int cache_rows,
                        int64_t cache_req_stride, float scale, int causal, const int32_t *dyn, int kv_len_max, void *ws,
                        int max_splits, void *out_frag, int64_t out_req_stride, int64_t out_tile_stride, int q_tiles,
                        void *stream);
int dfl_attn_head_batch_f32(const float *xq_parts, int nparts, int64_t part_stride, int64_t ldq, int q_col, int k_col,
                            int v_col, int R, int64_t xq_req_stride, int n_q, int n_kv, const void *q_norm_w,
                            const void *k_norm_w, float eps, const void *cos_tab, const void *sin_tab, int max_pos,
                            void *kcache, void *vcache, int cache_rows, int64_t cache_req_stride, float scale, int causal,
                            const int32_t *dyn, int kv_len_max, void *ws, int max_splits, void *out_frag,
                            int64_t out_req_stride, void *stream);

int dfl_topk_rows(const void *logits, int64_t ld, int rows, int V, int k, float *out_val, int32_t *out_idx, float *out_lse,
                  void *stream);

int dfl_candidate_select(const int64_t *blocks, int64_t blk_stride, const int64_t *posterior, int64_t post_stride,
                         const float *scores, int n_cand, int bs, int64_t *output_ids, int64_t output_len, int32_t *dyn,
                         const int64_t *stop_ids, int n_stop, int32_t *result, void *stream);

int dfl_moe_route(const void *logits, int ld, int E, int top_k, int norm_topk, void *wt, int32_t *active, int32_t *list,
                  int32_t *n_active, const int32_t *dyn, int dyn_word, void *stream);
int dfl_moe_router(const void *h, int64_t ldh, const void *norm_w, float eps, void *xn_frag, const void *wp_router, int K,
                   int E, int top_k, int norm_topk, void *rlog, int ld, void *wt, int32_t *active, int32_t *list,
                   int32_t *n_active, const int32_t *dyn, int dyn_word, int32_t *ticket, void *stream);
int dfl_gemm_silu_mul_experts(const void *wp_gateup, int64_t wp_expert_stride, const dfl_rows *x, int E, int I, int K,
                              void *act_frag, int64_t act_expert_stride, const int32_t *list, const int32_t *n_active,
                              const int32_t *dyn, void *stream);
int dfl_moe_gate_up(const dfl_weight *w_gateup, const void *x_frag, int E, int I, int K, void *act_frag, const int32_t *list,
                    const int32_t *n_active, const int32_t *dyn, int valid_word, void *stream);
int dfl_moe_down(const dfl_weight *w_down, int64_t wp_expert_stride, const void *act_frag, int64_t act_expert_stride,
                 const void *wt, const int32_t *list, const int32_t *n_active, int E, int N, int I, int nsplit, float *out,
                 void *stream);

int dfl_argmax(const void *logits, int dtype, int rows, int64_t V, int64_t *ids, void *stream);

int dfl_sample_rows(const void *logits, int64_t ld, int rows, int V, uint64_t seed, float inv_t, int rng_stream, int pos0,
                    const int32_t *pos, int extra, int64_t *out_ids, float *margin_out, void *stream);

int dfl_sample_rows_nucleus(const void *logits, int64_t ld, int64_t tile_stride, int tiles, int V, int row0, int nrows,
                            const int32_t *dyn, int nrows_dyn_word, int pos_word, int pos_base, const int32_t *positions,
                            int pos_add, int tiles_per_req, const int64_t *seeds, uint64_t seed, const int32_t *top_k_dev,
                            int top_k, const float *top_p_dev, float top_p, const float *inv_t_dev, float inv_t,
                            int rng_stream, int extra, int64_t *out_ids, int64_t out_stride, int out_off, float *thr_out,
                            int32_t *kept_out, void *stream);

int dfl_accept_commit(const int64_t *block_ids, const int64_t *posterior, int bs, int64_t *output_ids,
                      int64_t output_len, int32_t *dyn, const int64_t *stop_ids, int n_stop, int32_t *result,
                      int64_t *next_block, int rearm_n, int64_t mask_id, int32_t *dyn_t, void *stream);

int64_t dfl_prefill_rows_padded(int P);

int dfl_prefill_gemm_rows(const void *wp, const void *x_frag, int P, int N, int K, void *out, int64_t ldo, void *stream);

int dfl_prefill_gemm_resid(const void *wp, const void *x_frag, int P, int N, int K, void *h_io, int64_t ldh, void *tap,
                           int64_t ldtap, void *stream);

int dfl_prefill_gemm_silu(const void *wp_gateup, const void *x_frag, int P, int I, int K, void *act_frag, void *stream);

int dfl_prefill_norm_pack(const void *h, int64_t ldh, int P, int H, const void *norm_w, float eps, void *x_frag,
                          void *stream);
int dfl_prefill_pack_rows(const void *rows, int64_t ld, int P, int K, void *x_frag, void *stream);

int dfl_prefill_qk_rope(void *qkv_rows, int64_t ld, int P, int q_col, int k_col, int v_col, int n_q, int n_kv,
                        const void *q_norm_w, const void *k_norm_w, float eps, const void *cos_tab, const void *sin_tab,
// ... 91 lines not shown
```

Before: 1732.

## Stream gate-up and lm_head weights in a lossless 13-bit packed bf16 format

Adds a BF16X13 weight format. Each bf16 value becomes 8 low bits, a 4-bit exponent offset from a per-tile base, and a sign bit, with one patch word per tile for a single outlier. The GEMM kernels decode this in registers before the MFMA. The aim is to cut the HBM bytes streamed by the memory-bound skinny gate-up and greedy lm_head GEMMs. The cost is extra ALU decode work, an extra packed twin of those weights in memory, and a fallback to plain bf16 for tiles with more than one outlier.

```diff
diff --git a/dflash_amd/_lib.py b/dflash_amd/_lib.py
--- a/dflash_amd/_lib.py
+++ b/dflash_amd/_lib.py
@@ -26,7 +26,7 @@
 
 _rb = C.POINTER(RowsBatch)
 
-W_BF16, W_E4M3 = 0, 1
+W_BF16, W_E4M3, W_BF16X13 = 0, 1, 2
 
 
 class Weight(C.Structure):
diff --git a/dflash_amd/csrc/gemm_rows.h b/dflash_amd/csrc/gemm_rows.h
--- a/dflash_amd/csrc/gemm_rows.h
+++ b/dflash_amd/csrc/gemm_rows.h
@@ -55,6 +55,69 @@
     return wr[f];
 }
 
+typedef uint32_t u32x2 __attribute__((ext_vector_type(2)));
+typedef unsigned short u16x2 __attribute__((ext_vector_type(2)));
+#define W13_QUAD_BYTES 3328
+struct W13Extra {
+  uint32_t sg[2];
+  u32x2 meta;
+};
+
+template <int AUX = 2>
+__device__ __forceinline__ void load_quads_w13(bf16x8 (&wr)[6], uint32_t (&sg)[2], const char *first, int nq, int l,
+                                               int half = -1) {
+  const __amdgpu_buffer_rsrc_t r =
+      __builtin_amdgcn_make_buffer_rsrc(const_cast<char *>(first), 0, (nq < 0 ? 0 : nq) * W13_QUAD_BYTES, 0x00020000);
+  const bool mine = half < 0 || ((l >> 3) & 1) == half;
+  const int voff = mine ? l * 16 : 0x40000000, voff4 = mine ? l * 4 : 0x40000000;
+#pragma unroll
+  for (int q = 0; q < 2; ++q) sg[q] = __builtin_amdgcn_raw_buffer_load_b32(r, voff4 + 3072, q * W13_QUAD_BYTES, AUX);
+#pragma unroll
+  for (int q = 0; q < 2; ++q) {
+#pragma unroll
+    for (int p = 2; p < 5; ++p)
+      wr[3 * q + p % 3] =
+          __builtin_bit_cast(bf16x8, __builtin_amdgcn_raw_buffer_load_b128(r, voff + (p % 3) * 1024, q * W13_QUAD_BYTES, AUX));
+  }
+}
+
+__device__ __forceinline__ u32x2 w13_meta(const u32x2 *meta, int t, int w) {
+  typedef const __attribute__((address_space(4))) u32x2 *cptr;
+  return *(cptr)(uintptr_t)(meta + (size_t)__builtin_amdgcn_readfirstlane(t) * 16 + w);
+}
+
+__device__ __forceinline__ uint32_t w13_high(uint32_t c, uint32_t sgw, int r, u16x2 hb2) {
+  const uint32_t nz = ((c + 0x0f0f0f0fu) >> 4) & 0x01010101u;
+  const u16x2 e = __builtin_bit_cast(u16x2, nz) * hb2 + __builtin_bit_cast(u16x2, c);
+  return __builtin_bit_cast(uint32_t, e) | ((sgw << (7 - r)) & 0x80808080u);
+}
+
+__device__ __forceinline__ bf16x8 w13_frag(const bf16x8 (&wr)[6], const W13Extra &ex, int f, int l) {
+  const int q = f >> 2, ff = f & 3;
+  const u32x4 lw = __builtin_bit_cast(u32x4, wr[3 * q + (ff >> 1)]);
+  const uint32_t la = (ff & 1) ? lw[2] : lw[0], lb = (ff & 1) ? lw[3] : lw[1];
+  const uint32_t n = __builtin_bit_cast(u32x4, wr[3 * q + 2])[ff];
+  const uint32_t hb = __builtin_amdgcn_readfirstlane(ex.meta[0]) & 0x7f, pw = __builtin_amdgcn_readfirstlane(ex.meta[1]);
+  const u16x2 hb2 = {(unsigned short)hb, (unsigned short)hb};
+  const uint32_t ha = w13_high(n & 0x0f0f0f0fu, ex.sg[q], 2 * ff, hb2);
+  const uint32_t hh = w13_high((n >> 4) & 0x0f0f0f0fu, ex.sg[q], 2 * ff + 1, hb2);
+  u32x4 o;
+  o[0] = __builtin_amdgcn_perm(ha, la, 0x05010400u);
+  o[1] = __builtin_amdgcn_perm(ha, la, 0x07030602u);
+  o[2] = __builtin_amdgcn_perm(hh, lb, 0x05010400u);
+  o[3] = __builtin_amdgcn_perm(hh, lb, 0x07030602u);
+  if ((pw >> 28) == (8u | (uint32_t)f)) {
+    const int pl = (pw >> 22) & 63, el = (pw >> 19) & 7;
+    const uint32_t raw = pw & 0xffffu;
+#pragma unroll
+    for (int d = 0; d < 4; ++d) {
+      const uint32_t nd = (el & 1) ? (o[d] & 0xffffu) | (raw << 16) : (o[d] & 0xffff0000u) | raw;
+      o[d] = (l == pl && (el >> 1) == d) ? nd : o[d];
+    }
+  }
+  return __builtin_bit_cast(bf16x8, o);
+}
+
 typedef float f32x16 __attribute__((ext_vector_type(16)));
 __device__ __forceinline__ f32x16 tile_scales(const float *wscale, int t) {
   typedef const __attribute__((address_space(4))) f32x16 *cptr;
diff --git a/dflash_amd/csrc/gemm_skinny.hip b/dflash_amd/csrc/gemm_skinny.hip
--- a/dflash_amd/csrc/gemm_skinny.hip
+++ b/dflash_amd/csrc/gemm_skinny.hip
@@ -136,11 +136,12 @@
 
 constexpr int gemm_fr(int MT, bool CHUNKED) { return CHUNKED ? 4 : (MT == 1 ? 8 : 4); }
 
-template <int MT, bool CHUNKED, int EPI, bool NORM, bool W8 = false>
+template <int MT, bool CHUNKED, int EPI, bool NORM, bool W8 = false, bool W13 = false>
 __device__ __forceinline__ void gemm_body(const GemmArgs &a, const SampleArgs &sa) {
   GSTAMP(0);
+  static_assert(!W13 || (MT == 1 && !CHUNKED && !W8), "W13: the single-tile, single-pass bf16 kernels only");
   constexpr int FR = gemm_fr(MT, CHUNKED);
-  constexpr int NW = W8 ? FR / 2 : FR;
+  constexpr int NW = W13 ? 6 : (W8 ? FR / 2 : FR);
   __shared__ float red[2][16][MT][256];
   __shared__ float ssred[NORM ? MT : 1][16][16];
   __shared__ bf16x8 nwl[NORM ? MT : 1][NORM ? 512 : 1];
@@ -171,6 +172,7 @@
 
   bf16x8 wA[NW], wB[NW];
   float scA = 1.f, scB = 1.f;
+  W13Extra exA{}, exB{};
   bf16x8 xA[MT][FR], xB[MT][FR];
   bf16x8 xr[MT][FR];
 
@@ -220,8 +222,17 @@
       sc = a.wscale[(size_t)t * 16 + (tid & 15)];
     }
   };
-  auto load_item = [&](bf16x8(&wr)[NW], float &sc, bf16x8(&xb)[MT][FR], int t, int c, int half) {
-    if constexpr (W8)
+  auto load_w13 = [&](bf16x8(&wr)[NW], W13Extra &ex, int t, int ks0, int nf, int half) {
+    if constexpr (W13) {
+      const char *base = reinterpret_cast<const char *>(a.wp);
+      load_quads_w13(wr, ex.sg, base + ((size_t)t * (a.KS >> 2) + (ks0 >> 2)) * W13_QUAD_BYTES, nf >> 2, l, half);
+      ex.meta = w13_meta(reinterpret_cast<const u32x2 *>(a.wscale), nf > 0 ? t : 0, w);
+    }
+  };
+  auto load_item = [&](bf16x8(&wr)[NW], float &sc, W13Extra &ex, bf16x8(&xb)[MT][FR], int t, int c, int half) {
+    if constexpr (W13)
+      load_w13(wr, ex, t, ks0_of(c), nf_of(c), half);
+    else if constexpr (W8)
       load_w8(wr, sc, t, ks0_of(c), nf_of(c), half);
     else
       load_ksteps<FR>(wr, a.wp + ((size_t)t * a.KS + ks0_of(c)) * 64, nf_of(c), l, half);
@@ -292,7 +303,7 @@
     }
   };
 
-  auto process = [&](bf16x8(&wr)[NW], float wsc, bf16x8(&xb)[MT][FR], int t, int c, int pos) {
+  auto process = [&](bf16x8(&wr)[NW], float wsc, const W13Extra &ex, bf16x8(&xb)[MT][FR], int t, int c, int pos) {
     if (!CHUNKED || c == 0) {
 #pragma unroll
       for (int mt = 0; mt < MT; ++mt) acc[mt] = (f32x4){0.f, 0.f, 0.f, 0.f};
@@ -307,7 +318,12 @@
           const bool keep = ks0c + f < a.KS && (a.src[mt].mode == 0 || (l & 15) < nv[mt]);
           xv = keep ? xb[mt][f] : (bf16x8){0, 0, 0, 0, 0, 0, 0, 0};
         }
-        acc[mt] = __builtin_amdgcn_mfma_f32_16x16x32_bf16(weight_frag<W8>(wr, f), xv, acc[mt], 0, 0, 0);
+        bf16x8 wf;
+        if constexpr (W13)
+          wf = w13_frag(wr, ex, f, l);
+        else
+          wf = weight_frag<W8>(wr, f);
+        acc[mt] = __builtin_amdgcn_mfma_f32_16x16x32_bf16(wf, xv, acc[mt], 0, 0, 0);
       }
     if (!CHUNKED || c == a.nch - 1) finish(t, pos, wsc);
   };
@@ -380,7 +396,9 @@
       __builtin_amdgcn_s_barrier();
       __builtin_amdgcn_sched_barrier(0);
     }
-    if constexpr (W8)
+    if constexpr (W13)
+      load_w13(wA, exA, SILU ? 2 * (int)blockIdx.x : first_tile, ks0_of(0), first_live ? nf0 : 0, first_half);
+    else if constexpr (W8)
       load_w8(wA, scA, SILU ? 2 * (int)blockIdx.x : first_tile, ks0_of(0), first_live ? nf0 : 0, first_half);
     else if (!moe)
       load_ksteps<FR>(wA, a.wp + ((size_t)(SILU ? 2 * blockIdx.x : first_tile) * a.KS + ks0_of(0)) * 64,
@@ -428,6 +446,8 @@
   } else {
     if constexpr (W8)
       load_w8(wA, scA, first_tile, ks0_of(0), first_live ? nf0 : 0, first_half);
+    else if constexpr (W13)
+      ;
     else if (nitems > 0 || !moe)
       load_ksteps<FR>(wA, a.wp + ((size_t)first_tile * a.KS + ks0_of(0)) * 64, first_live ? nf0 : 0, l, first_half);
     GSTAMP(6);
@@ -447,8 +467,8 @@
         cn = 0;
         ++jn;
       }
-      if (i + 1 < nitems) load_item(wB, scB, xB, tile_of(jn), cn, half_of(jn));
-      process(wA, scA, xA, tile_of(j), c, j);
+      if (i + 1 < nitems) load_item(wB, scB, exB, xB, tile_of(jn), cn, half_of(jn));
+      process(wA, scA, exA, xA, tile_of(j), c, j);
       if (i == 0) GSTAMP(4);
       if (i + 1 >= nitems) break;
       int j2 = jn, c2 = cn + 1;
@@ -456,8 +476,8 @@
         c2 = 0;
         ++j2;
       }
-      if (i + 2 < nitems) load_item(wA, scA, xA, tile_of(j2), c2, half_of(j2));
-      process(wB, scB, xB, tile_of(jn), cn, jn);
+      if (i + 2 < nitems) load_item(wA, scA, exA, xA, tile_of(j2), c2, half_of(j2));
+      process(wB, scB, exB, xB, tile_of(jn), cn, jn);
       if (i + 2 >= nitems) break;
       j = j2;
       c = c2;
@@ -497,6 +517,11 @@
   gemm_body<1, CHUNKED, EPI, NORM, true>(with_head<CHUNKED, NORM>(rest, GEMM_HEAD_NAMES), SampleArgs{});
 }
 
+template <int EPI, bool NORM>
+__global__ __launch_bounds__(1024) void k_gemm_w13(GEMM_HEAD_PARAMS, GemmArgs rest) {
+  gemm_body<1, false, EPI, NORM, false, true>(with_head<false, NORM>(rest, GEMM_HEAD_NAMES), SampleArgs{});
+}
+
 template <bool NORM>
 __global__ __launch_bounds__(1024) void k_gemm_s(GEMM_HEAD_PARAMS, GemmArgs rest, SampleArgs sa) {
   gemm_body<1, false, EPI_SAMPLE, NORM>(with_head<false, NORM>(rest, GEMM_HEAD_NAMES), sa);
@@ -537,6 +562,30 @@
     }
   }
   hipLaunchKernelGGL((k_gemm<MT, CHUNKED, EPI, false>), grid, dim3(1024), 0, stream, GEMM_HEAD_OF(h), a);
+  return true;
+}
+
+static int64_t w13_quads_bytes(int N, int K) { return (int64_t)(N / 16) * (K / 128) * W13_QUAD_BYTES; }
+
+template <int EPI>
+bool launch_gemm_w13(const char *who, GemmArgs &a, const dfl_weight *w, int N, dim3 grid, hipStream_t stream) {
+  if (w->scale) {
+    dfl_set_error("%s: a DFL_W_BF16X13 weight takes no scale vector (the bases and patch words follow the codes)", who);
+    return false;
+  }
+  if (a.KS % 64 || a.nfr % 4 || a.nfr * 16 != a.KS) {
+    dfl_set_error("%s: DFL_W_BF16X13 covers K = 2048 and K = 4096 only (whole quads of four k-steps per wave; K=%d, %d k-steps "
+                  "per wave)", who, a.KS * 32, a.nfr);
+    return false;
+  }
+  a.wscale = reinterpret_cast<const float *>(reinterpret_cast<const char *>(w->wp) + w13_quads_bytes(N, a.KS * 32));
+  a.gx = (int)grid.x;
+  GemmHead h;
+  if (!gemm_head<false>(h, a)) return false;
+  if (a.src[0].mode == 2)
+    hipLaunchKernelGGL((k_gemm_w13<EPI, true>), grid, dim3(1024), 0, stream, GEMM_HEAD_OF(h), a);
+  else
+    hipLaunchKernelGGL((k_gemm_w13<EPI, false>), grid, dim3(1024), 0, stream, GEMM_HEAD_OF(h), a);
   return true;
 }
 
@@ -740,7 +789,7 @@
 }
 
 namespace {
-template <bool W8>
+template <bool W8, bool W13 = false>
 int gemm_silu_mul_impl(const char *who, const dfl_weight *w, const dfl_rows *x, int I, int K, void *act_frag,
                        const int32_t *dyn, void *stream) {
   DFL_REQUIRE(w->wp && act_frag && (!W8 || w->scale), "%s: null pointer", who);
@@ -758,7 +807,11 @@
   if (W8) a.nfr += a.nfr & 1;
   a.nch = 1;
   a.act = (bf16_t *)act_frag;
-  if (!launch_gemm<1, false, EPI_SILU, W8>(a, dim3(grid_x_for(I / 16), 1), (hipStream_t)stream)) return DFL_EINVAL;
+  if constexpr (W13) {
+    if (!launch_gemm_w13<EPI_SILU>(who, a, w, 2 * I, dim3(grid_x_for(I / 16), 1), (hipStream_t)stream)) return DFL_EINVAL;
+  } else if (!launch_gemm<1, false, EPI_SILU, W8>(a, dim3(grid_x_for(I / 16), 1), (hipStream_t)stream)) {
+    return DFL_EINVAL;
+  }
   DFL_CHECK_LAUNCH(who);
   return DFL_OK;
 }
@@ -767,6 +820,8 @@
 extern "C" int dfl_gemm_silu_mul(const dfl_weight *w_gateup, const dfl_rows *x, int I, int K, void *act_frag,
                                  const int32_t *dyn, void *stream) {
   const char *who = "dfl_gemm_silu_mul";
+  if (w_gateup && w_gateup->format == DFL_W_BF16X13)
+    return gemm_silu_mul_impl<false, true>(who, w_gateup, x, I, K, act_frag, dyn, stream);
   if (!weight_ok(who, w_gateup)) return DFL_EINVAL;
   return w_gateup->format == DFL_W_BF16 ? gemm_silu_mul_impl<false>(who, w_gateup, x, I, K, act_frag, dyn, stream)
                                         : gemm_silu_mul_impl<true>(who, w_gateup, x, I, K, act_frag, dyn, stream);
@@ -805,7 +860,7 @@
 int gemm_argmax_impl(const char *who, const dfl_weight *w, const dfl_rows *x, int V, int K, int row0, int nrows,
                      const int32_t *dyn, int nrows_dyn_word, void *ws, int64_t *out_ids, int out_off, void *logits,
                      float *margin_out, hipEvent_t ev0, hipEvent_t ev1, void *stream, const SampleArgs *smp = nullptr) {
-  const bool w8 = w->format == DFL_W_E4M3;
+  const bool w8 = w->format == DFL_W_E4M3, w13 = w->format == DFL_W_BF16X13;
   DFL_REQUIRE(w->wp && ws && out_ids && (!w8 || w->scale), "%s: null pointer", who);
   DFL_REQUIRE(V > 0 && K > 0 && V % 16 == 0 && K % (w8 ? 64 : 32) == 0, "%s: need V%%16==0, K%%%d==0 (V=%d K=%d)", who,
               w8 ? 64 : 32, V, K);
@@ -847,6 +902,8 @@
       hipLaunchKernelGGL(k_gemm_s<true>, dim3(gx, 1), dim3(1024), 0, (hipStream_t)stream, GEMM_HEAD_OF(h), a, *smp);
     else
       hipLaunchKernelGGL(k_gemm_s<false>, dim3(gx, 1), dim3(1024), 0, (hipStream_t)stream, GEMM_HEAD_OF(h), a, *smp);
+  } else if (w13) {
+    if (!launch_gemm_w13<EPI_ARGMAX>(who, a, w, V, dim3(gx, 1), (hipStream_t)stream)) return DFL_EINVAL;
   } else if (w8) {
     if (!launch_gemm<1, false, EPI_ARGMAX, true>(a, dim3(gx, 1), (hipStream_t)stream)) return DFL_EINVAL;
   } else {
@@ -864,7 +921,7 @@
                                const int32_t *dyn, int nrows_dyn_word, void *ws, int64_t *out_ids, int out_off,
                                void *logits, float *margin_out, void *ev_start, void *ev_end, void *stream) {
   const char *who = "dfl_gemm_argmax";
-  if (!weight_ok(who, w)) return DFL_EINVAL;
+  if (!(w && w->format == DFL_W_BF16X13) && !weight_ok(who, w)) return DFL_EINVAL;
   return gemm_argmax_impl(who, w, x, V, K, row0, nrows, dyn, nrows_dyn_word, ws, out_ids, out_off, logits, margin_out,
                           (hipEvent_t)ev_start, (hipEvent_t)ev_end, stream);
 }
diff --git a/dflash_amd/model.py b/dflash_amd/model.py
--- a/dflash_amd/model.py
+++ b/dflash_amd/model.py
@@ -55,10 +55,12 @@
 
 
 class DFlashDraftModel:
-    def __init__(self, config, device=None, weight_format: str = "bf16"):
+    def __init__(self, config, device=None, weight_format: str = "bf16", stream_format: str = "auto"):
         if weight_format not in WEIGHT_FORMATS:
             raise ValueError(f"weight_format must be one of {WEIGHT_FORMATS}, got {weight_format!r}")
         self.weight_format = weight_format
+        self.x13 = ops.check_stream_format(stream_format) and weight_format == "bf16"
+        self.stream_format = stream_format
         self.config = DFlashConfig.from_any(config)
         c = self.config
         if c.head_dim != 128:
@@ -74,6 +76,7 @@
         if weight_format == "fp8_e4m3" and any(k % 64 for k in (c.hidden_size, c.intermediate_size, c.fc_in, c.q_dim)):
             raise NotImplementedError("fp8_e4m3 weights need hidden, intermediate, fc input and q widths % 64 == 0")
         self.w: Optional[dict] = None
+        self.gu13: list = []
         self.w8: Optional[dict] = None
         self.fp8_stream = True
         self._ws = None
@@ -121,6 +124,7 @@
              "norm": dev("norm.weight"), "layers": []}
         if fp8:
             w8["fc"] = ops.pack_weight_fp8(*top8.pop("fc"))
+        gu13 = []
         for i in range(c.num_hidden_layers):
             p = f"layers.{i}."
             l8 = {}
@@ -139,6 +143,8 @@
                 "q_norm": dev(p + "self_attn.q_norm.weight"), "k_norm": dev(p + "self_attn.k_norm.weight"),
                 "ln1": dev(p + "input_layernorm.weight"), "ln2": dev(p + "post_attention_layernorm.weight"),
             })
+            gu13.append(ops.bf16x13_twin(w["layers"][-1]["gu"], 2 * c.intermediate_size, c.hidden_size, "gateup")
+                        if self.x13 else None)
             del qkv, gate, up, o, down
         w["kv_all"] = torch.cat([lw["qkv"][c.q_dim * c.hidden_size:] for lw in w["layers"]]).contiguous()
         w["k_norm_all"] = torch.stack([lw["k_norm"] for lw in w["layers"]]).contiguous()
@@ -151,16 +157,17 @@
         torch.cuda.synchronize(self.device)
         self.w = w
         self.w8 = w8
+        self.gu13 = gu13
         self._tile_layers = {}
         self._ws = None
         return self
 
     @classmethod
-    def from_pretrained(cls, path: str, device=None, weight_format: str = "bf16", **_):
+    def from_pretrained(cls, path: str, device=None, weight_format: str = "bf16", stream_format: str = "auto", **_):
         from safetensors.torch import load_file
         with open(os.path.join(path, "config.json")) as f:
             cfg = json.load(f)
-        model = cls(cfg, device=device, weight_format=weight_format)
+        model = cls(cfg, device=device, weight_format=weight_format, stream_format=stream_format)
         sd = {}
         for fn in sorted(os.listdir(path)):
             if fn.endswith(".safetensors"):
@@ -234,6 +241,8 @@
         if key not in self._lm_head_cache:
             self._lm_head_cache.clear()
             self._lm_head_cache[key] = ops.pack_weight(wt.detach().to(device=self.device, dtype=BF16).contiguous())
+            if self.x13:
+                ops.bf16x13_twin(self._lm_head_cache[key], wt.shape[0], wt.shape[1], "lm_head")
         return self._lm_head_cache[key]
 
     def packed_lm_head_fp8(self, lm_head) -> ops.Fp8Weight:
@@ -430,8 +439,9 @@
                 if not fuse_o:
                     ops.gemm_resid(lm["o"], src["attn"][t], H, c.q_dim, hrow[t], add_residual=True, ss_out=ws["ss_h"][t],
                                    dyn=dt)
+            gu = lm["gu"] if ww is not w or self.gu13[i] is None else self.gu13[i]
             for t, dt in tiles:
-                ops.gemm_silu_mul(lm["gu"], src["ln2"][i][t], I, H, ws["act_frag"][t], dt)
+                ops.gemm_silu_mul(gu, src["ln2"][i][t], I, H, ws["act_frag"][t], dt)
             for t, dt in tiles:
                 ops.gemm_resid(lm["down"], src["act"][t], H, I, hrow[t], add_residual=True, ss_out=ws["ss_h"][t],
                                dyn=dt)
@@ -514,7 +524,10 @@
             ev = self.lm_head_events if t == 0 else None
             if ev is not None and self.lm_head_events_log is not None:
                 self.lm_head_events_log.append(ev)
-            ops.gemm_argmax(lm_head_wp, x, c.vocab_size, c.hidden_size, row0, nrows, ws["argmax_ws"], block_ids,
+            head = lm_head_wp
+            if self.x13 and isinstance(head, torch.Tensor):
+                head = ops.bf16x13_twin(head, c.vocab_size, c.hidden_size, "lm_head") or head
+            ops.gemm_argmax(head, x, c.vocab_size, c.hidden_size, row0, nrows, ws["argmax_ws"], block_ids,
                             16 * t + row0, logits=None if logits is None else logits[16 * t:16 * t + 16],
                             margins=margins, events=ev)
 
diff --git a/dflash_amd/ops.py b/dflash_amd/ops.py
--- a/dflash_amd/ops.py
+++ b/dflash_amd/ops.py
@@ -4,7 +4,7 @@
 
 import torch
 
-from ._lib import W_BF16, W_E4M3, Rows, Weight, check, lib
+from ._lib import W_BF16, W_BF16X13, W_E4M3, Rows, Weight, check, lib
 
 BF16, F32, I32, I64 = torch.bfloat16, torch.float32, torch.int32, torch.int64
 DYN_S, DYN_TAU, DYN_BS, DYN_POS0, DYN_START, DYN_STOP, DYN_CYCLE = range(7)
@@ -158,7 +158,101 @@
     return cache[qkv_parts]
 
 
+X13_QUAD_BYTES = 3328
+STREAM_FORMATS = ("auto", "bf16")
+X13_KINDS = {"gateup": True, "lm_head": True}
+
+
+class Bf16x13Weight(NamedTuple):
+    data: torch.Tensor
+    N: int
+    K: int
+
+
+def bf16x13_covers(N: int, K: int) -> bool:
+    return N > 0 and N % 16 == 0 and K in (2048, 4096)
+
+
+def pack_weight_bf16x13(wp: torch.Tensor, N: int, K: int, tiles_per_pass: int = 256):
+    if not bf16x13_covers(N, K):
+        raise ValueError(f"dflash_amd: bf16x13 covers K = 2048 or 4096 and N % 16 == 0 (N={N} K={K})")
+    if wp.dtype != BF16 or wp.numel() != N * K:
+        raise ValueError("dflash_amd: pack_weight_bf16x13 takes the packed bf16 weight of N * K elements")
+    nt, KS, dev = N // 16, K // 32, wp.device
+    nfr, Q = KS // 16, KS // 4
+    src = wp.view(torch.int16).view(nt, KS, 64, 8)
+    qbytes = nt * Q * X13_QUAD_BYTES
+    data = torch.empty(qbytes + nt * 16 * 8, dtype=U8, device=dev)
+    quads, meta = data[:qbytes].view(nt, Q, X13_QUAD_BYTES), data[qbytes:].view(I32).view(nt, 16, 2)
+    rsh = torch.arange(8, dtype=I32, device=dev).view(1, 1, 4, 1, 2, 1)
+    patched = refused = 0
+    for t0 in range(0, nt, tiles_per_pass):
+        wi = src[t0:t0 + tiles_per_pass].to(I32) & 0xffff
+        T = wi.shape[0]
+        lo, h7, sign = (wi & 0xff).to(U8), (wi >> 8) & 0x7f, wi >> 15
+        hb = (h7.amax(dim=(1, 2, 3)) - 15).clamp_(min=0)
+        c = h7 - hb.view(T, 1, 1, 1)
+        exc = (h7 != 0) & (c < 1)
+        c = torch.where(c < 1, torch.zeros_like(c), c)
+        ex = exc.view(T, 16, nfr * 512)
+        cnt = ex.sum(dim=2)
+        refused += int((cnt > 1).sum())
+        patched += int((cnt == 1).sum())
+        idx = ex.to(I32).argmax(dim=2)
+        raw = wi.view(T, 16, nfr * 512).gather(2, idx.unsqueeze(2)).squeeze(2)
+        word = ((8 + idx // 512) << 28) | (((idx // 8) % 64) << 22) | ((idx % 8) << 19) | raw
+        word = torch.where(cnt == 1, word - (1 << 32), torch.zeros_like(word)).to(I32)
+        meta[t0:t0 + T, :, 0] = hb.to(I32).view(T, 1)
+        meta[t0:t0 + T, :, 1] = word
+        lq = lo.view(T, Q, 4, 64, 8)
+        cq = c.view(T, Q, 4, 64, 8)
+        nb = (cq[..., :4] | (cq[..., 4:] << 4)).to(U8)
+        sg = (sign.view(T, Q, 4, 64, 2, 4) << rsh).sum(dim=(2, 4)).to(U8)
+        out = quads[t0:t0 + T]
+        out[:, :, 0:1024] = lq[:, :, 0:2].permute(0, 1, 3, 2, 4).reshape(T, Q, 1024)
+        out[:, :, 1024:2048] = lq[:, :, 2:4].permute(0, 1, 3, 2, 4).reshape(T, Q, 1024)
+        out[:, :, 2048:3072] = nb.permute(0, 1, 3, 2, 4).reshape(T, Q, 1024)
+        out[:, :, 3072:3328] = sg.reshape(T, Q, 256)
+    report = {"items": nt * 16, "patched": patched, "refused": refused}
+    if refused:
+        return None, report
+    return Bf16x13Weight(data, N, K), report
+
+
+_x13_twins = {}
+
+
+def bf16x13_twin(wp: torch.Tensor, N: int, K: int, kind: str):
+    import weakref
+    if not X13_KINDS[kind] or not bf16x13_covers(N, K):
+        return None
+    key = wp.data_ptr()
+    hit = _x13_twins.get(key)
+    if hit is None or hit[0]() is not wp or hit[1:3] != (N, K):
+        for k in [k for k, v in _x13_twins.items() if v[0]() is None]:
+            del _x13_twins[k]
+        twin, report = pack_weight_bf16x13(wp, N, K)
+        hit = _x13_twins[key] = (weakref.ref(wp), N, K, twin, report)
+    return hit[3]
+
+
+def bf16x13_report() -> dict:
+    live = [v for v in _x13_twins.values() if v[0]() is not None]
+    return {"packed": sum(v[3] is not None for v in live), "kept_bf16": sum(v[3] is None for v in live),
+            "patched_items": sum(v[4]["patched"] for v in live), "refused_items": sum(v[4]["refused"] for v in live)}
+
+
+def check_stream_format(stream_format: str) -> bool:
+    if stream_format not in STREAM_FORMATS:
+        raise ValueError(f"stream_format must be one of {STREAM_FORMATS}, got {stream_format!r}")
+    return stream_format == "auto"
+
+
 def _w(wp, N: int, K: int, name: str) -> Weight:
+    if isinstance(wp, Bf16x13Weight):
+        if (wp.N, wp.K) != (N, K):
+            raise ValueError(f"dflash_amd: {name} is a bf16x13 weight of {wp.N} x {wp.K}, the launch asks for {N} x {K}")
+        return Weight(_p(wp.data, U8, name), None, W_BF16X13)
     if not isinstance(wp, Fp8Weight):
         return Weight(_p(wp, BF16, name), None, W_BF16)
     if (wp.N, wp.K) != (N, K):
diff --git a/dflash_amd/target.py b/dflash_amd/target.py
--- a/dflash_amd/target.py
+++ b/dflash_amd/target.py
@@ -56,7 +56,10 @@
 
 class NativeTarget:
     def __init__(self, hf_model, max_splits: int = 32, attn_impl: str = "head", keep_hf: bool = True,
-                 prefill: str = "native", weight_format: str = "bf16", expert_format: str = "bf16"):
+                 prefill: str = "native", weight_format: str = "bf16", expert_format: str = "bf16",
+                 stream_format: str = "auto"):
+        self.x13 = ops.check_stream_format(stream_format) and weight_format == "bf16"
+        self.stream_format = stream_format
         if attn_impl not in ("head", "fused"):
             raise ValueError("attn_impl must be 'head' or 'fused'")
         if prefill not in ("native", "hf"):
@@ -138,9 +141,10 @@
             mat("lm_head.weight", h8, "lm")
             self.lm_wp8 = ops.pack_weight_fp8(*h8.pop("lm"))
         self.layers = []
+        self.gu13 = []
         for i in range(self.L):
             p = f"model.layers.{i}."
-            l8 = {}
+            l8, gu13 = {}, None
             qkv = torch.cat([mat(p + "self_attn.q_proj.weight", l8, "q"), mat(p + "self_attn.k_proj.weight", l8, "k"),
                              mat(p + "self_attn.v_proj.weight", l8, "v")], dim=0)
             has_qk = (p + "self_attn.q_norm.weight") in sd
@@ -186,6 +190,8 @@
                 lw["gu"] = ops.pack_weight_gateup(mat(p + "mlp.gate_proj.weight", l8, "gate"),
                                                   mat(p + "mlp.up_proj.weight", l8, "up"))
                 lw["down"] = ops.pack_weight(mat(p + "mlp.down_proj.weight", l8, "down"))
+                if self.x13:
+                    gu13 = ops.bf16x13_twin(lw["gu"], 2 * self.I, self.H, "gateup")
                 if e8:
                     self.experts8.append(None)
             if fp8:
@@ -193,6 +199,7 @@
                     raise NotImplementedError("NativeTarget: fp8_e4m3 needs dense MLP layers")
                 self.layers8.append(ops.pack_layer_fp8(l8))
             self.layers.append(lw)
+            self.gu13.append(gu13)
             del qkv, l8
         self.norm = w("model.norm.weight")
         self.embed = w("model.embed_tokens.weight")
@@ -249,6 +256,7 @@
                 raise NotImplementedError("NativeTarget(keep_hf=False) needs the native prefill (widths % 128, FFN widths % 64)")
             if self.lm_wp is None:
                 self.lm_wp = ops.pack_weight(self.lm_head.weight.detach().to(BF16).contiguous())
+                self._head_twin()
             self.hf = None
             self.model = SimpleNamespace(embed_tokens=_Weight(self.embed), rotary_emb=self._rotary)
             self.lm_head = _Weight(self.lm_head.weight.detach())
@@ -304,6 +312,11 @@
 
     def share_lm_head(self, packed: torch.Tensor) -> None:
         self.lm_wp = packed
+        self._head_twin()
+
+    def _head_twin(self) -> None:
+        if self.x13 and self.lm_wp is not None:
+            ops.bf16x13_twin(self.lm_wp, self.V, self.H, "lm_head")
 
     def streams_fp8(self, bs: int = 16) -> bool:
         if self.layers8 is None or not self.fp8_stream or self.attn_impl != "head" or self.wide_hidden:
@@ -658,6 +671,7 @@
         w8 = self.streams_fp8(bs)
         Lm = self.layers8 if w8 else Ls
         head = self.lm_wp8 if w8 else self.lm_wp
+        x13 = self.x13 and not w8
         if len(tiles) == 2 and self.wide_one_pass and self.attn_impl == "head":
             return self._verify_wide(block_ids, start, cache, bs, tap_layers, taps, logits_out, temperature, cos, sin, seed,
                                      flt)
@@ -702,8 +716,9 @@
                 gev = self.gu_events if (self.gu_events is not None and self.gu_events[0] == i) else None
                 if gev is not None:
                     gev[1].record()
+                gu = self.gu13[i] if x13 and self.gu13[i] is not None else lm["gu"]
                 for t, dt in tiles:
-                    ops.gemm_silu_mul(lm["gu"], src["ln2"][i][t], self.I, H, ws["act"][t], dt)
+                    ops.gemm_silu_mul(gu, src["ln2"][i][t], self.I, H, ws["act"][t], dt)
                 if gev is not None:
                     gev[2].record()
                 for t, dt in tiles:
@@ -737,6 +752,8 @@
             return post[:bs].unsqueeze(0), taps
         if temperature >= 1e-5:
             logits = torch.empty(16 * len(tiles), self.V, dtype=BF16, device=self._dev)
+        elif x13:
+            head = ops.bf16x13_twin(head, self.V, H, "lm_head") or head
         for t, dt in tiles:
             ops.gemm_argmax(head, fin[t], self.V, H, 0, min(16, bs - 16 * t), ws["argmax_ws"], post, 16 * t,
                             dyn=dt, logits=None if logits is None else logits[16 * t:16 * t + 16])
diff --git a/include/dflash_hip.h b/include/dflash_hip.h
--- a/include/dflash_hip.h
+++ b/include/dflash_hip.h
@@ -34,7 +34,7 @@
   int32_t mode;
 } dfl_rows;
 
-enum { DFL_W_BF16 = 0, DFL_W_E4M3 = 1 };
+enum { DFL_W_BF16 = 0, DFL_W_E4M3 = 1, DFL_W_BF16X13 = 2 };
 typedef struct dfl_weight {
   const void *wp;
   const float *scale;
```

Measured after the change: 1802, median of 6. 1.04x the previous value.
